# pigimonaco/Pinocchio

Measured on AMD Instinct MI355X. Metric: grid-cells/sec for full Fmax sweep (all smoothing radii) + 3LPT, 1024^3 box, higher is better.
Workload: dtype f64

## Files before the change

### include/pinfmax.h

```cpp
#ifndef PINFMAX_H
#define PINFMAX_H

#include <stddef.h>
#include <stdint.h>

#ifdef __cplusplus
extern "C" {
#endif

#define PF_NBINS 210
#define PF_MAX_SMOOTH 64

typedef struct pf_ctx pf_ctx;

typedef struct {
  int64_t n;
  int     rank;
  int     nranks;
  int     device;
  int     field_bytes;
  int     flags;
} pf_config;

#define PF_FLAG_TIMING 1
// ... 140 lines not shown
int pf_gather_velocities(pf_ctx *ctx, const pf_peak_region *box, size_t count, const unsigned int *frag_pos, const int *order,
                         size_t capacity, unsigned int *index, void *vel24, size_t *found);
int pf_refresh_velocities(pf_ctx *ctx, const pf_peak_region *box, size_t count, const unsigned int *frag_pos, const int *order,
                          void *frag, const pf_product_layout *layout, const pf_prev_layout *prev, size_t *found);
int pf_debug_gather_velocities(int n, int x0, int nxl, int pb, const void *cols24, const pf_peak_region *box, size_t count,
                               const unsigned int *frag_pos, const int *order, unsigned int *index, void *vel24, size_t *found);
typedef struct { size_t stride; long off_Mass, off_Vel, off_Vel_2LPT, off_Vel_3LPT_1, off_Vel_3LPT_2,
                 off_Vel_prev, off_Vel_2LPT_prev, off_Vel_3LPT_1_prev, off_Vel_3LPT_2_prev; } pf_group_layout;
int pf_group_velocity_sums(pf_ctx *ctx, const pf_peak_region *box, size_t count, const unsigned int *frag_pos,
                           const int *group_id, size_t group_stride, int first_group,
                           size_t capacity, int *group, unsigned int *npart, double *sum24,
                           size_t *groups_found, size_t *particles_found);
int pf_refresh_segment(pf_ctx *ctx, const pf_peak_region *box, size_t count, const unsigned int *frag_pos, const int *order,
                       const int *group_id, size_t group_stride, int first_group,
                       void *frag, const pf_product_layout *layout, const pf_prev_layout *prev,
                       void *groups, size_t ngroups, const pf_group_layout *gl,
                       size_t *loose, size_t *grouped, size_t *mass_mismatch);
int pf_debug_group_velocity_sums(int n, int x0, int nxl, int pb, const void *cols24, const pf_peak_region *box, size_t count,
                                 const unsigned int *frag_pos, const int *group_id, int first_group,
                                 int *group, unsigned int *npart, double *sum24, size_t *groups_found, size_t *particles_found);
int pf_debug_groupvel_times(double *ms3);
#define PF_PLC_LAST_CHECK 0
#define PF_PLC_EVENTS 1
typedef struct { int n; const double *x, *comvdist, *hubble; int nk; const double *grow[4], *fomega[4];
                 double logkmin, deltalogk, k_for_GM, rad_gm0; int nsmooth; const double *k_gm_displ; } pf_plc_cosmology;
typedef struct { int i, j, k; double F1, F2; } pf_plc_replication;
typedef struct { double center[3], xvers[3], yvers[3], zvers[3], aperture, Fstop, InterPartDist; long long GSglobal[3];
                 size_t nrep; const pf_plc_replication *repls; double LastzForPLC, delta_z; int nzbins; } pf_plc_geometry;
typedef struct { int myseg, use_v31; double z_seg, z_prev; } pf_plc_segment;
typedef struct { size_t stride; long off_Mass, off_Pos, off_name, off_Flast, off_good, off_point, off_Vel, off_Vel_2LPT, off_Vel_3LPT_1, off_Vel_3LPT_2,
                 off_Vel_prev, off_Vel_2LPT_prev, off_Vel_3LPT_1_prev, off_Vel_3LPT_2_prev; } pf_plc_group_layout;
typedef struct { size_t stride; long off_Mass, off_name, off_z, off_x, off_v; } pf_plc_out_layout;
int pf_plc_set_cosmology(pf_ctx *ctx, const pf_plc_cosmology *cosmo);
int pf_plc_set_geometry(pf_ctx *ctx, const pf_plc_geometry *geom);
int pf_plc_cross(pf_ctx *ctx, int mode, const pf_plc_segment *seg, const pf_peak_region *box,
                 size_t ncand, const void *groups, const pf_plc_group_layout *gl,
                 const void *f_lo, size_t f_lo_stride, int min_mass,
                 size_t capacity, void *plcgroups, const pf_plc_out_layout *ol,
                 unsigned int *cand_of, int *rep_of, double *nz,
                 size_t *count, size_t *unconverged);
int pf_debug_plc_times(double *ms2);
typedef struct { double F, InterPartDist, ParticleMass, hfactor; long long GSglobal[3]; int pbc[3]; int min_mass; } pf_catalog_params;
typedef struct { size_t stride; long off_name, off_M, off_x, off_v, off_q, off_n; } pf_catalog_out_layout;
typedef struct { int nbin; double mmin, deltam; } pf_mf_bins;
int pf_catalog(pf_ctx *ctx, const pf_plc_segment *seg, const pf_peak_region *box, const pf_catalog_params *par,
               size_t ngroups, const void *groups, const pf_plc_group_layout *gl,
               size_t capacity, void *catalog, const pf_catalog_out_layout *ol, unsigned int *group_of,
               const pf_mf_bins *bins, int *ninbin, double *massinbin, size_t *count);
int pf_debug_catalog_times(double *ms2);
int pf_debug_catalog_parts(double *ms4);
typedef struct { double sigma0, k_sigma, k_point; int order; } pf_point_params;
int pf_point_states(pf_ctx *ctx, const pf_plc_segment *seg, const pf_peak_region *box, const pf_point_params *par,
                    size_t count, const unsigned int *frag_pos, const int *order,
                    size_t capacity, unsigned int *index, void *states, size_t *found);
int pf_debug_point_states(int n, int x0, int nxl, int pb, const void *fmax_col, const void *cols24,
                          pf_ctx *tables_ctx, const pf_plc_segment *seg, const pf_peak_region *box, const pf_point_params *par,
                          size_t count, const unsigned int *frag_pos, const int *order,
                          unsigned int *index, void *states, size_t *found);
int pf_debug_point_times(double *ms2);
int pf_get_block(pf_ctx *ctx, const char *name, int id_bytes, void *host);
int pf_get_second_derivative(pf_ctx *ctx, int i, double *host);
int pf_get_kvector(pf_ctx *ctx, int which, double *host);
int pf_get_density(pf_ctx *ctx, double *host);
int pf_debug_replicated_rows(pf_ctx *ctx, int kx0, int nkx, double *host);
int pf_forward_transform(pf_ctx *ctx, const double *real_host, double *spec_host);
int pf_reverse_transform(pf_ctx *ctx, const double *spec_host, double *real_host);
int pf_derivative(pf_ctx *ctx, const double *spec_host, int first_derivative, int second_derivative, double rs_cells,
                  int order, double *real_host);
int pf_debug_math(pf_ctx *ctx, int which, const double *a, const double *b, size_t count, double *out);
int pf_debug_stream_rate(pf_ctx *ctx, int kind, int reps, double *gbps);
int pf_debug_lines(int field_bytes, int n, int pass, int mul, int band, int nouter, int ncols, int pre, double rs,
                   double growth, int outer_offset, const double *in, double *out);
int pf_debug_pk(int which, const float *a, const float *b, float *out, int count);
int pf_debug_gfft(int n, int dir, const double *in, double *out);
int pf_debug_gfft_lines(int n, int mode, int dir, int nlines, const double *in, double *out);
int pf_debug_strided_jobs(int field_bytes, int n, int njobs, int nin, const int *in_of, const int *mul, int nouter, int ncols,
                          const double *in, double *out);
int pf_debug_strided_band(int field_bytes, int n, int njobs, int nin, const int *in_of, const int *mul, int nouter, int ncols,
                          int in_pitch, int out_pitch, int band_e, int band_outer, int outer_offset, int pre, double rs, double growth,
                          const double *in, double *out, int *guard_ok);
int pf_debug_zpass_jobs(int field_bytes, int n, int form, int njobs, const int *mul, const int *out_f32, int in_place, int nrows, int band,
                        double norm, const double *dc, int ncu, const double *spec, const double *hess, const double *acc, double *out,
                        int *sentinel_ok);
int pf_debug_strided_xfuse(int field_bytes, int n, int njobs, const int *mul, int nouter, int ncols, int pre, double rs, double growth,
                           int outer_offset, const double *in, double *out_fused, double *out_plain);
int pf_debug_invariant_reruns(pf_ctx *ctx);
int pf_solve_ran_beside_zpass(pf_ctx *ctx);
int pf_transform_path(pf_ctx *ctx);
int pf_invgrow_table_status(pf_ctx *ctx, int ismooth, double *max_rel_err);
int pf_collapse_cells(pf_ctx *ctx, int ismooth, const double *d, size_t count, double *F);
enum { PF_ARITH_FAST = 0, PF_ARITH_EXACT = 1 };
int pf_set_arithmetic(pf_ctx *ctx, int flavour);
int pf_get_arithmetic(pf_ctx *ctx);
#define PF_CENSUS_BINS 64
typedef struct {
  unsigned long long cells;
  unsigned long long differing_bits;
  unsigned long long hist[PF_CENSUS_BINS];
  unsigned long long beyond_2ulp;
  unsigned long long rmax_differing;
  unsigned long long nonfinite;
  unsigned long long outliers;
  double max_abs, max_ulps;
  unsigned long long max_abs_cell;
} pf_census;
typedef struct { unsigned long long cell; double fast, exact; int rmax_fast, rmax_exact; } pf_census_cell;
int pf_flavour_census(pf_ctx *ctx, int ns, const double *radius_cells, double *true_variance,
                      pf_census *out, size_t capacity, pf_census_cell *cells);
int pf_debug_census(int product_bytes, unsigned long long first_cell, size_t count,
                    const void *fmax_fast, const int *rmax_fast, const void *fmax_exact, const int *rmax_exact,
                    pf_census *out, size_t capacity, pf_census_cell *cells);

int pf_power_bins(int n);
typedef struct {
  unsigned long long modes;
  unsigned long long nonfinite;
} pf_power_info;
int pf_power_spectrum(pf_ctx *ctx, int which, int ns, const double *radius_cells,
                      unsigned long long *nmodes, unsigned long long *k2sum, double *power,
                      double *variance, pf_power_info *info);
int pf_debug_power_spectrum(int field_bytes, int n, int y0, int nyl, const double *spec_host,
                            int ns, const double *radius_cells,
                            unsigned long long *nmodes, unsigned long long *k2sum, double *power,
                            double *variance, pf_power_info *info);
int pf_debug_power_times(double *ms);

#define PF_MATTER_NGP 1
#define PF_MATTER_DECONVOLVE 2
typedef struct {
  unsigned long long deposited, nonfinite, outside, empty_cells, max_cell, sum_hi32, sum_lo32, modes, nonfinite_modes;
} pf_matter_info;
int pf_matter_power(pf_ctx *ctx, int flags, const double *weight,
                    unsigned long long *nmodes, unsigned long long *k2sum, double *power, double *cross,
                    double *density_host, pf_matter_info *info);
int pf_debug_matter_deposit(int pb, int n, const void *vel12_host, int flags, const double *weight,
                            unsigned long long *grid_host, pf_matter_info *info);
int pf_debug_matter_shells(int field_bytes, int n, int y0, int nyl, const double *spec_m, const double *spec_lin,
                           int flags, unsigned long long *nmodes, unsigned long long *k2sum, double *power, double *cross,
                           pf_matter_info *info);
int pf_debug_matter_times(double *ms);
int pf_debug_matter_form(int *form);

int pf_matter_power_slabs(pf_ctx *ctx, int flags, const double *weight,
                          unsigned long long *nmodes, unsigned long long *k2sum, double *power, double *cross,
                          double *density_host, pf_matter_info *info);
int pf_debug_matter_slabs(pf_ctx *ctx, const void *vel12_slab_host, int flags, const double *weight,
                          unsigned long long *grid_slab_host, pf_matter_info *info);
int pf_debug_matter_exchange(unsigned long long out[6]);

#define PF_HALO_NGP 1
#define PF_HALO_DECONVOLVE 2
#define PF_HALO_MASS_WEIGHT 4
#define PF_HALO_MAX_BINS 8
typedef struct {
  unsigned long long selected, weight_sum, weight2_hi, weight2_lo, nonfinite, outside,
                     empty_cells, max_cell, modes, nonfinite_modes;
} pf_halo_info;
int pf_halo_power(pf_ctx *ctx, int flags, size_t count, const double *pos, double scale, const int *mass,
                  int nbins, const int *mass_range,
                  unsigned long long *nmodes, unsigned long long *k2sum,
                  double *power, double *cross, pf_halo_info *info);
int pf_debug_halo_deposit(int n, int x0, int nxl, int flags, size_t count, const double *pos, double scale,
                          const int *mass, int lo, int hi, unsigned long long *grid_host, pf_halo_info *info);
int pf_debug_halo_times(double *ms);

#define PF_MULTIPOLE_ORDERS 3
// ... 45 lines not shown
```

### pinocchio_amd/_lib.py

```python
from __future__ import annotations

import ctypes as C
import os

PKG = os.path.dirname(os.path.abspath(__file__))
SO = os.environ.get("PINFMAX_LIB") or os.path.join(PKG, "libpinfmax_hip.so")
NBINS = 210
MAX_SMOOTH = 64

FLAG_TIMING = 1
FLAG_DOUBLE_PRODUCTS = 2
MAP_CURRENT = 0
MAP_UPDATE = 1
NEIGH_SKIP, NEIGH_GOOD, NEIGH_PEAK = 1, 2, 4


class Config(C.Structure):
    _fields_ = [("n", C.c_int64), ("rank", C.c_int), ("nranks", C.c_int), ("device", C.c_int),
                ("field_bytes", C.c_int), ("flags", C.c_int)]


class ProductLayout(C.Structure):
    _fields_ = [("stride", C.c_size_t), ("off_Rmax", C.c_int), ("off_Fmax", C.c_int), ("off_Vel", C.c_int),
                ("off_Vel_2LPT", C.c_int), ("off_Vel_3LPT_1", C.c_int), ("off_Vel_3LPT_2", C.c_int)]
# ... 181 lines not shown
                                C.POINTER(C.c_uint), C.POINTER(C.c_size_t)]),
    "pf_debug_distribute": (C.c_int, [C.c_int, C.c_int, C.c_int, C.POINTER(C.c_float), C.c_double, C.POINTER(SubBox), C.POINTER(C.c_uint),
                                      C.c_size_t, C.POINTER(C.c_uint), C.POINTER(C.c_uint), C.POINTER(C.c_size_t)]),
    "pf_distribute_sorted": (C.c_int, [_vp, C.c_double, C.POINTER(SubBox), C.POINTER(C.c_uint), C.POINTER(ProductLayout), C.c_size_t, _vp,
                                       C.POINTER(C.c_uint), C.POINTER(C.c_uint), C.POINTER(C.c_int), C.POINTER(C.c_size_t)]),
    "pf_organize": (C.c_int, [_vp, C.POINTER(ProductLayout), C.c_size_t, _vp, C.POINTER(C.c_uint), C.POINTER(C.c_uint), C.POINTER(C.c_int)]),
    "pf_debug_organize": (C.c_int, [C.c_size_t, C.POINTER(C.c_float), C.POINTER(C.c_uint), C.POINTER(C.c_uint), C.POINTER(C.c_uint), C.POINTER(C.c_int)]),
    "pf_map_create": (C.c_int, [_vp, C.POINTER(PeakRegion), C.POINTER(_vp)]),
    "pf_map_destroy": (None, [_vp]),
    "pf_map_length": (C.c_size_t, [_vp]),
    "pf_map_fill_box": (C.c_int, [_vp]),
    "pf_map_update": (C.c_int, [_vp, C.c_size_t, _dp, C.POINTER(C.c_int), C.c_double, C.POINTER(C.c_ulonglong)]),
    "pf_map_commit": (C.c_int, [_vp, C.c_int]),
    "pf_map_get": (C.c_int, [_vp, C.c_int, C.POINTER(C.c_uint)]),
    "pf_map_set": (C.c_int, [_vp, C.c_int, C.POINTER(C.c_uint)]),
    "pf_map_count": (C.c_int, [_vp, C.c_int, C.POINTER(C.c_ulonglong)]),
    "pf_debug_map_atomics": (C.c_int, [_vp, C.POINTER(C.c_ulonglong)]),
    "pf_distribute_map": (C.c_int, [_vp, C.c_double, _vp, C.c_int, C.POINTER(ProductLayout), C.c_size_t, _vp, C.POINTER(C.c_uint),
                                    C.POINTER(C.c_size_t)]),
    "pf_distribute_sorted_map": (C.c_int, [_vp, C.c_double, _vp, C.c_int, C.POINTER(ProductLayout), C.c_size_t, _vp, C.POINTER(C.c_uint),
                                           C.POINTER(C.c_uint), C.POINTER(C.c_int), C.POINTER(C.c_size_t)]),
    "pf_count_peaks_map": (C.c_int, [_vp, C.c_double, _vp, C.c_int, C.POINTER(C.c_ulonglong)]),
    "pf_neighbours": (C.c_int, [_vp, C.POINTER(PeakRegion), C.c_size_t, C.POINTER(C.c_uint), _vp, C.c_size_t, C.POINTER(C.c_int),
                                C.POINTER(C.c_ubyte), C.POINTER(C.c_ulonglong)]),
    "pf_debug_neigh_ms": (C.c_int, [_dp, _dp]),
    "pf_distribute_sorted_neighbours_map": (C.c_int, [_vp, C.c_double, _vp, C.c_int, C.POINTER(ProductLayout), C.c_size_t, _vp, C.POINTER(C.c_uint),
                                                      C.POINTER(C.c_uint), C.POINTER(C.c_int), C.POINTER(C.c_int), C.POINTER(C.c_ubyte),
                                                      C.POINTER(C.c_ulonglong), C.POINTER(C.c_size_t)]),
    "pf_back_reset": (C.c_int, [_vp]),
    "pf_distribute_back": (C.c_int, [_vp, C.POINTER(PeakRegion), C.c_size_t, C.POINTER(C.c_uint), _vp, C.c_size_t, _vp, C.c_size_t, C.POINTER(C.c_size_t)]),
    "pf_back_apply": (C.c_int, [_vp, C.c_size_t, _vp, C.c_size_t, _vp, C.c_size_t, _vp, C.c_size_t]),
    "pf_update_back": (C.c_int, [_vp, _vp, C.c_size_t, C.c_long, C.c_long]),
    "pf_debug_distribute_back": (C.c_int, [C.c_int, C.c_int, C.c_int, C.POINTER(PeakRegion), C.c_size_t, C.POINTER(C.c_uint), C.POINTER(C.c_float),
                                           C.POINTER(C.c_int), C.POINTER(C.c_float), C.POINTER(C.c_int), C.POINTER(C.c_size_t)]),
    "pf_shift_displacements": (C.c_int, [_vp]),
    "pf_drop_prev": (C.c_int, [_vp]),
    "pf_prev_shifts": (C.c_int, [_vp]),
    "pf_gather_velocities": (C.c_int, [_vp, C.POINTER(PeakRegion), C.c_size_t, C.POINTER(C.c_uint), C.POINTER(C.c_int), C.c_size_t, C.POINTER(C.c_uint), _vp,
                                       C.POINTER(C.c_size_t)]),
    "pf_refresh_velocities": (C.c_int, [_vp, C.POINTER(PeakRegion), C.c_size_t, C.POINTER(C.c_uint), C.POINTER(C.c_int), _vp, C.POINTER(ProductLayout),
                                        C.POINTER(PrevLayout), C.POINTER(C.c_size_t)]),
    "pf_debug_gather_velocities": (C.c_int, [C.c_int, C.c_int, C.c_int, C.c_int, _vp, C.POINTER(PeakRegion), C.c_size_t, C.POINTER(C.c_uint), C.POINTER(C.c_int),
                                             C.POINTER(C.c_uint), _vp, C.POINTER(C.c_size_t)]),
    "pf_group_velocity_sums": (C.c_int, [_vp, C.POINTER(PeakRegion), C.c_size_t, C.POINTER(C.c_uint), C.POINTER(C.c_int), C.c_size_t, C.c_int, C.c_size_t,
                                         C.POINTER(C.c_int), C.POINTER(C.c_uint), C.POINTER(C.c_double), C.POINTER(C.c_size_t), C.POINTER(C.c_size_t)]),
    "pf_refresh_segment": (C.c_int, [_vp, C.POINTER(PeakRegion), C.c_size_t, C.POINTER(C.c_uint), C.POINTER(C.c_int), C.POINTER(C.c_int), C.c_size_t, C.c_int,
                                     _vp, C.POINTER(ProductLayout), C.POINTER(PrevLayout), _vp, C.c_size_t, C.POINTER(GroupLayout), C.POINTER(C.c_size_t),
                                     C.POINTER(C.c_size_t), C.POINTER(C.c_size_t)]),
    "pf_debug_group_velocity_sums": (C.c_int, [C.c_int, C.c_int, C.c_int, C.c_int, _vp, C.POINTER(PeakRegion), C.c_size_t, C.POINTER(C.c_uint),
                                               C.POINTER(C.c_int), C.c_int, C.POINTER(C.c_int), C.POINTER(C.c_uint), C.POINTER(C.c_double),
                                               C.POINTER(C.c_size_t), C.POINTER(C.c_size_t)]),
    "pf_debug_groupvel_times": (C.c_int, [C.POINTER(C.c_double)]),
    "pf_plc_set_cosmology": (C.c_int, [_vp, C.POINTER(PlcCosmology)]),
    "pf_plc_set_geometry": (C.c_int, [_vp, C.POINTER(PlcGeometry)]),
    "pf_plc_cross": (C.c_int, [_vp, C.c_int, C.POINTER(PlcSegment), C.POINTER(PeakRegion), C.c_size_t, _vp, C.POINTER(PlcGroupLayout), _vp, C.c_size_t, C.c_int,
                               C.c_size_t, _vp, C.POINTER(PlcOutLayout), C.POINTER(C.c_uint), C.POINTER(C.c_int), C.POINTER(C.c_double), C.POINTER(C.c_size_t),
                               C.POINTER(C.c_size_t)]),
    "pf_debug_plc_times": (C.c_int, [C.POINTER(C.c_double)]),
    "pf_catalog": (C.c_int, [_vp, C.POINTER(PlcSegment), C.POINTER(PeakRegion), C.POINTER(CatalogParams), C.c_size_t, _vp, C.POINTER(PlcGroupLayout), C.c_size_t, _vp,
                             C.POINTER(CatalogOutLayout), C.POINTER(C.c_uint), C.POINTER(MfBins), C.POINTER(C.c_int), C.POINTER(C.c_double), C.POINTER(C.c_size_t)]),
    "pf_debug_catalog_times": (C.c_int, [C.POINTER(C.c_double)]),
    "pf_debug_catalog_parts": (C.c_int, [C.POINTER(C.c_double)]),
    "pf_point_states": (C.c_int, [_vp, C.POINTER(PlcSegment), C.POINTER(PeakRegion), C.POINTER(PointParams), C.c_size_t, C.POINTER(C.c_uint), C.POINTER(C.c_int),
                                  C.c_size_t, C.POINTER(C.c_uint), _vp, C.POINTER(C.c_size_t)]),
    "pf_debug_point_states": (C.c_int, [C.c_int, C.c_int, C.c_int, C.c_int, _vp, _vp, _vp, C.POINTER(PlcSegment), C.POINTER(PeakRegion), C.POINTER(PointParams),
                                        C.c_size_t, C.POINTER(C.c_uint), C.POINTER(C.c_int), C.POINTER(C.c_uint), _vp, C.POINTER(C.c_size_t)]),
    "pf_debug_point_times": (C.c_int, [C.POINTER(C.c_double)]),
    "pf_set_collapse_model": (C.c_int, [_vp, C.c_int, C.POINTER(C.c_double), C.c_int, C.POINTER(C.c_double)]),
    "pf_set_modified_gravity": (C.c_int, [_vp, C.c_double, C.c_double, C.c_int, C.POINTER(C.c_double)]),
    "pf_set_tabulated_ct": (C.c_int, [_vp, C.c_int, C.POINTER(C.c_double)]),
    "pf_ct_build": (C.c_int, [_vp, C.c_int, C.c_double, C.POINTER(C.c_double)]),
    "pf_ct_load": (C.c_int, [_vp, C.c_int, C.c_double, C.POINTER(C.c_double)]),
    "pf_debug_math": (C.c_int, [_vp, C.c_int, C.POINTER(C.c_double), C.POINTER(C.c_double), C.c_size_t, C.POINTER(C.c_double)]),
    "pf_debug_stream_rate": (C.c_int, [_vp, C.c_int, C.c_int, _dp]),
    "pf_debug_lines": (C.c_int, [C.c_int, C.c_int, C.c_int, C.c_int, C.c_int, C.c_int, C.c_int, C.c_int, C.c_double, C.c_double, C.c_int, _dp, _dp]),
    "pf_debug_pk": (C.c_int, [C.c_int, C.POINTER(C.c_float), C.POINTER(C.c_float), C.POINTER(C.c_float), C.c_int]),
    "pf_debug_gfft": (C.c_int, [C.c_int, C.c_int, _dp, _dp]),
    "pf_debug_gfft_lines": (C.c_int, [C.c_int, C.c_int, C.c_int, C.c_int, _dp, _dp]),
    "pf_debug_strided_jobs": (C.c_int, [C.c_int, C.c_int, C.c_int, C.c_int, C.POINTER(C.c_int), C.POINTER(C.c_int), C.c_int, C.c_int, _dp, _dp]),
    "pf_debug_strided_band": (C.c_int, [C.c_int, C.c_int, C.c_int, C.c_int, C.POINTER(C.c_int), C.POINTER(C.c_int), C.c_int, C.c_int, C.c_int, C.c_int,
                                        C.c_int, C.c_int, C.c_int, C.c_int, C.c_double, C.c_double, _dp, _dp, C.POINTER(C.c_int)]),
    "pf_debug_zpass_jobs": (C.c_int, [C.c_int, C.c_int, C.c_int, C.c_int, C.POINTER(C.c_int), C.POINTER(C.c_int), C.c_int, C.c_int, C.c_int, C.c_double,
                                      _dp, C.c_int, _dp, _dp, _dp, _dp, C.POINTER(C.c_int)]),
    "pf_debug_strided_xfuse": (C.c_int, [C.c_int, C.c_int, C.c_int, C.POINTER(C.c_int), C.c_int, C.c_int, C.c_int, C.c_double, C.c_double, C.c_int,
                                         _dp, _dp, _dp]),
    "pf_debug_invariant_reruns": (C.c_int, [_vp]),
    "pf_solve_ran_beside_zpass": (C.c_int, [_vp]),
    "pf_transform_path": (C.c_int, [_vp]),
    "pf_invgrow_table_status": (C.c_int, [_vp, C.c_int, _dp]),
    "pf_set_loopback_exchange": (C.c_int, [_vp, C.c_int]),
    "pf_loopback_active": (C.c_int, [_vp]),
    "pf_set_sources_in_sweep": (C.c_int, [_vp, C.c_int]),
    "pf_set_lpt_order": (C.c_int, [_vp, C.c_int]),
    "pf_set_ct_interpolation": (C.c_int, [_vp, C.c_int]),
    "pf_set_transposed_spectra": (C.c_int, [_vp, C.c_int]),
    "pf_replicated_spectrum": (C.c_int, [_vp]),
    "pf_update_products": (C.c_int, [_vp, _vp, C.POINTER(ProductLayout)]),
    "pf_set_growth_table": (C.c_int, [_vp, C.c_int, C.POINTER(C.c_double), C.c_int, C.c_double, C.c_double, C.c_double]),
    "pf_get_second_derivative": (C.c_int, [_vp, C.c_int, _dp]),
    "pf_get_kvector": (C.c_int, [_vp, C.c_int, _dp]),
    "pf_get_density": (C.c_int, [_vp, _dp]),
    "pf_debug_replicated_rows": (C.c_int, [_vp, C.c_int, C.c_int, _dp]),
    "pf_plan_bytes": (C.c_int, [C.POINTER(Config), C.POINTER(C.c_size_t), C.POINTER(C.c_size_t)]),
    "pf_forward_transform": (C.c_int, [_vp, _dp, _dp]),
    "pf_reverse_transform": (C.c_int, [_vp, _dp, _dp]),
    "pf_collapse_cells": (C.c_int, [_vp, C.c_int, _dp, C.c_size_t, _dp]),
    "pf_set_arithmetic": (C.c_int, [_vp, C.c_int]),
    "pf_get_arithmetic": (C.c_int, [_vp]),
    "pf_flavour_census": (C.c_int, [_vp, C.c_int, _dp, _dp, C.POINTER(Census), C.c_size_t, C.POINTER(CensusCell)]),
    "pf_debug_census": (C.c_int, [C.c_int, C.c_ulonglong, C.c_size_t, _vp, C.POINTER(C.c_int), _vp, C.POINTER(C.c_int), C.POINTER(Census), C.c_size_t,
                                  C.POINTER(CensusCell)]),
    "pf_power_bins": (C.c_int, [C.c_int]),
    "pf_power_spectrum": (C.c_int, [_vp, C.c_int, C.c_int, _dp, C.POINTER(C.c_ulonglong), C.POINTER(C.c_ulonglong), _dp, _dp, C.POINTER(PowerInfo)]),
    "pf_debug_power_spectrum": (C.c_int, [C.c_int, C.c_int, C.c_int, C.c_int, _dp, C.c_int, _dp, C.POINTER(C.c_ulonglong), C.POINTER(C.c_ulonglong), _dp, _dp,
                                          C.POINTER(PowerInfo)]),
    "pf_debug_power_times": (C.c_int, [_dp]),
    "pf_matter_power": (C.c_int, [_vp, C.c_int, _dp, C.POINTER(C.c_ulonglong), C.POINTER(C.c_ulonglong), _dp, _dp, _dp, C.POINTER(MatterInfo)]),
    "pf_debug_matter_deposit": (C.c_int, [C.c_int, C.c_int, _vp, C.c_int, _dp, C.POINTER(C.c_ulonglong), C.POINTER(MatterInfo)]),
    "pf_debug_matter_shells": (C.c_int, [C.c_int, C.c_int, C.c_int, C.c_int, _dp, _dp, C.c_int, C.POINTER(C.c_ulonglong), C.POINTER(C.c_ulonglong), _dp, _dp,
                                         C.POINTER(MatterInfo)]),
    "pf_debug_matter_times": (C.c_int, [_dp]),
    "pf_debug_matter_form": (C.c_int, [C.POINTER(C.c_int)]),
    "pf_matter_power_slabs": (C.c_int, [_vp, C.c_int, _dp, C.POINTER(C.c_ulonglong), C.POINTER(C.c_ulonglong), _dp, _dp, _dp, C.POINTER(MatterInfo)]),
    "pf_debug_matter_slabs": (C.c_int, [_vp, _vp, C.c_int, _dp, C.POINTER(C.c_ulonglong), C.POINTER(MatterInfo)]),
    "pf_debug_matter_exchange": (C.c_int, [C.POINTER(C.c_ulonglong)]),
    "pf_halo_power": (C.c_int, [_vp, C.c_int, C.c_size_t, _dp, C.c_double, C.POINTER(C.c_int), C.c_int, C.POINTER(C.c_int), C.POINTER(C.c_ulonglong),
                                C.POINTER(C.c_ulonglong), _dp, _dp, C.POINTER(HaloInfo)]),
    "pf_debug_halo_deposit": (C.c_int, [C.c_int, C.c_int, C.c_int, C.c_int, C.c_size_t, _dp, C.c_double, C.POINTER(C.c_int), C.c_int, C.c_int,
                                        C.POINTER(C.c_ulonglong), C.POINTER(HaloInfo)]),
    "pf_debug_halo_times": (C.c_int, [_dp]),
    "pf_halo_multipoles": (C.c_int, [_vp, C.c_int, C.c_size_t, _dp, _dp, C.c_double, C.c_double, C.c_int, C.POINTER(C.c_int), C.c_int, C.POINTER(C.c_int),
                                     C.POINTER(C.c_ulonglong), C.POINTER(C.c_ulonglong), _dp, _dp, C.POINTER(HaloInfo)]),
    "pf_debug_halo_deposit_rsd": (C.c_int, [C.c_int, C.c_int, C.c_int, C.c_int, C.c_size_t, _dp, _dp, C.c_double, C.c_double, C.c_int, C.POINTER(C.c_int), C.c_int, C.c_int,
                                            C.POINTER(C.c_ulonglong), C.POINTER(HaloInfo)]),
    "pf_debug_multipole_shells": (C.c_int, [C.c_int, C.c_int, C.c_int, C.c_int, _dp, _dp, C.c_int, C.c_int, C.POINTER(C.c_ulonglong), C.POINTER(C.c_ulonglong), _dp, _dp, _dp,
                                            C.POINTER(MatterInfo)]),
    "pf_debug_multipole_form": (C.c_int, [C.POINTER(C.c_int)]),
    "pf_halo_correlation": (C.c_int, [_vp, C.c_int, C.c_size_t, _dp, _dp, C.c_double, C.c_double, C.c_int, C.POINTER(C.c_int), C.c_int, C.POINTER(C.c_int),
                                      C.POINTER(C.c_ulonglong), C.POINTER(C.c_ulonglong), _dp, _dp, C.POINTER(CorrInfo)]),
    "pf_debug_corr_form": (C.c_int, [C.c_int, C.c_int, C.c_int, C.c_int, _dp, _dp, C.c_int, C.c_int, _dp, C.POINTER(MatterInfo)]),
    "pf_debug_corr_shells": (C.c_int, [C.c_int, C.c_int, C.c_int, C.c_int, _dp, C.c_int, C.POINTER(C.c_ulonglong), C.POINTER(C.c_ulonglong), _dp, _dp,
                                       C.POINTER(C.c_ulonglong)]),
    "pf_debug_corr_times": (C.c_int, [_dp]),
    "pf_get_cputime": (C.c_int, [_vp, C.POINTER(CpuTime)]),
    "pf_reset_cputime": (C.c_int, [_vp]),
    "pf_kernel_stats": (C.c_int, [_vp, C.POINTER(KernelStat), C.c_int, C.POINTER(C.c_int)]),
    "pf_reset_kernel_stats": (C.c_int, [_vp]),
    "pf_synchronize": (C.c_int, [_vp]),
    "pf_device_bytes": (C.c_size_t, [_vp]),
}

_lib = None


def source_sha() -> str:
    import glob
    import hashlib
    h = hashlib.sha256()
    for path in sorted(glob.glob(os.path.join(PKG, "csrc", "*.hip")) + glob.glob(os.path.join(PKG, "csrc", "*.h")) +
                       glob.glob(os.path.join(PKG, "csrc", "*.cpp"))):
        h.update(os.path.basename(path).encode())
        with open(path, "rb") as fh:
            h.update(fh.read())
    return h.hexdigest()[:16]


# ... 15 lines not shown
```

### pinocchio_amd/csrc/pf_api.hip

```cpp
#include <hip/hip_runtime.h>

#include <math.h>
#include <stdarg.h>
#include <stdio.h>
#include <stdlib.h>
#include <string.h>

#include <atomic>
#include <string>
#include <functional>
#include <vector>

#include "../../include/pinfmax.h"
#include "pf_collapse_core.h"
#include "pf_hostpool.h"
#include "pf_internal.h"

extern "C" void pf_rccl_release(void *link);
extern "C" int pf_rccl_link_count(void *link);

static thread_local char g_err[512] = "";
int pf_fail(int task, const char *fmt, ...) {
  va_list ap;
  va_start(ap, fmt);
// ... 181 lines not shown
  }
  c->evs.clear();
  for (auto &e : c->phase_evs) {
    float ms = 0; hipEventElapsedTime(&ms, e.a, e.b);
    double s = 1e-3 * ms;
    if (e.kind == 0) c->cpu.deriv += s; else if (e.kind == 1) c->cpu.coll += s; else if (e.kind == 2) c->cpu.lpt += s;
    else if (e.kind == 3) c->cpu.mem_transf += s; else if (e.kind == 4) c->cpu.fmax += s;
    c->evpool.push_back(e.a); c->evpool.push_back(e.b);
  }
  c->phase_evs.clear();
}

static size_t ncell_of(const pf_ctx *c) { return (size_t)c->nxl * c->n * c->n; }
static int dev_alloc(pf_ctx *c, void **p, size_t bytes) {
  HIPCHK(c, hipMalloc(p, bytes));
  c->dev_bytes += bytes;
  return 0;
}

static int ensure_b2(pf_ctx *c, bool quiet = false) {
  if (c->blockB2) return 0;
  if (hipMalloc((void **)&c->blockB2, 6 * c->field_bytes) != hipSuccess) {
    (void)hipGetLastError(); c->blockB2 = nullptr;
    return quiet ? 1 : pf_fail(c->rank, "hipMalloc of the second field set failed (%.1f GB; %.1f GB held by this context)", 6e-9 * c->field_bytes, 1e-9 * c->dev_bytes);
  }
  c->dev_bytes += 6 * c->field_bytes;
  for (int i = 0; i < 6; i++) c->B2[i] = c->blockB2 + i * c->field_bytes;
  return 0;
}
static int inv_rows(pf_ctx *c, int set, bool quiet = false) {
  if (c->INV[set][0]) return 0;
  const size_t row_set = ncell_of(c) * sizeof(double);
  if (2 * c->field_bytes < row_set) return pf_fail(c->rank, "internal: an invariant row set does not fit two fields");
  if (set == 1) {
    if (ensure_b2(c, quiet)) return 1;
    for (int k = 0; k < 3; k++) c->INV[1][k] = (double *)(c->blockB2 + 2 * k * c->field_bytes);
    return 0;
  }
  for (int k = 0; k < 2; k++)
    if (!c->inv_own[k]) PFCHK(c, dev_alloc(c, (void **)&c->inv_own[k], row_set));
  c->INV[0][0] = (double *)c->blockS; c->INV[0][1] = c->inv_own[0]; c->INV[0][2] = c->inv_own[1];
  return 0;
}

static void host_twiddles(int n, int fb, std::vector<char> &h) {
  h.resize((size_t)n * 2 * fb);
  for (int j = 0; j < n; j++) {
    long double a = 2.0L * 3.14159265358979323846264338327950288L * (long double)j / (long double)n;
    double re = (double)cosl(a), im = (double)sinl(a);
    if (j == 0) { re = 1; im = 0; } else if (4 * j == n) { re = 0; im = 1; } else if (2 * j == n) { re = -1; im = 0; } else if (4 * j == 3 * n) { re = 0; im = -1; }
    if (fb == 8) { ((double *)h.data())[2 * j] = re; ((double *)h.data())[2 * j + 1] = im; }
    else { ((float *)h.data())[2 * j] = (float)re; ((float *)h.data())[2 * j + 1] = (float)im; }
  }
}

extern "C" void pf_layout_3lpt(pf_product_layout *l) {
  l->stride = 56; l->off_Rmax = 0; l->off_Fmax = 4; l->off_Vel = 8; l->off_Vel_2LPT = 20; l->off_Vel_3LPT_1 = 32; l->off_Vel_3LPT_2 = 44;
}

static size_t ncell(const pf_ctx *c) { return (size_t)c->nxl * c->n * c->n; }
static long long rpitch(const pf_ctx *c) { return c->general ? c->n : 2 * c->nzp; }
static double spec_bytes_alg(const pf_ctx *c) { return (double)c->n * c->nyl * c->nzh * 2.0 * c->fb; }
static double real_bytes_alg(const pf_ctx *c) { return (double)ncell(c) * c->fb; }

static int env_int(const char *name, int dflt) { const char *e = getenv(name); return e ? atoi(e) : dflt; }
static void read_tuning(PfTuning *t) {
  t->zpass_persist = env_int("PF_ZPASS_PERSIST", 24);
  t->zpass_inv_wg_per_cu = env_int("PF_ZPASS_INV_WG_PER_CU", 32);
  if (t->zpass_inv_wg_per_cu <= 0) t->zpass_inv_wg_per_cu = 32;
  t->spline_lut = env_int("PF_SPLINE_LUT", 1) != 0;
  t->exchange_rows = env_int("PF_EXCHANGE_ROWS", 1) != 0;
  t->invariants = env_int("PF_INVARIANTS", 1);
  t->lpt_fuse = env_int("PF_LPT_FUSE", 1);
  t->collapse_wg_per_cu = env_int("PF_COLLAPSE_WG_PER_CU", 8);
  if (t->collapse_wg_per_cu <= 0) t->collapse_wg_per_cu = 8;
  t->general = env_int("PF_GENERAL", 0) != 0;

  t->pipeline = env_int("PF_PIPELINE", 1) != 0;
  t->replicate = env_int("PF_REPLICATE_DK", -1);
  t->exact_libm = env_int("PF_EXACT_LIBM", 0) != 0;
  t->solve_beside_z = env_int("PF_SOLVE_BESIDE_Z", -1);
  t->gtab = env_int("PF_GTAB", 1) != 0;
  t->lpt_xfuse = env_int("PF_LPT_XFUSE", 1) != 0;
  t->lpt3b_start = env_int("PF_LPT3B_START", 0) != 0;
  t->preflight = env_int("PF_PREFLIGHT", 1) != 0;
  t->handoff_chunk_mb = env_int("PF_HANDOFF_CHUNK_MB", 256);
  if (t->handoff_chunk_mb <= 0) t->handoff_chunk_mb = 256;
  t->handoff_threads = env_int("PF_HANDOFF_THREADS", 0);
  t->host_register = env_int("PF_HOST_REGISTER", 0) != 0;
  t->distribute_lds = env_int("PF_DISTRIBUTE_LDS", 1) != 0;
  const char *fault = getenv("PF_DEBUG_PIPELINE_FAULT");
  t->debug_fault = !fault ? 0 : !strcmp(fault, "recv") ? 1 : !strcmp(fault, "send") ? 2 : 0;
  t->prune_eps = 8.673617379884035e-19;
  if (const char *e = getenv("PF_PRUNE_EPS")) t->prune_eps = atof(e);
}

static void plan_bytes(const pf_ctx *c, size_t *at_create, size_t *peak) {
  const size_t field = c->field_bytes, nc = ncell_of(c);
  size_t fields = 1 + 3 + 6 + 3;
  if (c->P > 1) fields += 3;
  if (c->replicate) fields += (size_t)c->P;
  if (c->pipeline) fields += 6;
  if (c->general) fields += 1;
  size_t b = fields * field + nc * ((size_t)c->pb + sizeof(int) + 12 * (size_t)c->pb);
  b += (2 * PF_NBLK + PF_NBLK + SC_COUNT) * sizeof(double) + PF_NBINS * sizeof(unsigned long long) +
       (size_t)(PF_MAX_SMOOTH + 1) * (5 * PF_KNOT_CAP * sizeof(double) + PF_GT_DOUBLES * sizeof(double) + PF_GT_MAX_BINS * sizeof(unsigned short)) +
       4 * PF_KBIN_CAP * sizeof(double) + (size_t)c->n * sizeof(double) + (size_t)c->n * 2 * c->fb;
  *at_create = b;
  b += 6 * field;
  if (c->fb == 4 && !c->general && pf_c2r_invariants_supported(c->fb, c->n)) b += 2 * nc * sizeof(double);
  *peak = b;
}
extern "C" int pf_plan_bytes(const pf_config *cfg, size_t *at_create, size_t *peak) {
  if (!cfg || cfg->nranks < 1 || cfg->n < 4 || cfg->n % cfg->nranks || (cfg->field_bytes != 4 && cfg->field_bytes != 8)) return 1;
  PfTuning tune;
  read_tuning(&tune);
  pf_ctx v;
  const int n = (int)cfg->n;
  const bool pow2 = !(n & (n - 1));
  v.n = n; v.P = cfg->nranks; v.fb = cfg->field_bytes; v.pb = (cfg->flags & PF_FLAG_DOUBLE_PRODUCTS) ? 8 : 4;
  v.general = tune.general || (!pow2 && !pf_mixed_supported(n));
  v.nzh = n / 2 + 1; v.nzp = v.general ? v.nzh : n / 2 + 64 / v.fb; v.nxl = v.nyl = n / v.P;
  v.field_bytes = (size_t)v.n * v.nyl * v.nzp * 2 * v.fb;
  v.pipeline = v.P > 1 && tune.pipeline;
  v.replicate = v.P > 1 && !v.general && (tune.replicate < 0 ? v.P <= 4 : tune.replicate != 0);
  size_t a = 0, b = 0;
  plan_bytes(&v, &a, &b);
  if (at_create) *at_create = a;
  if (peak) *peak = b;
  return 0;
}

static int create_body(pf_ctx *c, const pf_config *cfg) {
  const int rank = cfg->rank;
  HIPCHK(c, hipSetDevice(cfg->device));
  c->field_bytes = (size_t)c->n * c->nyl * c->nzp * 2 * c->fb;
  c->replicate = c->P > 1 && !c->general && (c->tune.replicate < 0 ? c->P <= 4 : c->tune.replicate != 0);
  if (c->tune.preflight) {
    size_t at_create = 0, peak = 0, free_b = 0, total_b = 0;
    plan_bytes(c, &at_create, &peak);
    HIPCHK(c, hipMemGetInfo(&free_b, &total_b));
    if (peak > free_b)
      return pf_fail(rank, "pf_create: %d^3 on %d ranks with %d-byte fields needs %.1f GB of device memory per rank (%.1f GB at creation, the rest with the "
                           "LPT part), device %d has %.1f GB free of %.1f GB", c->n, c->P, c->fb, 1e-9 * peak, 1e-9 * at_create, cfg->device, 1e-9 * free_b, 1e-9 * total_b);
  }
  HIPCHK(c, hipStreamCreate(&c->stream));
  HIPCHK(c, hipStreamCreate(&c->cstream));
  {
    int lo = 0, hi = 0;
    HIPCHK(c, hipDeviceGetStreamPriorityRange(&lo, &hi));
    HIPCHK(c, hipStreamCreateWithPriority(&c->sstream, hipStreamNonBlocking, lo));
  }
  for (int i = 0; i < 2; i++) {
    HIPCHK(c, hipEventCreateWithFlags(&c->ev_y[i], hipEventDisableTiming));
    HIPCHK(c, hipEventCreateWithFlags(&c->ev_s[i], hipEventDisableTiming));
    HIPCHK(c, hipEventCreateWithFlags(&c->ev_x[i], hipEventDisableTiming));
    HIPCHK(c, hipEventCreateWithFlags(&c->ev_r[i], hipEventDisableTiming));
  }
  {
    hipDeviceProp_t prop;
    HIPCHK(c, hipGetDeviceProperties(&prop, cfg->device));
    c->fast_libm = !c->tune.exact_libm;
    c->ncu = prop.multiProcessorCount;
    c->prune_eps = c->tune.prune_eps;
    c->collapse_blocks = prop.multiProcessorCount * c->tune.collapse_wg_per_cu;
    if (c->collapse_blocks > PF_NBLK) c->collapse_blocks = PF_NBLK;
// ... 267 lines not shown
  if (!piece) return pf_fail(c->rank, "hand-off: a record of %zu bytes does not fit the staging pieces", granule);
  const size_t np = (bytes + piece - 1) / piece;
  auto issue = [&](size_t k) -> int {
    const int b = (int)(k & 1);
    const size_t off = k * piece, len = bytes - off < piece ? bytes - off : piece;
    const char *src = src_dev ? src_dev + off : handoff_dev(c, b);
    if (fill(off, len, handoff_dev(c, b), h->st[b])) return 1;
    HIPCHK(c, hipMemcpyAsync(h->pin[b], src, len, hipMemcpyDeviceToHost, h->st[b]));
    return 0;
  };
  if (np && issue(0)) return 1;
  for (size_t k = 0; k < np; k++) {
    if (k + 1 < np && issue(k + 1)) return 1;
    const int b = (int)(k & 1);
    HIPCHK(c, hipStreamSynchronize(h->st[b]));
    const size_t off = k * piece, len = bytes - off < piece ? bytes - off : piece;
    char *dst = host + off; const char *src = h->pin[b];
    h->pool->run(len, [=](size_t a, size_t e) { memcpy(dst + a, src + a, e - a); });
  }
  return 0;
}
static int no_fill(size_t, size_t, char *, hipStream_t) { return 0; }
static int handoff_h2d(pf_ctx *c, char *dst_dev, const char *host, size_t bytes) {
  PfHandoff *h;
  if (handoff_get(c, &h)) return 1;
  PFCHK(c, handoff_begin(c, h));
  const size_t piece = h->chunk, np = (bytes + piece - 1) / piece;
  for (size_t k = 0; k < np; k++) {
    const int b = (int)(k & 1);
    const size_t off = k * piece, len = bytes - off < piece ? bytes - off : piece;
    HIPCHK(c, hipStreamSynchronize(h->st[b]));
    char *dst = h->pin[b]; const char *src = host + off;
    h->pool->run(len, [=](size_t a, size_t e) { memcpy(dst + a, src + a, e - a); });
    HIPCHK(c, hipMemcpyAsync(dst_dev + off, h->pin[b], len, hipMemcpyHostToDevice, h->st[b]));
  }
  for (int i = 0; i < 2; i++) HIPCHK(c, hipStreamSynchronize(h->st[i]));
  return 0;
}
static bool handoff_registered(pf_ctx *c, PfHandoff *h, void *host, size_t bytes) {
  if (!h->want_register || ((uintptr_t)host & 4095)) return false;
  if (h->reg_ptr == host && h->reg_bytes >= bytes) return true;
  if (h->reg_ptr) { (void)hipHostUnregister(h->reg_ptr); h->reg_ptr = nullptr; h->reg_bytes = 0; }
  if (hipHostRegister(host, bytes, hipHostRegisterDefault) != hipSuccess) { (void)hipGetLastError(); return false; }
  h->reg_ptr = host; h->reg_bytes = bytes;
  return true;
}

static int ilog2i(int v) { int l = 0; while ((1 << l) < v) l++; return l; }
static PfAddr addr_ky_x(const pf_ctx *c) {
  PfAddr a; a.os = c->nzp; a.el_shift = ilog2i(c->n); a.el_len = c->n; a.ehs = 0; a.els = (long long)c->nyl * c->nzp; return a;
}
static PfAddr addr_blocks_y(const pf_ctx *c) {
  PfAddr a; a.os = (long long)c->nyl * c->nzp; a.el_shift = ilog2i(c->nyl); a.el_len = c->nyl; a.ehs = (long long)c->nxl * c->nyl * c->nzp; a.els = c->nzp; return a;
}
static PfAddr addr_yblocks_x(const pf_ctx *c, int zp) {
  PfAddr a; a.os = (long long)c->nxl * zp; a.el_shift = ilog2i(c->nxl); a.el_len = c->nxl; a.ehs = (long long)c->nyl * c->nxl * c->nzp; a.els = zp; return a;
}
static PfAddr addr_yblocks_y(const pf_ctx *c, int zp) {
  PfAddr a; a.os = zp; a.el_shift = ilog2i(c->nyl); a.el_len = c->nyl; a.ehs = (long long)c->nyl * c->nxl * c->nzp; a.els = (long long)c->nxl * zp; return a;
}
static PfAddr addr_full_x(const pf_ctx *c) {
  PfAddr a; a.os = c->nzp; a.el_shift = ilog2i(c->n); a.el_len = c->n; a.ehs = 0; a.els = (long long)c->n * c->nzp; return a;
}
static PfAddr addr_local_x(const pf_ctx *c, int zp) {
  PfAddr a; a.os = (long long)c->nxl * zp; a.el_shift = ilog2i(c->nxl); a.el_len = c->nxl; a.ehs = 0; a.els = zp; return a;
}
static PfAddr addr_local_y(const pf_ctx *c, int zp) {
  PfAddr a; a.os = zp; a.el_shift = ilog2i(c->n); a.el_len = c->n; a.ehs = 0; a.els = (long long)c->nxl * zp; return a;
}
static PfAddr addr_xs_y(const pf_ctx *c) {
  PfAddr a; a.os = (long long)c->n * c->nzp; a.el_shift = ilog2i(c->n); a.el_len = c->n; a.ehs = 0; a.els = c->nzp; return a;
}

struct Job { const void *in; void *out; int mul; };

static int xpass(pf_ctx *c, int kind, int dir, int njobs, const Job *jobs, int pre, double rs, double growth, int nin, int band = 1 << 30,
                 bool out_yblocks = false, bool replicated = false, bool fwd_first = false) {
  PfStridedParams p; memset(&p, 0, sizeof(p));
  p.njobs = njobs;
  for (int j = 0; j < njobs; j++) { p.job[j].in = jobs[j].in; p.job[j].out = jobs[j].out; p.job[j].mul = jobs[j].mul; }
  p.ain = p.aout = addr_ky_x(c);
  if (out_yblocks) p.aout = addr_yblocks_x(c, band_zpitch(c, band));
  p.ncols = c->nzh; p.nouter = c->nyl; p.pre = pre; p.outer_offset = c->rank * c->nyl; p.rs = rs; p.growth = growth; p.tw = c->tw;
  p.etab = c->etab; p.dev = c->dev;
  if (replicated) {
    p.ain = addr_full_x(c); p.aout = addr_local_x(c, band_zpitch(c, band));
    p.nouter = c->n; p.outer_offset = 0; p.out_e0 = c->rank * c->nxl; p.out_ne = c->nxl;
  }
  if (pre && rs != 0.0) PFCHK(c, pf_launch_exp_table(c->etab, c->n, rs, c->stream));
  p.band_e = p.band_outer = c->n;
  double frac_cols = 1.0, frac_in = 1.0, frac_outer = 1.0;
  if (band < c->n / 2) {
    p.band_e = p.band_outer = band;
    p.ncols = band + 1;
    frac_cols = (double)(band + 1) / c->nzh; frac_in = frac_outer = (double)(2 * band + 1) / c->n;
  }
  KTimer t(c, kind, (nin * frac_in * (replicated ? c->P : 1) + njobs) * frac_cols * frac_outer * spec_bytes_alg(c));
  if (fwd_first) {
    if (dir < 0 || replicated) return pf_fail(c->rank, "xpass: a pending forward x-transform goes with an inverse pass over this rank's own spectrum");
    PFCHK(c, pf_launch_strided_xfuse(c->fb, c->n, p, c->stream));
    return 0;
  }
  PFCHK(c, pf_launch_strided(c->fb, c->n, dir, p, c->stream));
  return 0;
}
static int ypass(pf_ctx *c, int kind, int dir, int njobs, const Job *jobs, bool in_blocks, bool out_blocks, int nin, int band = 1 << 30,
                 bool in_yblocks = false, bool in_local = false) {
  PfStridedParams p; memset(&p, 0, sizeof(p));
  p.njobs = njobs;
  for (int j = 0; j < njobs; j++) { p.job[j].in = jobs[j].in; p.job[j].out = jobs[j].out; p.job[j].mul = jobs[j].mul; }
  p.ain = in_blocks ? (in_yblocks ? addr_yblocks_y(c, band_zpitch(c, band)) : addr_blocks_y(c)) : addr_xs_y(c);
  if (in_local) p.ain = addr_local_y(c, band_zpitch(c, band));
  p.aout = out_blocks ? addr_blocks_y(c) : addr_xs_y(c);
  p.ncols = c->nzh; p.nouter = c->nxl; p.pre = 0; p.outer_offset = 0; p.rs = 0; p.growth = 1; p.tw = c->tw; p.dev = c->dev;
  p.band_e = p.band_outer = c->n;
  double frac_cols = 1.0, frac_in = 1.0;
  if (band < c->n / 2) {
    p.band_e = band;
    p.ncols = band + 1;
    frac_cols = (double)(band + 1) / c->nzh; frac_in = (double)(2 * band + 1) / c->n;
  }
  KTimer t(c, kind, (nin * frac_in + njobs) * frac_cols * spec_bytes_alg(c));
  PFCHK(c, pf_launch_strided(c->fb, c->n, dir, p, c->stream));
  return 0;
}
struct ZJob { const void *in; void *out; int mul; int f32; };
static int zpass_c2r(pf_ctx *c, int kind, int njobs, const ZJob *jobs, const double *dc, int band = 1 << 30, bool invariants = false,
                     void *acc = nullptr) {
  PfC2RParams p; memset(&p, 0, sizeof(p));
  p.njobs = njobs;
  double outb = 0;
  for (int j = 0; j < njobs; j++) {
    p.job[j].in = jobs[j].in; p.job[j].out = jobs[j].out; p.job[j].mul = jobs[j].mul; p.job[j].out_f32 = jobs[j].f32;
    outb += jobs[j].f32 ? (double)ncell(c) * 4.0 : real_bytes_alg(c);
  }
  p.nlines = (long long)c->nxl * c->n; p.in_pitch = c->nzp; p.out_pitch = 2 * c->nzp;
  p.norm = 1.0 / ((double)c->n * c->n * c->n); p.dc = dc; p.tw = c->tw;
  p.band_k = c->n;
  double frac_in = 1.0;
  if (band < c->n / 2) { p.band_k = band; frac_in = (double)(band + 1) / c->nzh; }
  p.ncu = c->ncu; p.dev = c->dev; p.persist_per_cu = c->tune.zpass_persist; p.inv_per_cu = c->tune.zpass_inv_wg_per_cu;
  p.flag = c->scal + SC_INV_FLAG;
  if (acc) {
    p.acc = acc;
    const bool start_here = c->s3b_start_absent;
    KTimer t(c, KS_ZPASS_LPT3B, njobs * frac_in * spec_bytes_alg(c) + (start_here ? 7.0 : 8.0) * real_bytes_alg(c));
    PFCHK(c, pf_launch_c2r_invariants(c->fb, c->n, p, c->stream, start_here ? 2 : 1));
    c->s3b_start_absent = false;
    return 0;
  }
  if (invariants) {
    if (c->fb == 4) {
      if (inv_rows(c, c->inv_w)) return 1;
      for (int k = 0; k < 3; k++) p.inv_out[k] = c->INV[c->inv_w][k];
      p.inv_pitch = c->n;
      if (c->inv_w == 0) c->have_sources = false;
    }
    KTimer t(c, KS_ZPASS_INV, njobs * frac_in * spec_bytes_alg(c) + 3.0 * (double)ncell(c) * 8.0);
    PFCHK(c, pf_launch_c2r_invariants(c->fb, c->n, p, c->stream));
    return 0;
  }
  KTimer t(c, kind, njobs * frac_in * spec_bytes_alg(c) + outb);
  PFCHK(c, pf_launch_c2r(c->fb, c->n, p, c->stream));
  return 0;
}

__global__ void k_debug_idle(long long ticks) {
  const long long t0 = wall_clock64();
  while (wall_clock64() - t0 < ticks) __builtin_amdgcn_s_sleep(32);
}
template <class Pre, class Dst, class Post, class Band>
static int pipelined_band(pf_ctx *c, int count, int nf, Pre pre, Dst dst, Post post, Band band, bool local = false) {
  void *A[2][3];
  const void *R[3];
  if (local) {
    for (int i = 0; i < count; i++) {
      void *D[3];
      for (int f = 0; f < nf; f++) { D[f] = dst(i, 0, f); R[f] = D[f]; }
      if (pre(i, D)) return 1;
      if (post(i, R)) return 1;
    }
    return 0;
  }
  for (int f = 0; f < 3; f++) { A[0][f] = c->A[f]; A[1][f] = c->pipeline ? (void *)(c->blockA2 + f * c->field_bytes) : c->A[f]; }
  if (c->P == 1 || !c->pipeline) {
    for (int i = 0; i < count; i++) {
      if (pre(i, A[0])) return 1;
      for (int f = 0; f < nf; f++) {
        R[f] = A[0][f];
        if (c->P > 1) { void *d = dst(i, 0, f); PFCHK(c, exchange_band(c, A[0][f], d, band(i))); R[f] = d; }
      }
      if (post(i, R)) return 1;
    }
    return 0;
  }
  auto issue = [&](int i) -> int {
    const int s = i & 1;
    if (c->tune.debug_fault == 2) hipLaunchKernelGGL(k_debug_idle, dim3(1), dim3(1), 0, c->stream, 200000LL);
    if (pre(i, A[s])) return 1;
    HIPCHK(c, hipEventRecord(c->ev_x[s], c->stream));
    if (c->tune.debug_fault != 2) HIPCHK(c, hipStreamWaitEvent(c->cstream, c->ev_x[s], 0));
    for (int f = 0; f < nf; f++) PFCHK(c, exchange_band(c, A[s][f], dst(i, s, f), band(i), c->cstream));
    HIPCHK(c, hipEventRecord(c->ev_r[s], c->cstream));
    return 0;
  };
  if (issue(0)) return 1;
  for (int i = 0; i < count; i++) {
    if (i + 1 < count && issue(i + 1)) return 1;
    if (c->tune.debug_fault != 1) HIPCHK(c, hipStreamWaitEvent(c->stream, c->ev_r[i & 1], 0));
    for (int f = 0; f < nf; f++) R[f] = dst(i, i & 1, f);
    if (post(i, R)) return 1;
  }
  return 0;
}
template <class Pre, class Dst, class Post>
static int pipelined(pf_ctx *c, int count, int nf, Pre pre, Dst dst, Post post) {
  return pipelined_band(c, count, nf, pre, dst, post, [](int) { return 1 << 30; });
}
static void *recv_field(pf_ctx *c, int set, int f) { return (char *)(set ? c->recvA2 : c->recvA) + (size_t)f * c->field_bytes; }

static int g_filter(pf_ctx *c, const void *in, void *out, int a, int b, double rs, int order, bool normalise) {
  double growth = order ? c->growth[order - 1] : 1.0;
  const int o = order - 1;
  const bool tab = order && c->gt_n[o];
// ... 1634 lines not shown
      return pf_fail(c->rank, "pf_debug_exchange: row-range all-to-all failed");
    HIPCHK(c, hipMemcpyAsync(h.data(), recv, h.size() * 8, hipMemcpyDeviceToHost, c->stream));
    HIPCHK(c, hipStreamSynchronize(c->stream));
    for (int p = 0; p < c->P; p++)
      for (size_t i = 0; i < nw; i++) {
        const bool in = 8 * i >= off[p] && 8 * i < off[p] + len[p];
        const unsigned long long want = in ? (((unsigned long long)p << 48) | ((unsigned long long)c->rank << 40) | i) : 0ull;
        if (h[p * nw + i] != want) return pf_fail(c->rank, "pf_debug_exchange: row-range exchange, wrong word from rank %d at %zu", p, i);
      }
  }
  if (c->ared) {
    double v[2] = {1.0 + c->rank, 2.0};
    HIPCHK(c, hipMemcpyAsync(c->scal, v, sizeof(v), hipMemcpyHostToDevice, c->stream));
    if (c->ared(c->ared_user, c->scal, 2, 0, (void *)c->stream)) return pf_fail(c->rank, "pf_debug_exchange: all-reduce failed");
    HIPCHK(c, hipMemcpyAsync(v, c->scal, sizeof(v), hipMemcpyDeviceToHost, c->stream));
    HIPCHK(c, hipStreamSynchronize(c->stream));
    if (v[0] != 0.5 * c->P * (c->P + 1) || v[1] != 2.0 * c->P) return pf_fail(c->rank, "pf_debug_exchange: wrong all-reduce result");
    HIPCHK(c, hipMemsetAsync(c->scal, 0, 2 * sizeof(double), c->stream));
  }
  return 0;
}

extern "C" int pf_debug_lines(int field_bytes, int n, int pass, int mul, int band, int nouter, int ncols, int pre, double rs,
                              double growth, int outer_offset, const double *in, double *out) {
  double *flag_out = (pass == 4 && out) ? out + (size_t)3 * nouter * n : nullptr;
  if (!in || !out || nouter < 1 || (field_bytes != 8 && field_bytes != 4) || n < 8 || n > 2048 || pass < 0 || pass > 4)
    return pf_fail(0, "pf_debug_lines: bad argument");
  if (n & (n - 1)) {
    PfMixedPlan pl;
    if (!(pass <= 1 ? pf_mixed_plan(n, false, &pl) : (n % 2 == 0 && pf_mixed_plan(n / 2, true, &pl))))
      return pf_fail(0, "pf_debug_lines: no stage plan for %d points in pass %d", n, pass);
  } else if (n < 16) return pf_fail(0, "pf_debug_lines: bad argument");
  if (pass == 4 && !pf_c2r_invariants_supported(field_bytes, n))
    return pf_fail(0, "pf_debug_lines: the invariant z-pass takes rows whose six lines fit a workgroup (fp64 rows of at most 1024 points, fp32 rows of at most 2048; n = 8 m as the grids)");
  const int fb = field_bytes, nzh = n / 2 + 1;
  pf_ctx *nc = nullptr;
  size_t n_in, n_out;
  const int pc = (ncols + 15) & ~15;
  if (pass <= 1) { if (ncols < 1) return pf_fail(0, "pf_debug_lines: ncols"); n_in = n_out = (size_t)nouter * n * ncols * 2; }
  else if (pass == 2) { n_in = (size_t)nouter * nzh * 2; n_out = (size_t)nouter * n; }
  else if (pass == 3) { n_in = (size_t)nouter * n; n_out = (size_t)nouter * nzh * 2; }
  else { n_in = (size_t)6 * nouter * nzh * 2; n_out = (size_t)3 * nouter * n; }
  const size_t n_in_alloc = pass == 3 ? (n_in > n_out ? n_in : n_out) : n_in;
  void *d_in = nullptr, *d_out = nullptr, *d_tw = nullptr; double *d_etab = nullptr, *d_flag = nullptr;
  PfTuning tune;
  read_tuning(&tune);
  int dev = 0, ncu = 0;
  {
    hipDeviceProp_t prop;
    if (hipGetDevice(&dev) != hipSuccess || hipGetDeviceProperties(&prop, dev) != hipSuccess) return pf_fail(0, "pf_debug_lines: no HIP device");
    ncu = prop.multiProcessorCount;
  }
  std::vector<char> tw;
  host_twiddles(n, fb, tw);
  int rc = 0;
  auto body = [&]() -> int {
    const size_t nrows01 = (size_t)nouter * n;
    const size_t dev01 = nrows01 * (size_t)pc * 2;
    HIPCHK(nc, hipMalloc(&d_in, (pass <= 1 ? dev01 : n_in_alloc) * fb));
    const size_t out_b = (pass == 4) ? 8 : (size_t)fb;
    HIPCHK(nc, hipMalloc(&d_out, (pass <= 1 ? dev01 : n_out) * out_b));
    HIPCHK(nc, hipMalloc(&d_tw, tw.size()));
    HIPCHK(nc, hipMalloc((void **)&d_etab, (size_t)n * sizeof(double)));
    HIPCHK(nc, hipMalloc((void **)&d_flag, sizeof(double)));
    HIPCHK(nc, hipMemset(d_flag, 0, sizeof(double)));
    HIPCHK(nc, hipMemcpy(d_tw, tw.data(), tw.size(), hipMemcpyHostToDevice));
    const size_t hrow = (size_t)ncols * 2 * fb, drow = (size_t)pc * 2 * fb;
    if (pass <= 1) HIPCHK(nc, hipMemset(d_in, 0, dev01 * fb));
    if (fb == 8) {
      if (pass <= 1) HIPCHK(nc, hipMemcpy2D(d_in, drow, in, hrow, hrow, nrows01, hipMemcpyHostToDevice));
      else HIPCHK(nc, hipMemcpy(d_in, in, n_in * 8, hipMemcpyHostToDevice));
    } else {
      std::vector<float> h(n_in);
      for (size_t i = 0; i < n_in; i++) h[i] = (float)in[i];
      if (pass <= 1) HIPCHK(nc, hipMemcpy2D(d_in, drow, h.data(), hrow, hrow, nrows01, hipMemcpyHostToDevice));
      else HIPCHK(nc, hipMemcpy(d_in, h.data(), n_in * 4, hipMemcpyHostToDevice));
    }
    HIPCHK(nc, hipMemset(d_out, 0, (pass <= 1 ? dev01 : n_out) * out_b));
    if (pass <= 1) {
      PfStridedParams p; memset(&p, 0, sizeof(p));
      p.njobs = 1; p.job[0].in = d_in; p.job[0].out = d_out; p.job[0].mul = mul;
      p.ain.os = (long long)n * pc; p.ain.el_shift = ilog2i(n); p.ain.el_len = n; p.ain.ehs = 0; p.ain.els = pc; p.aout = p.ain;
      p.ncols = ncols; p.nouter = nouter; p.pre = pre; p.outer_offset = outer_offset; p.rs = rs; p.growth = growth; p.tw = d_tw; p.etab = d_etab;
      p.band_e = p.band_outer = n; p.dev = dev;
      if (band < n / 2) p.band_e = band;
      if (pre && rs != 0.0) PFCHK0(pf_launch_exp_table(d_etab, n, rs, nullptr));
      PFCHK0(pf_launch_strided(fb, n, pass == 0 ? +1 : -1, p, nullptr));
    } else if (pass == 2 || pass == 4) {
      PfC2RParams p; memset(&p, 0, sizeof(p));
      p.njobs = pass == 2 ? 1 : 6;
      static const int mul6[6] = {PF_MUL_ONE, PF_MUL_ONE, PF_MUL_K2, PF_MUL_ONE, PF_MUL_K, PF_MUL_K};
      for (int j = 0; j < p.njobs; j++) {
        p.job[j].in = (char *)d_in + (size_t)j * nouter * nzh * 2 * fb;
        p.job[j].out = pass == 2 ? d_out : (char *)d_out + (size_t)(j % 3) * nouter * n * 8;
        if (pass == 4 && j < 3) p.inv_out[j] = (double *)((char *)d_out + (size_t)j * nouter * n * 8);
        p.job[j].mul = pass == 2 ? mul : mul6[j]; p.job[j].out_f32 = 0;
      }
      p.nlines = nouter; p.in_pitch = nzh; p.out_pitch = n; p.norm = 1.0; p.dc = nullptr; p.tw = d_tw; p.band_k = band < n / 2 ? band : n;
      p.ncu = ncu; p.dev = dev; p.persist_per_cu = tune.zpass_persist; p.inv_per_cu = tune.zpass_inv_wg_per_cu; p.flag = d_flag;
      p.inv_pitch = n;
      if (pass == 2) PFCHK0(pf_launch_c2r(fb, n, p, nullptr));
      else PFCHK0(pf_launch_c2r_invariants(fb, n, p, nullptr, 0));
    } else {
      PfR2CParams p; p.in = d_in; p.out = d_out; p.nlines = nouter; p.in_pitch = n; p.out_pitch = nzh; p.tw = d_tw;
      PFCHK0(pf_launch_r2c(fb, n, p, nullptr));
    }
    HIPCHK(nc, hipDeviceSynchronize());
    if (pass == 4 && flag_out) HIPCHK(nc, hipMemcpy(flag_out, d_flag, sizeof(double), hipMemcpyDeviceToHost));
    if (fb == 8 || pass == 4) {
      if (pass <= 1) HIPCHK(nc, hipMemcpy2D(out, hrow, d_out, drow, hrow, nrows01, hipMemcpyDeviceToHost));
      else HIPCHK(nc, hipMemcpy(out, d_out, n_out * 8, hipMemcpyDeviceToHost));
    } else {
      std::vector<float> h(n_out);
      if (pass <= 1) HIPCHK(nc, hipMemcpy2D(h.data(), hrow, d_out, drow, hrow, nrows01, hipMemcpyDeviceToHost));
      else HIPCHK(nc, hipMemcpy(h.data(), d_out, n_out * 4, hipMemcpyDeviceToHost));
      for (size_t i = 0; i < n_out; i++) out[i] = (double)h[i];
    }
    return 0;
  };
  rc = body();
  hipFree(d_in); hipFree(d_out); hipFree(d_tw); hipFree(d_etab); hipFree(d_flag);
  return rc;
}

extern "C" int pf_debug_strided_jobs(int field_bytes, int n, int njobs, int nin, const int *in_of, const int *mul, int nouter, int ncols,
                                     const double *in, double *out) {
  if (!in || !out || !in_of || !mul || njobs < 1 || njobs > PF_MAX_JOBS || nin < 1 || nin > njobs || nouter < 1 || ncols < 1 || (field_bytes != 8 && field_bytes != 4) ||
      n < 16 || n > 2048 || ((n & (n - 1)) && !pf_mixed_supported(n)))
    return pf_fail(0, "pf_debug_strided_jobs: bad argument");
  const int fb = field_bytes, pc = (ncols + 15) & ~15;
  pf_ctx *nc = nullptr;
  const size_t nrows = (size_t)nouter * n, field = nrows * (size_t)pc * 2;
  void *d_in = nullptr, *d_out = nullptr, *d_tw = nullptr;
  int dev = 0;
  if (hipGetDevice(&dev) != hipSuccess) return pf_fail(0, "pf_debug_strided_jobs: no HIP device");
  std::vector<char> tw;
  host_twiddles(n, fb, tw);
  auto body = [&]() -> int {
    HIPCHK(nc, hipMalloc(&d_in, (size_t)nin * field * fb));
    HIPCHK(nc, hipMalloc(&d_out, (size_t)njobs * field * fb));
    HIPCHK(nc, hipMalloc(&d_tw, tw.size()));
    HIPCHK(nc, hipMemcpy(d_tw, tw.data(), tw.size(), hipMemcpyHostToDevice));
    HIPCHK(nc, hipMemset(d_in, 0, (size_t)nin * field * fb));
    HIPCHK(nc, hipMemset(d_out, 0, (size_t)njobs * field * fb));
    const size_t hrow = (size_t)ncols * 2 * fb, drow = (size_t)pc * 2 * fb, hfield = nrows * (size_t)ncols * 2;
    std::vector<float> hf;
    for (int i = 0; i < nin; i++) {
      const void *src = in + (size_t)i * hfield;
      if (fb == 4) { hf.resize(hfield); for (size_t k = 0; k < hfield; k++) hf[k] = (float)in[(size_t)i * hfield + k]; src = hf.data(); }
      HIPCHK(nc, hipMemcpy2D((char *)d_in + (size_t)i * field * fb, drow, src, hrow, hrow, nrows, hipMemcpyHostToDevice));
    }
    PfStridedParams p; memset(&p, 0, sizeof(p));
    p.njobs = njobs;
    for (int j = 0; j < njobs; j++) {
      if (in_of[j] < 0 || in_of[j] >= nin) return pf_fail(0, "pf_debug_strided_jobs: in_of");
      p.job[j].in = (char *)d_in + (size_t)in_of[j] * field * fb; p.job[j].out = (char *)d_out + (size_t)j * field * fb; p.job[j].mul = mul[j];
    }
    p.ain.os = (long long)n * pc; p.ain.el_shift = (n & (n - 1)) ? 0 : ilog2i(n); p.ain.el_len = n; p.ain.ehs = 0; p.ain.els = pc; p.aout = p.ain;
    p.ncols = ncols; p.nouter = nouter; p.tw = d_tw; p.band_e = p.band_outer = n; p.dev = dev; p.growth = 1.0;
    PFCHK0(pf_launch_strided(fb, n, +1, p, nullptr));
    HIPCHK(nc, hipDeviceSynchronize());
    for (int j = 0; j < njobs; j++) {
      if (fb == 8) HIPCHK(nc, hipMemcpy2D(out + (size_t)j * hfield, hrow, (char *)d_out + (size_t)j * field * fb, drow, hrow, nrows, hipMemcpyDeviceToHost));
      else {
        hf.resize(hfield);
        HIPCHK(nc, hipMemcpy2D(hf.data(), hrow, (char *)d_out + (size_t)j * field * fb, drow, hrow, nrows, hipMemcpyDeviceToHost));
        for (size_t k = 0; k < hfield; k++) out[(size_t)j * hfield + k] = (double)hf[k];
      }
    }
    return 0;
  };
  const int rc = body();
  hipFree(d_in); hipFree(d_out); hipFree(d_tw);
  return rc;
}

extern "C" int pf_debug_strided_band(int field_bytes, int n, int njobs, int nin, const int *in_of, const int *mul, int nouter, int ncols,
                                     int in_pitch, int out_pitch, int band_e, int band_outer, int outer_offset, int pre, double rs, double growth,
                                     const double *in, double *out, int *guard_ok) {
  if (!in || !out || !in_of || !mul || !guard_ok || njobs < 1 || njobs > PF_MAX_JOBS || nin < 1 || nin > njobs || nouter < 1 || ncols < 1 ||
      (field_bytes != 8 && field_bytes != 4) || n < 16 || n > 2048 || ((n & (n - 1)) && !pf_mixed_supported(n)) || band_e < 0 || band_outer < 0 ||
      outer_offset < 0 || outer_offset >= n)
    return pf_fail(0, "pf_debug_strided_band: bad argument");
  const int fb = field_bytes, line = 64 / fb;
  if (in_pitch < ncols || out_pitch < ncols || in_pitch % line || out_pitch % line || in_pitch > 4096 || out_pitch > 4096)
    return pf_fail(0, "pf_debug_strided_band: rows of %d columns need pitches of whole 128-byte lines (%d complex) that hold them, not %d / %d", ncols, line, in_pitch, out_pitch);
  for (int j = 0; j < njobs; j++) if (in_of[j] < 0 || in_of[j] >= nin) return pf_fail(0, "pf_debug_strided_band: in_of");
  *guard_ok = 0;
  pf_ctx *nc = nullptr;
  const size_t nrows = (size_t)nouter * n, cb = (size_t)2 * fb;
  const size_t in_field = nrows * (size_t)in_pitch * cb, out_field = nrows * (size_t)out_pitch * cb;
  const size_t slot = (in_field > out_field ? in_field : out_field) + 4096, guard = slot - out_field;
  void *d_in = nullptr, *d_out = nullptr, *d_tw = nullptr; double *d_etab = nullptr;
  int dev = 0;
  if (hipGetDevice(&dev) != hipSuccess) return pf_fail(0, "pf_debug_strided_band: no HIP device");
  std::vector<char> tw;
  host_twiddles(n, fb, tw);
  auto body = [&]() -> int {
    HIPCHK(nc, hipMalloc(&d_in, (size_t)nin * in_field));
    HIPCHK(nc, hipMalloc(&d_out, (size_t)njobs * slot));
    HIPCHK(nc, hipMalloc(&d_tw, tw.size()));
    HIPCHK(nc, hipMalloc((void **)&d_etab, (size_t)n * sizeof(double)));
    HIPCHK(nc, hipMemcpy(d_tw, tw.data(), tw.size(), hipMemcpyHostToDevice));
    HIPCHK(nc, hipMemset(d_in, 0x7f, (size_t)nin * in_field));
    for (int j = 0; j < njobs; j++) {
      HIPCHK(nc, hipMemset((char *)d_out + (size_t)j * slot, 0, out_field));
      HIPCHK(nc, hipMemset((char *)d_out + (size_t)j * slot + out_field, 0xa5, guard));
    }
    const size_t hrow = (size_t)ncols * cb, hfield = nrows * (size_t)ncols * 2;
    std::vector<float> hf;
    for (int i = 0; i < nin; i++) {
      const void *src = in + (size_t)i * hfield;
      if (fb == 4) { hf.resize(hfield); for (size_t k = 0; k < hfield; k++) hf[k] = (float)in[(size_t)i * hfield + k]; src = hf.data(); }
      HIPCHK(nc, hipMemcpy2D((char *)d_in + (size_t)i * in_field, (size_t)in_pitch * cb, src, hrow, hrow, nrows, hipMemcpyHostToDevice));
    }
    PfStridedParams p; memset(&p, 0, sizeof(p));
    p.njobs = njobs;
    for (int j = 0; j < njobs; j++) { p.job[j].in = (char *)d_in + (size_t)in_of[j] * in_field; p.job[j].out = (char *)d_out + (size_t)j * slot; p.job[j].mul = mul[j]; }
    p.ain.os = (long long)n * in_pitch; p.ain.el_shift = (n & (n - 1)) ? 0 : ilog2i(n); p.ain.el_len = n; p.ain.ehs = 0; p.ain.els = in_pitch;
    p.aout = p.ain; p.aout.os = (long long)n * out_pitch; p.aout.els = out_pitch;
    p.ncols = ncols; p.nouter = nouter; p.pre = pre ? 1 : 0; p.outer_offset = outer_offset; p.rs = rs; p.growth = growth; p.tw = d_tw; p.etab = d_etab; p.dev = dev;
    p.band_e = band_e < n / 2 ? band_e : n; p.band_outer = band_outer < n / 2 ? band_outer : n;
    if (pre && rs != 0.0) PFCHK0(pf_launch_exp_table(d_etab, n, rs, nullptr));
    PFCHK0(pf_launch_strided(fb, n, +1, p, nullptr));
    HIPCHK(nc, hipDeviceSynchronize());
    for (int j = 0; j < njobs; j++) {
      const char *f = (const char *)d_out + (size_t)j * slot;
      if (fb == 8) HIPCHK(nc, hipMemcpy2D(out + (size_t)j * hfield, hrow, f, (size_t)out_pitch * cb, hrow, nrows, hipMemcpyDeviceToHost));
      else {
        hf.resize(hfield);
        HIPCHK(nc, hipMemcpy2D(hf.data(), hrow, f, (size_t)out_pitch * cb, hrow, nrows, hipMemcpyDeviceToHost));
        for (size_t k = 0; k < hfield; k++) out[(size_t)j * hfield + k] = (double)hf[k];
      }
    }
    std::vector<unsigned char> g(guard);
    int ok = 1;
    for (int j = 0; j < njobs; j++) {
      HIPCHK(nc, hipMemcpy(g.data(), (const char *)d_out + (size_t)j * slot + out_field, guard, hipMemcpyDeviceToHost));
      for (size_t k = 0; k < guard; k++) if (g[k] != 0xa5) { ok = 0; break; }
    }
    *guard_ok = ok;
    return 0;
  };
  const int rc = body();
  hipFree(d_in); hipFree(d_out); hipFree(d_tw); hipFree(d_etab);
  return rc;
}

extern "C" int pf_debug_zpass_jobs(int field_bytes, int n, int form, int njobs, const int *mul, const int *out_f32, int in_place, int nrows, int band,
                                   double norm, const double *dc, int ncu, const double *spec, const double *hess, const double *acc, double *out,
                                   int *sentinel_ok) {
  static const int mul6[6] = {PF_MUL_ONE, PF_MUL_ONE, PF_MUL_K2, PF_MUL_ONE, PF_MUL_K, PF_MUL_K};
  if (!spec || !out || !sentinel_ok || (field_bytes != 8 && field_bytes != 4) || n < 16 || n > 2048 || n % 2 || form < 0 || form > 2 || nrows < 1 ||
      nrows > (1 << 20) || band < 0 || ncu < 0)
    return pf_fail(0, "pf_debug_zpass_jobs: bad argument");
  const int fb = field_bytes;
  if (n & (n - 1)) {
    PfMixedPlan pl;
    if (!pf_mixed_supported(n) || !pf_mixed_plan(n / 2, true, &pl)) return pf_fail(0, "pf_debug_zpass_jobs: no stage plan for rows of %d points", n);
  }
  int f32[PF_MAX_JOBS], mu[PF_MAX_JOBS];
  if (form == 0) {
    if (!mul || !out_f32 || njobs < 1 || njobs > PF_MAX_JOBS) return pf_fail(0, "pf_debug_zpass_jobs: njobs");
    for (int j = 0; j < njobs; j++) {
      if (mul[j] < PF_MUL_ONE || mul[j] > PF_MUL_IK || out_f32[j] < 0 || out_f32[j] > 2) return pf_fail(0, "pf_debug_zpass_jobs: mul / out_f32");
      if (out_f32[j] == 2 && fb != 8) return pf_fail(0, "pf_debug_zpass_jobs: double products go with fp64 fields");
      if (in_place && out_f32[j] != 0) return pf_fail(0, "pf_debug_zpass_jobs: only F rows of the fields' own pitch are written in place");
      mu[j] = mul[j]; f32[j] = out_f32[j];
    }
  } else {
    if (!hess || !acc) return pf_fail(0, "pf_debug_zpass_jobs: bad argument");
    if (!pf_c2r_invariants_supported(fb, n) || (form == 2 && (n & (n - 1))))
      return pf_fail(0, "pf_debug_zpass_jobs: no contracting z-pass (mode %d) for rows of %d points in fields of %d bytes", form, n, fb);
    njobs = 6; in_place = 0;
    for (int j = 0; j < 6; j++) { mu[j] = mul6[j]; f32[j] = 0; }
  }
  *sentinel_ok = 0;
  pf_ctx *nc = nullptr;
  const size_t nzh = (size_t)n / 2 + 1, nzp = (size_t)n / 2 + 64 / fb;
  const size_t R = (size_t)nrows, row_b = 2 * nzp * fb;
  const size_t field_b = R * row_b;
  auto out_rows_b = [&](int j) { return f32[j] == 0 ? field_b : R * n * (f32[j] == 1 ? 4 : fb); };
  auto out_buf_b = [&](int j) { return f32[j] == 0 ? field_b : out_rows_b(j) + (size_t)n * 8 + 4096; };
  void *d_in[PF_MAX_JOBS] = {}, *d_out[PF_MAX_JOBS] = {}, *d_acc = nullptr, *d_tw = nullptr; double *d_dc = nullptr;
  int dev = 0;
  {
    hipDeviceProp_t prop;
    if (hipGetDevice(&dev) != hipSuccess || hipGetDeviceProperties(&prop, dev) != hipSuccess) return pf_fail(0, "pf_debug_zpass_jobs: no HIP device");
    if (ncu == 0) ncu = prop.multiProcessorCount;
  }
  PfTuning tune;
  read_tuning(&tune);
  std::vector<char> tw;
  host_twiddles(n, fb, tw);
  auto image = [&](const double *src, size_t cnt, std::vector<unsigned char> &h) {
    h.assign(field_b, 0xa5);
    for (size_t r = 0; r < R; r++)
      for (size_t k = 0; k < cnt; k++) {
        if (fb == 8) ((double *)(h.data() + r * row_b))[k] = src[r * cnt + k];
        else ((float *)(h.data() + r * row_b))[k] = (float)src[r * cnt + k];
      }
  };
  auto body = [&]() -> int {
    std::vector<unsigned char> h, before[PF_MAX_JOBS], acc_before, after;
    for (int j = 0; j < njobs; j++) {
      HIPCHK(nc, hipMalloc(&d_in[j], field_b));
      image(spec + (size_t)j * R * nzh * 2, nzh * 2, h);
      HIPCHK(nc, hipMemcpy(d_in[j], h.data(), field_b, hipMemcpyHostToDevice));
      if (in_place) { d_out[j] = d_in[j]; before[j] = h; continue; }
      HIPCHK(nc, hipMalloc(&d_out[j], out_buf_b(j)));
      if (form == 0) before[j].assign(out_buf_b(j), 0xa5);
      else image(hess + (size_t)j * R * n, (size_t)n, before[j]);
      HIPCHK(nc, hipMemcpy(d_out[j], before[j].data(), before[j].size(), hipMemcpyHostToDevice));
    }
    if (form != 0) {
      HIPCHK(nc, hipMalloc(&d_acc, field_b));
      image(acc, (size_t)n, acc_before);
      HIPCHK(nc, hipMemcpy(d_acc, acc_before.data(), field_b, hipMemcpyHostToDevice));
    }
    HIPCHK(nc, hipMalloc(&d_tw, tw.size()));
    HIPCHK(nc, hipMemcpy(d_tw, tw.data(), tw.size(), hipMemcpyHostToDevice));
    if (dc) {
      HIPCHK(nc, hipMalloc((void **)&d_dc, sizeof(double)));
      HIPCHK(nc, hipMemcpy(d_dc, dc, sizeof(double), hipMemcpyHostToDevice));
    }
    PfC2RParams p; memset(&p, 0, sizeof(p));
    p.njobs = njobs;
    for (int j = 0; j < njobs; j++) { p.job[j].in = d_in[j]; p.job[j].out = d_out[j]; p.job[j].mul = mu[j]; p.job[j].out_f32 = f32[j]; }
    p.nlines = nrows; p.in_pitch = (long long)nzp; p.out_pitch = 2 * (long long)nzp;
    p.norm = norm; p.dc = d_dc; p.tw = d_tw;
    p.band_k = band < n / 2 ? band : n;
    p.ncu = ncu; p.dev = dev; p.persist_per_cu = tune.zpass_persist; p.inv_per_cu = tune.zpass_inv_wg_per_cu;
    if (form == 0) PFCHK0(pf_launch_c2r(fb, n, p, nullptr));
    else { p.acc = d_acc; PFCHK0(pf_launch_c2r_invariants(fb, n, p, nullptr, form)); }
    HIPCHK(nc, hipDeviceSynchronize());
    int ok = 1;
    auto collect = [&](const std::vector<unsigned char> &got, const std::vector<unsigned char> &was, size_t pitch_b, size_t sb, double *dst) {
      for (size_t r = 0; r < R; r++) {
        const unsigned char *g = got.data() + r * pitch_b;
        if (dst) for (size_t k = 0; k < (size_t)n; k++) dst[r * n + k] = sb == 8 ? ((const double *)g)[k] : (double)((const float *)g)[k];
        const size_t from = r * pitch_b + (dst ? (size_t)n * sb : 0), to = (r + 1) * pitch_b;
        if (memcmp(got.data() + from, was.data() + from, to - from)) ok = 0;
      }
      if (got.size() > R * pitch_b && memcmp(got.data() + R * pitch_b, was.data() + R * pitch_b, got.size() - R * pitch_b)) ok = 0;
    };
    for (int j = 0; j < njobs; j++) {
      after.resize(before[j].size());
      HIPCHK(nc, hipMemcpy(after.data(), d_out[j], after.size(), hipMemcpyDeviceToHost));
      if (form != 0) collect(after, before[j], row_b, fb, nullptr);
      else if (f32[j] == 0) collect(after, before[j], row_b, fb, out + (size_t)j * R * n);
      else { const size_t sb = f32[j] == 1 ? 4 : fb; collect(after, before[j], (size_t)n * sb, sb, out + (size_t)j * R * n); }
    }
    if (form != 0) {
      after.resize(field_b);
      HIPCHK(nc, hipMemcpy(after.data(), d_acc, field_b, hipMemcpyDeviceToHost));
      collect(after, acc_before, row_b, fb, out);
    }
    *sentinel_ok = ok;
    return 0;
  };
  const int rc = body();
  for (int j = 0; j < PF_MAX_JOBS; j++) { if (d_out[j] != d_in[j]) hipFree(d_out[j]); hipFree(d_in[j]); }
  hipFree(d_acc); hipFree(d_tw); hipFree(d_dc);
  return rc;
}

extern "C" int pf_debug_strided_xfuse(int field_bytes, int n, int njobs, const int *mul, int nouter, int ncols, int pre, double rs, double growth,
                                      int outer_offset, const double *in, double *out_fused, double *out_plain) {
  if (!in || !out_fused || !out_plain || !mul || njobs < 1 || njobs > PF_MAX_JOBS || nouter < 1 || ncols < 1 || (field_bytes != 8 && field_bytes != 4) ||
      outer_offset < 0 || outer_offset >= n)
    return pf_fail(0, "pf_debug_strided_xfuse: bad argument");
  if (!pf_strided_xfuse_supported(field_bytes, n)) return pf_fail(0, "pf_debug_strided_xfuse: no fused x-pass for lines of %d points in fields of %d bytes", n, field_bytes);
  const int fb = field_bytes, pc = (ncols + 15) & ~15;
  pf_ctx *nc = nullptr;
  const size_t nrows = (size_t)nouter * n, field = nrows * (size_t)pc * 2;
  void *d_in = nullptr, *d_mid = nullptr, *d_out = nullptr, *d_tw = nullptr; double *d_etab = nullptr;
  int dev = 0;
  if (hipGetDevice(&dev) != hipSuccess) return pf_fail(0, "pf_debug_strided_xfuse: no HIP device");
  std::vector<char> tw;
  host_twiddles(n, fb, tw);
  auto body = [&]() -> int {
    HIPCHK(nc, hipMalloc(&d_in, field * fb));
    HIPCHK(nc, hipMalloc(&d_mid, field * fb));
    HIPCHK(nc, hipMalloc(&d_out, (size_t)2 * njobs * field * fb));
    HIPCHK(nc, hipMalloc(&d_tw, tw.size()));
    HIPCHK(nc, hipMalloc((void **)&d_etab, (size_t)n * sizeof(double)));
    HIPCHK(nc, hipMemcpy(d_tw, tw.data(), tw.size(), hipMemcpyHostToDevice));
    HIPCHK(nc, hipMemset(d_in, 0, field * fb));
    HIPCHK(nc, hipMemset(d_mid, 0, field * fb));
    HIPCHK(nc, hipMemset(d_out, 0, (size_t)2 * njobs * field * fb));
    const size_t hrow = (size_t)ncols * 2 * fb, drow = (size_t)pc * 2 * fb, hfield = nrows * (size_t)ncols * 2;
    std::vector<float> hf;
    const void *src = in;
    if (fb == 4) { hf.resize(hfield); for (size_t k = 0; k < hfield; k++) hf[k] = (float)in[k]; src = hf.data(); }
    HIPCHK(nc, hipMemcpy2D(d_in, drow, src, hrow, hrow, nrows, hipMemcpyHostToDevice));
    PfStridedParams p; memset(&p, 0, sizeof(p));
    p.ain.os = (long long)n * pc; p.ain.el_shift = ilog2i(n); p.ain.el_len = n; p.ain.ehs = 0; p.ain.els = pc; p.aout = p.ain;
    p.ncols = ncols; p.nouter = nouter; p.tw = d_tw; p.etab = d_etab; p.band_e = p.band_outer = n; p.dev = dev; p.outer_offset = outer_offset;
    PfStridedParams q = p;
    q.njobs = njobs; q.pre = pre ? 1 : 0; q.rs = rs; q.growth = growth;
    if (pre && rs != 0.0) PFCHK0(pf_launch_exp_table(d_etab, n, rs, nullptr));
    for (int j = 0; j < njobs; j++) { q.job[j].in = d_in; q.job[j].out = (char *)d_out + (size_t)j * field * fb; q.job[j].mul = mul[j]; }
    PFCHK0(pf_launch_strided_xfuse(fb, n, q, nullptr));
    p.njobs = 1; p.job[0].in = d_in; p.job[0].out = d_mid; p.job[0].mul = PF_MUL_ONE; p.growth = 1.0;
    PFCHK0(pf_launch_strided(fb, n, -1, p, nullptr));
    for (int j = 0; j < njobs; j++) { q.job[j].in = d_mid; q.job[j].out = (char *)d_out + (size_t)(njobs + j) * field * fb; }
    PFCHK0(pf_launch_strided(fb, n, +1, q, nullptr));
    HIPCHK(nc, hipDeviceSynchronize());
    for (int j = 0; j < 2 * njobs; j++) {
      double *dst = (j < njobs ? out_fused : out_plain) + (size_t)(j % njobs) * hfield;
      const char *f = (const char *)d_out + (size_t)j * field * fb;
      if (fb == 8) HIPCHK(nc, hipMemcpy2D(dst, hrow, f, drow, hrow, nrows, hipMemcpyDeviceToHost));
      else {
        hf.resize(hfield);
        HIPCHK(nc, hipMemcpy2D(hf.data(), hrow, f, drow, hrow, nrows, hipMemcpyDeviceToHost));
        for (size_t k = 0; k < hfield; k++) dst[k] = (double)hf[k];
      }
    }
    return 0;
  };
  const int rc = body();
  hipFree(d_in); hipFree(d_mid); hipFree(d_out); hipFree(d_tw); hipFree(d_etab);
  return rc;
}

extern "C" int pf_ctx_set_rccl(pf_ctx *c, void *link) {
  if (!c) return 1;
  pf_rccl_release(c->rccl);
  c->rccl = link;
  return 0;
}
extern "C" int pf_release_rccl(pf_ctx *c) {
  if (!c) return 1;
  if (c->rccl) {
    hipStreamSynchronize(c->stream); hipStreamSynchronize(c->cstream);
    pf_rccl_release(c->rccl); c->rccl = nullptr;
    c->a2a = nullptr; c->a2av = nullptr; c->ared = nullptr; c->a2a_user = c->a2av_user = c->ared_user = nullptr;
  }
  return 0;
}
extern "C" int pf_rccl_comm_count(pf_ctx *c) {
  if (!c) return -1;
  return c->rccl ? pf_rccl_link_count(c->rccl) : 0;
}
extern "C" int pf_ctx_rank_size(pf_ctx *c, int *rank, int *nranks) {
  if (!c) return 1;
  *rank = c->rank; *nranks = c->P;
// ... 3 lines not shown
```

### pinocchio_amd/csrc/pf_fft_core.h

```cpp
#pragma once

#if defined(__HIPCC__)
#define PF_HD __host__ __device__ __forceinline__
#else
#define PF_HD inline
#endif
#include "pf_cxpk.h"
#ifndef PF_PK_F32
#define PF_PK_F32 1
#endif
#if defined(__HIP_DEVICE_COMPILE__) && PF_PK_F32
#define PF_PK_DEV 1
#else
#define PF_PK_DEV 0
#endif

template <typename F>
struct alignas(2 * sizeof(F)) pfc {
  F x, y;
};

template <typename F> PF_HD pfc<F> pf_mk(F x, F y) { pfc<F> r; r.x = x; r.y = y; return r; }
template <typename F> struct pf_is_f32 { static constexpr bool value = false; };
template <> struct pf_is_f32<float> { static constexpr bool value = true; };
// ... 20 lines not shown
  PF_IF_PK(F, PfCxPk::muli<DIR>(pf_pk(a)))
  return DIR > 0 ? pf_mk<F>(-a.y, a.x) : pf_mk<F>(a.y, -a.x);
}
template <int DIR, typename F> PF_HD pfc<F> pf_addi(pfc<F> a, pfc<F> b) { PF_IF_PK(F, PfCxPk::addi<DIR>(pf_pk(a), pf_pk(b))) return a + pf_mul_i<DIR>(b); }
template <int DIR, typename F> PF_HD pfc<F> pf_subi(pfc<F> a, pfc<F> b) { PF_IF_PK(F, PfCxPk::subi<DIR>(pf_pk(a), pf_pk(b))) return a - pf_mul_i<DIR>(b); }
template <typename F> PF_HD pfc<F> pf_addc(pfc<F> a, pfc<F> b) { PF_IF_PK(F, PfCxPk::addc(pf_pk(a), pf_pk(b))) return a + pf_conj(b); }
template <typename F> PF_HD pfc<F> pf_subc(pfc<F> a, pfc<F> b) { PF_IF_PK(F, PfCxPk::subc(pf_pk(a), pf_pk(b))) return a - pf_conj(b); }

#if defined(__HIPCC__)
typedef float pf_f32x2 __attribute__((ext_vector_type(2)));
#endif
template <typename F> struct pf_lane { typedef F type; static constexpr int n = 1; };
#if defined(__HIPCC__)
template <> struct pf_lane<pf_f32x2> { typedef float type; static constexpr int n = 2; };
#endif
template <typename F> PF_HD pfc<F> pf_bcast(pfc<typename pf_lane<F>::type> a) { return pf_mk<F>((F)a.x, (F)a.y); }
template <typename F> PF_HD pfc<F> pf_zero() { return pf_mk<F>((F)0, (F)0); }

#ifndef PF_NT
#define PF_NT 1
#endif
#if defined(__HIPCC__)
template <typename F> struct pf_vec2 { typedef F type __attribute__((ext_vector_type(2))); };
template <typename F> __device__ __forceinline__ pfc<F> pf_ld_stream(const pfc<F> *p) {
#if PF_NT
  const typename pf_vec2<F>::type v = __builtin_nontemporal_load(reinterpret_cast<const typename pf_vec2<F>::type *>(p));
  return pf_mk<F>(v.x, v.y);
#else
  return *p;
#endif
}
template <typename F> __device__ __forceinline__ void pf_st_stream(pfc<F> *p, pfc<F> v) {
#if PF_NT
  typename pf_vec2<F>::type t;
  t.x = v.x; t.y = v.y;
  __builtin_nontemporal_store(t, reinterpret_cast<typename pf_vec2<F>::type *>(p));
#else
  *p = v;
#endif
}
#endif

constexpr int pf_ilog2(int n) { return n <= 1 ? 0 : 1 + pf_ilog2(n >> 1); }
constexpr bool pf_pair16_length(int n) { return n >= 128 && pf_ilog2(n) % 3 == 1; }
constexpr int pf_nstages(int n, bool p16 = false) { return p16 ? (pf_ilog2(n) - 4) / 3 + 1 : (pf_ilog2(n) + 2) / 3; }
constexpr int pf_radix(int n, int s, bool p16 = false) {
  return p16 ? (s == 0 ? 16 : 8) : (s < pf_ilog2(n) / 3 ? 8 : (1 << (pf_ilog2(n) - 3 * (pf_ilog2(n) / 3))));
}
constexpr int pf_ns(int n, int s, bool p16 = false) { return s == 0 ? 1 : pf_ns(n, s - 1, p16) * pf_radix(n, s - 1, p16); }
template <int N, bool P16 = false> PF_HD int pf_line_index(int tl, int m) {
  return P16 ? (tl >> 1) + (N / 16) * (tl & 1) + m * (N / 8) : tl + m * (N / 8);
}

template <int DIR, typename F> PF_HD void pf_bfly2(pfc<F> &a, pfc<F> &b) {
  pfc<F> t = a - b;
  a = a + b;
  b = t;
}
template <int DIR, typename F> PF_HD void pf_bfly4(pfc<F> &v0, pfc<F> &v1, pfc<F> &v2, pfc<F> &v3) {
  pfc<F> a = v0 + v2, b = v0 - v2, c = v1 + v3, d = v1 - v3;
  v0 = a + c;
  v1 = pf_addi<DIR>(b, d);
  v2 = a - c;
  v3 = pf_subi<DIR>(b, d);
}
template <int DIR, typename F> PF_HD void pf_bfly8(pfc<F> (&u)[8]) {
  pf_bfly4<DIR>(u[0], u[2], u[4], u[6]);
  pf_bfly4<DIR>(u[1], u[3], u[5], u[7]);
  const F h = (F)0.70710678118654752440;
  pfc<F> o1, o3;
#if PF_PK_DEV
  if constexpr (pf_is_f32<F>::value) {
    o1 = pf_unpk<F>(PfCxPk::cmulc<DIR>(pf_pk(u[3]), 0.70710678118654752440, 0.70710678118654752440));
    o3 = pf_unpk<F>(PfCxPk::cmulc<DIR>(pf_pk(u[7]), -0.70710678118654752440, 0.70710678118654752440));
  } else
#endif
  {
    o1 = DIR > 0 ? pf_mk<F>(h * (u[3].x - u[3].y), h * (u[3].y + u[3].x))
                 : pf_mk<F>(h * (u[3].x + u[3].y), h * (u[3].y - u[3].x));
    o3 = DIR > 0 ? pf_mk<F>(h * (-u[7].x - u[7].y), h * (-u[7].y + u[7].x))
                 : pf_mk<F>(h * (-u[7].x + u[7].y), h * (-u[7].y - u[7].x));
  }
  pfc<F> e0 = u[0], e1 = u[2], e2 = u[4], e3 = u[6], o0 = u[1], o2 = u[5];
  u[0] = e0 + o0; u[4] = e0 - o0;
  u[1] = e1 + o1; u[5] = e1 - o1;
  u[2] = pf_addi<DIR>(e2, o2); u[6] = pf_subi<DIR>(e2, o2);
  u[3] = e3 + o3; u[7] = e3 - o3;
}

template <int N, int S, bool P16 = false> PF_HD int pf_stage_pos(int tl, int m) {
  if (P16 && S == 0) return 16 * (tl >> 1) + 8 * (tl & 1) + m;
  constexpr int R = (P16 && S == 0) ? 8 : pf_radix(N, S, P16), NS = pf_ns(N, S, P16), Q = 8 / R, NT = N / 8;
  const int q = m % Q, t = m / Q;
  const int jb = tl + q * NT;
  const int k = jb & (NS - 1);
  return (jb - k) * R + k + t * NS;
}

constexpr int pf_stage_ntw(int n, int s, bool p16 = false) { return pf_ns(n, s, p16) > 1 ? 8 / pf_radix(n, s, p16) : 0; }
constexpr int pf_ntw_before(int n, int s, bool p16 = false) { return s == 0 ? 0 : pf_ntw_before(n, s - 1, p16) + pf_stage_ntw(n, s - 1, p16); }
constexpr int pf_ntw_total(int n, bool p16 = false) { return pf_ntw_before(n, pf_nstages(n, p16), p16); }

template <typename F, int N, int S, int DIR, int TWS, int OFF = 0, bool P16 = false, int NW>
PF_HD void pf_stage_twiddles(int tl, const pfc<typename pf_lane<F>::type> *__restrict__ tw, pfc<F> (&w)[NW]) {
  constexpr int R = pf_radix(N, S, P16), NS = pf_ns(N, S, P16), Q = 8 / R, NT = N / 8;
  constexpr int TWM = (N / (NS * R)) * TWS;
  if (NS > 1) {
#pragma unroll
    for (int q = 0; q < Q; q++) {
      const int jb = tl + q * NT;
      const int k = jb & (NS - 1);
      w[OFF + q] = pf_bcast<F>(tw[k * TWM]);
      if (DIR < 0) w[OFF + q].y = -w[OFF + q].y;
    }
  }
}

template <typename F, int N, int S, int DIR, int OFF = 0, bool P16 = false, int NW>
PF_HD void pf_stage_apply(pfc<F> (&v)[8], const pfc<F> (&w)[NW]) {
  constexpr int R = pf_radix(N, S, P16), NS = pf_ns(N, S, P16), Q = 8 / R;
#pragma unroll
  for (int q = 0; q < Q; q++) {
    if (NS > 1) {
      const pfc<F> w1 = w[OFF + q];
      v[q + 1 * Q] = pf_cmul(v[q + 1 * Q], w1);
      if (R >= 4) {
        const pfc<F> w2 = pf_cmul(w1, w1), w3 = pf_cmul(w2, w1);
        v[q + 2 * Q] = pf_cmul(v[q + 2 * Q], w2);
        v[q + 3 * Q] = pf_cmul(v[q + 3 * Q], w3);
        if (R == 8) {
          const pfc<F> w4 = pf_cmul(w2, w2), w5 = pf_cmul(w4, w1), w6 = pf_cmul(w3, w3), w7 = pf_cmul(w4, w3);
          v[q + 4 * Q] = pf_cmul(v[q + 4 * Q], w4);
          v[q + 5 * Q] = pf_cmul(v[q + 5 * Q], w5);
          v[q + 6 * Q] = pf_cmul(v[q + 6 * Q], w6);
          v[q + 7 * Q] = pf_cmul(v[q + 7 * Q], w7);
        }
      }
    }
    if (R == 8) {
      pf_bfly8<DIR>(v);
    } else if (R == 4) {
      pf_bfly4<DIR>(v[q], v[q + Q], v[q + 2 * Q], v[q + 3 * Q]);
    } else if (R == 2) {
      pf_bfly2<DIR>(v[q], v[q + Q]);
    }
  }
}

template <typename F, int N, int S, int DIR, int TWS>
PF_HD void pf_stage(pfc<F> (&v)[8], int tl, const pfc<typename pf_lane<F>::type> *__restrict__ tw) {
  pfc<F> w[8 / pf_radix(N, S)];
  pf_stage_twiddles<F, N, S, DIR, TWS>(tl, tw, w);
  pf_stage_apply<F, N, S, DIR>(v, w);
}

template <int DIR, typename F> PF_HD void pf_pair16_local(pfc<F> (&v)[8], int tl) {
  pf_bfly8<DIR>(v);
  if (tl & 1) {
    const F c1 = (F)0.92387953251128675613, s1 = (F)0.38268343236508977173, h = (F)0.70710678118654752440;
    v[1] = DIR > 0 ? pf_mk<F>(c1 * v[1].x - s1 * v[1].y, c1 * v[1].y + s1 * v[1].x) : pf_mk<F>(c1 * v[1].x + s1 * v[1].y, c1 * v[1].y - s1 * v[1].x);
    v[2] = DIR > 0 ? pf_mk<F>(h * (v[2].x - v[2].y), h * (v[2].y + v[2].x)) : pf_mk<F>(h * (v[2].x + v[2].y), h * (v[2].y - v[2].x));
    v[3] = DIR > 0 ? pf_mk<F>(s1 * v[3].x - c1 * v[3].y, s1 * v[3].y + c1 * v[3].x) : pf_mk<F>(s1 * v[3].x + c1 * v[3].y, s1 * v[3].y - c1 * v[3].x);
    v[4] = pf_mul_i<DIR>(v[4]);
    v[5] = DIR > 0 ? pf_mk<F>(-s1 * v[5].x - c1 * v[5].y, -s1 * v[5].y + c1 * v[5].x) : pf_mk<F>(-s1 * v[5].x + c1 * v[5].y, -s1 * v[5].y - c1 * v[5].x);
    v[6] = DIR > 0 ? pf_mk<F>(h * (-v[6].x - v[6].y), h * (-v[6].y + v[6].x)) : pf_mk<F>(h * (-v[6].x + v[6].y), h * (-v[6].y - v[6].x));
    v[7] = DIR > 0 ? pf_mk<F>(-c1 * v[7].x - s1 * v[7].y, -c1 * v[7].y + s1 * v[7].x) : pf_mk<F>(-c1 * v[7].x + s1 * v[7].y, -c1 * v[7].y - s1 * v[7].x);
  }
}
template <typename F> PF_HD pfc<F> pf_pair16_combine1(pfc<F> v, pfc<F> o, F sgn) { return pf_mk<F>(o.x + sgn * v.x, o.y + sgn * v.y); }
template <typename F> PF_HD void pf_pair16_combine(pfc<F> (&v)[8], const pfc<F> (&o)[8], int tl) {
  const F sgn = (tl & 1) ? (F)-1 : (F)1;
#if defined(__HIP_DEVICE_COMPILE__)
#pragma unroll
#endif
  for (int m = 0; m < 8; m++) v[m] = pf_pair16_combine1(v[m], o[m], sgn);
}

PF_HD int pf_lpad(int p) { return p + (p >> 3); }

template <typename F> PF_HD pfc<F> pf_c2r_pre(pfc<F> xk, pfc<F> xmk, pfc<F> wk , bool k0) {
  if (k0) {
    return pf_mk<F>(xk.x + xmk.x, xk.x - xmk.x);
  }
  pfc<F> s = pf_addc(xk, xmk), d = pf_cmul(pf_subc(xk, xmk), wk);
  return pf_addi<+1>(s, d);
}
template <typename F> PF_HD pfc<F> pf_r2c_post(pfc<F> zk, pfc<F> zmk, pfc<F> wk ) {
  pfc<F> e = pf_scale(pf_addc(zk, zmk), (F)0.5);
  pfc<F> d = pf_scale(pf_subc(zk, zmk), (F)0.5);
#if PF_PK_DEV
  if constexpr (pf_is_f32<F>::value) return pf_subi<+1>(e, pf_cmulc(d, wk));
#endif
  pfc<F> o = pf_mk<F>(d.y, -d.x);
  return e + pf_cmul(o, pf_conj(wk));
}
```

### pinocchio_amd/csrc/pf_fft_kernels.hip

```cpp
#include <atomic>
#include <cstdio>

#include "pf_internal.h"
#include "pf_fft_core.h"

#include "pf_fft_stages.h"
#include "pf_fft16.h"
#include "pf_strided_addr.h"
#include "pf_collapse_core.h"

#ifndef PF_SLAB_STORE
#define PF_SLAB_STORE 1
#endif
template <typename F> struct PfCols {
  using S = F;
  static constexpr int n = 1;
  static __device__ __forceinline__ pfc<F> load(const pfc<S> *base, long long off) { return pf_ld_stream(base + off); }
  static __device__ __forceinline__ void store(pfc<S> *base, long long off, pfc<F> v, bool) { pf_st_stream(base + off, v); }
  static __device__ __forceinline__ pfc<F> load_ul(const pfc<S> *base, long long u, unsigned lane) {
    return pf_ld_stream(reinterpret_cast<const pfc<S> *>(reinterpret_cast<const char *>(base + u) + (size_t)(lane * (unsigned)sizeof(pfc<S>))));
  }
  static __device__ __forceinline__ void store_ul(pfc<S> *base, long long u, unsigned lane, pfc<F> v, bool) {
    pf_st_stream(reinterpret_cast<pfc<S> *>(reinterpret_cast<char *>(base + u) + (size_t)(lane * (unsigned)sizeof(pfc<S>))), v);
  }
};
template <> struct PfCols<pf_f32x2> {
  using S = float;
  static constexpr int n = 2;
  typedef float f4 __attribute__((ext_vector_type(4)));
  static __device__ __forceinline__ pfc<pf_f32x2> load(const pfc<float> *base, long long off) {
#if PF_NT
    const f4 t = __builtin_nontemporal_load(reinterpret_cast<const f4 *>(base + off));
#else
    const f4 t = *reinterpret_cast<const f4 *>(base + off);
#endif
    pfc<pf_f32x2> r;
    r.x = (pf_f32x2){t.x, t.z}; r.y = (pf_f32x2){t.y, t.w};
    return r;
  }
  static __device__ __forceinline__ void store(pfc<float> *base, long long off, pfc<pf_f32x2> v, bool v1) {
    if (v1) {
      const f4 t = (f4){v.x.x, v.y.x, v.x.y, v.y.y};
#if PF_NT
      __builtin_nontemporal_store(t, reinterpret_cast<f4 *>(base + off));
#else
      *reinterpret_cast<f4 *>(base + off) = t;
#endif
    } else {
      pf_st_stream(base + off, pf_mk<float>(v.x.x, v.y.x));
    }
  }
  static __device__ __forceinline__ pfc<pf_f32x2> load_ul(const pfc<float> *base, long long u, unsigned lane) {
    return load(reinterpret_cast<const pfc<float> *>(reinterpret_cast<const char *>(base + u) + (size_t)(lane * (unsigned)sizeof(pfc<float>))), 0);
  }
  static __device__ __forceinline__ void store_ul(pfc<float> *base, long long u, unsigned lane, pfc<pf_f32x2> v, bool v1) {
    store(reinterpret_cast<pfc<float> *>(reinterpret_cast<char *>(base + u) + (size_t)(lane * (unsigned)sizeof(pfc<float>))), 0, v, v1);
  }
};

constexpr int PF_DIR_XF = 2;
template <typename F, int N, int T, int DIRS, bool FA>
__global__ void __launch_bounds__(T *N / 8) __attribute__((amdgpu_waves_per_eu(4))) k_strided(const PfStridedParams p, const long long nwork, const int ntiles) {
  constexpr bool XF = DIRS == PF_DIR_XF;
  constexpr int DIR = XF ? +1 : DIRS;
  using C = pfc<F>;
  using COLS = PfCols<F>;
  using S = typename COLS::S;
  constexpr int NL = COLS::n;
  constexpr int NT = N / 8;
#ifndef PF_PAIR16
#define PF_PAIR16 1
#endif
  constexpr bool P16 = PF_PAIR16 && pf_pair16_length(N) && T == 8;
  extern __shared__ __attribute__((aligned(16))) char smem[];
  C *lds = reinterpret_cast<C *>(smem);
  const long long w = pf_xcd_swizzle(blockIdx.x, (nwork + 7) >> 3);
  if (w >= nwork) return;
  const int tid = threadIdx.x;
  const int c = tid % T, tl = tid / T;
  const int tile = (int)(w % ntiles);
  const int outer = (int)(w / ntiles);
  const int col = NL * (tile * T + c);
  const bool valid = col < p.ncols, valid1 = NL > 1 && col + 1 < p.ncols;
  const pfc<S> *__restrict__ tw = reinterpret_cast<const pfc<S> *>(p.tw);
  const double kf = 2.0 * 3.14159265358979323846 / (double)N;
  if (p.band_outer < N / 2) {
    int so = outer + p.outer_offset;
    if (so > N / 2) so -= N;
    if (so > p.band_outer || so < -p.band_outer) return;
  }

  C src[8], v[8];
  auto load_tile = [&](const void *inp, int tlj, int colj) {
    const pfc<S> *__restrict__ in = reinterpret_cast<const pfc<S> *>(inp);
#pragma unroll
    for (int m = 0; m < 8; m++) {
      const int e = pf_line_index<N, P16>(tlj, m);
      const int se = e > N / 2 ? e - N : e;
      const bool inband = se <= p.band_e && se >= -p.band_e;
      if constexpr (FA) src[m] = (valid && inband) ? COLS::load_ul(in, pf_addr_uniform<NT>(p.ain, outer, m, NL * tile * T), pf_addr_lane(p.ain, pf_line_index<N, P16>(tlj, 0), colj - NL * tile * T)) : pf_zero<F>();
      else src[m] = (valid && inband) ? COLS::load(in, pf_addr(p.ain, outer, e, colj)) : pf_zero<F>();
      if constexpr (NL > 1) { if (!valid1) { src[m].x.y = 0.f; src[m].y.y = 0.f; } }
    }
  };
  load_tile(p.job[0].in, tl, col);
  if constexpr (XF) {
    PfStages<F, N, -1, 1, 0, false, P16>::run(
        src, tl, tw, [&](int pos, C val) { lds[pos * T + c] = val; }, [&](int pos) { return lds[pos * T + c]; });
    if constexpr (P16) {
#pragma unroll
      for (int m = 0; m < 8; m++) lds[(tl + m * NT) * T + c] = src[m];
      __syncthreads();
#pragma unroll
      for (int m = 0; m < 8; m++) src[m] = lds[pf_line_index<N, P16>(tl, m) * T + c];
      __syncthreads();
    }
  }
  double ko = 0.0, woc[NL];
#pragma unroll
  for (int l = 0; l < NL; l++) woc[l] = 1.0;
  if (p.pre) {
    int so = outer + p.outer_offset;
    if (so > N / 2) so -= N;
    ko = kf * so;
#pragma unroll
    for (int l = 0; l < NL; l++) {
      const double kc = kf * (col + l);
      const double ko2kc2 = ko * ko + kc * kc;
      woc[l] = (p.rs != 0.0 ? exp(-0.5 * ko2kc2 * p.rs * p.rs) : 1.0) * p.growth;
    }
  }
#pragma unroll 1
  for (int j = 0; j < p.njobs; j++) {
    int tlj = tl, cj = c;
    asm volatile("" : "+v"(tlj), "+v"(cj));
    const int colj = NL * (tile * T + cj);
    if (p.pre && (j == 0 || p.job[j].in != p.job[j - 1].in)) {
      double we[8];
      if (p.rs != 0.0) {
#pragma unroll
        for (int m = 0; m < 8; m++) we[m] = p.etab[pf_line_index<N, P16>(tlj, m)];
      } else {
#pragma unroll
        for (int m = 0; m < 8; m++) we[m] = 1.0;
      }
#pragma unroll
      for (int l = 0; l < NL; l++) {
        const double kc = kf * (colj + l);
        const double ko2kc2 = ko * ko + kc * kc;
#pragma unroll
        for (int m = 0; m < 8; m++) {
          const int e = pf_line_index<N, P16>(tlj, m);
          const double ke = kf * (e > N / 2 ? e - N : e);
          const double k2 = ke * ke + ko2kc2;
          const S fac = (S)((k2 != 0.0) ? pf_div_fast(we[m] * woc[l], k2) : 0.0);
          if constexpr (NL > 1) { src[m].x[l] = src[m].x[l] * fac; src[m].y[l] = src[m].y[l] * fac; }
          else src[m] = pf_scale(src[m], (F)fac);
        }
      }
    }
    const int mul = p.job[j].mul;
#pragma unroll
    for (int m = 0; m < 8; m++) {
      const int e = pf_line_index<N, P16>(tlj, m);
      const F ke = (F)(S)(kf * (e > N / 2 ? e - N : e));
      C x = src[m];
      if (mul == PF_MUL_K) x = pf_scale(x, ke);
      else if (mul == PF_MUL_K2) x = pf_scale(x, ke * ke);
      else if (mul == PF_MUL_IK) x = pf_mul_i<+1>(pf_scale(x, ke));
      v[m] = x;
    }
    if (j + 1 < p.njobs && p.job[j + 1].in != p.job[j].in) load_tile(p.job[j + 1].in, tlj, colj);
    PfStages<F, N, DIR, 1, 0, false, P16>::run(
        v, tlj, tw, [&](int pos, C val) { lds[pos * T + cj] = val; }, [&](int pos) { return lds[pos * T + cj]; });
#if defined(PF_DUMMY_VALU) && PF_DUMMY_VALU > 0
    if constexpr (NL == 1) {
      double a = (double)v[0].x;
      for (int i = 0; i < PF_DUMMY_VALU; i++) a = __builtin_fma(a, 1.0000001, 1e-30);
      v[0].x = (F)a;
    }
#endif
    if (valid) {
      pfc<S> *__restrict__ out = reinterpret_cast<pfc<S> *>(p.job[j].out);
      if (PF_SLAB_STORE && p.out_ne > 0) {
#pragma unroll
        for (int m = 0; m < 8; m++) {
          const int e = tlj + m * NT;
          if ((unsigned)(e - p.out_e0) < (unsigned)p.out_ne) COLS::store(out, pf_addr(p.aout, outer, e, colj), v[m], valid1);
        }
      } else if constexpr (FA) {
        const unsigned lane = pf_addr_lane(p.aout, tlj, colj - NL * tile * T);
#pragma unroll
        for (int m = 0; m < 8; m++) COLS::store_ul(out, pf_addr_uniform<NT>(p.aout, outer, m, NL * tile * T), lane, v[m], valid1);
      } else {
#pragma unroll
        for (int m = 0; m < 8; m++) {
          const int e = tlj + m * NT;
          COLS::store(out, pf_addr(p.aout, outer, e, colj), v[m], valid1);
        }
      }
    }
  }
}

template <typename F, int N, int TL>
__global__ void __launch_bounds__(TL *(N / 16)) k_c2r(const PfC2RParams p) {
  using C = pfc<F>;
  constexpr int M = N / 2, NT = M / 8;
  constexpr int LPL = (M + 1 > M + M / 8) ? M + 1 : M + M / 8;
  constexpr int NTHR = TL * NT;
  extern __shared__ __attribute__((aligned(16))) char smem[];
  C *lds = reinterpret_cast<C *>(smem);
  const int tid = threadIdx.x;
  const int l = tid / NT, tl = tid % NT;
  const int job = blockIdx.x % p.njobs;
  const long long line0 = (long long)(blockIdx.x / p.njobs) * TL;
  const C *__restrict__ in = reinterpret_cast<const C *>(p.job[job].in);
  const int mul = p.job[job].mul;
  const C *__restrict__ tw = reinterpret_cast<const C *>(p.tw);

  for (int idx = tid; idx < TL * (M + 1); idx += NTHR) {
    const int ll = idx / (M + 1), k = idx % (M + 1);
    const long long row = line0 + ll;
    lds[ll * LPL + k] = (row < p.nlines && k <= p.band_k) ? in[row * p.in_pitch + k] : pf_mk<F>(0, 0);
  }
  __syncthreads();

  C *L = lds + l * LPL;
  const F kf = (F)(2.0 * 3.14159265358979323846 / (double)N);
  C v[8];
#pragma unroll
  for (int m = 0; m < 8; m++) {
    const int e = tl + m * NT;
    v[m] = pf_zfold<F>(L[e], L[M - e], e, M, mul, kf, tw[e], m == 0);
  }
  __syncthreads();

  PfStages<F, M, +1, 2>::run(
      v, tl, tw, [&](int pos, C val) { L[pf_lpad(pos)] = val; }, [&](int pos) { return L[pf_lpad(pos)]; });

  const long long row = line0 + l;
  if (row < p.nlines) {
    const F norm = (F)p.norm;
    const F dcv = p.dc ? (F)(*p.dc) : (F)0;
    if (p.job[job].out_f32 == 1) {
      float2 *o = reinterpret_cast<float2 *>(reinterpret_cast<float *>(p.job[job].out) + row * (long long)N);
#pragma unroll
      for (int m = 0; m < 8; m++) {
        const int n2 = tl + m * NT;
        o[n2] = make_float2((float)pf_norm_dc(v[m].x, norm, dcv), (float)pf_norm_dc(v[m].y, norm, dcv));
      }
    } else {
      C *o = reinterpret_cast<C *>(reinterpret_cast<F *>(p.job[job].out) + row * (p.job[job].out_f32 == 2 ? (long long)N : p.out_pitch));
#pragma unroll
      for (int m = 0; m < 8; m++) {
        const int n2 = tl + m * NT;
// ... 50 lines not shown
    C *L = lds + lj * LPL;
    C v[8];
#pragma unroll
    for (int m = 0; m < 8; m++) {
      const int e = tlj + m * NT;
      v[m] = pf_zfold<F>(L[e], L[M - e], e, M, mul, kf, tw[e], m == 0);
    }
    if (NT <= 64) pf_wave_sync(); else __syncthreads();
    if (t + gridDim.x < ntiles) fetch(t + gridDim.x);
    PfStages<F, M, +1, 2, 0, (NT <= 64)>::run(
        v, tlj, tw, [&](int pos, C val) { L[pf_lpad(pos)] = val; }, [&](int pos) { return L[pf_lpad(pos)]; });
    const long long row = (t / p.njobs) * TL + lj;
    if (row < p.nlines) {
      if (p.job[job].out_f32 == 1) {
        float2 *o = reinterpret_cast<float2 *>(reinterpret_cast<float *>(p.job[job].out) + row * (long long)N);
#pragma unroll
        for (int m = 0; m < 8; m++)
          pf_st_stream(reinterpret_cast<pfc<float> *>(&o[tlj + m * NT]), pf_mk<float>((float)pf_norm_dc(v[m].x, norm, dcv), (float)pf_norm_dc(v[m].y, norm, dcv)));
      } else {
        C *o = reinterpret_cast<C *>(reinterpret_cast<F *>(p.job[job].out) + row * (p.job[job].out_f32 == 2 ? (long long)N : p.out_pitch));
#pragma unroll
        for (int m = 0; m < 8; m++) pf_st_stream(&o[tlj + m * NT], pf_norm_dc2(v[m], norm, dcv));
      }
    }
    if (NT <= 64 || pf_nstages(M) == 1) __syncthreads();
  }
}

#ifndef PF_ZI_PREFETCH
#define PF_ZI_PREFETCH -1
#endif
#ifndef PF_ZI_WAVES
#define PF_ZI_WAVES 0
#endif
#define PF_ZI_PRAGMA_(x) _Pragma(#x)
#define PF_ZI_PRAGMA(x) PF_ZI_PRAGMA_(x)
#ifndef PF_ZI_SPEC_F32
#define PF_ZI_SPEC_F32 1
#endif
#ifndef PF_ZI_SPEC_512
#define PF_ZI_SPEC_512 1
#endif
#ifndef PF_ZI_SPEC_2048
#define PF_ZI_SPEC_2048 1
#endif
#ifndef PF_ZI_SPEC_LPT
#define PF_ZI_SPEC_LPT 0
#endif
#ifndef PF_ZI_RUNROLL
#define PF_ZI_RUNROLL 1
#endif
#ifndef PF_ZI_LATE
#define PF_ZI_LATE 0
#endif
#ifndef PF_ZI_SPEC
#define PF_ZI_SPEC 1
#endif
#ifndef PF_ZI_UNIFORM_MUL
#define PF_ZI_UNIFORM_MUL(F) (sizeof(F) == 4)
#endif
#ifndef PF_ZFOLD_K0_ALL
#define PF_ZFOLD_K0_ALL(F) (sizeof(F) == 8)
#endif
#ifndef PF_ZI_ROT
#define PF_ZI_ROT 2
#endif
#ifndef PF_ZI_OWN
#define PF_ZI_OWN 1
#endif
#ifndef PF_ZI_DMA
#define PF_ZI_DMA 0
#endif
template <typename F, int M> struct PfZiPlan {
  static constexpr bool lean = PF_ZI_PREFETCH < 0 ? (sizeof(F) == 8 && M >= 256) : PF_ZI_PREFETCH == 0;
  static constexpr int full = (M + 1 > M + M / 8) ? M + 1 : M + M / 8, narrow = (M + 1 > M + M / 16) ? M + 1 : M + M / 16;
  static constexpr int line = (lean && M >= 256) ? narrow : full;
  static __device__ __forceinline__ int pad(int p) { return (lean && M >= 256) ? p + (p >> 4) : pf_lpad(p); }
  static constexpr bool spec0 = PF_ZI_SPEC && !PF_ZI_DMA &&
                                (((M == 512 || (M == 256 && PF_ZI_SPEC_512)) && (lean || (PF_ZI_SPEC_F32 && sizeof(F) == 4))) ||
                                 (M == 1024 && sizeof(F) == 4 && PF_ZI_SPEC_2048));
  static constexpr bool spec(int mode) { return spec0 && (mode == 0 || PF_ZI_SPEC_LPT); }
  static constexpr int reducer_waves = M / 256;
};
template <typename F, int N, int MODE, bool SPEC>
__device__ __forceinline__ void pf_c2r_invariants_body(const PfC2RParams &p, long long nrows) {
  using C = pfc<F>;
  using F2 = typename pf_vec2<F>::type;
  constexpr bool IN_PLACE = sizeof(F) == 8;
  constexpr int M = N / 2, NT = M / 8, TL = 6;
  using PLAN = PfZiPlan<F, M>;
  constexpr int LPL = PLAN::line;
  constexpr bool DMA = PF_ZI_DMA && PLAN::lean && NT == 64 && sizeof(C) == 16;
  constexpr bool PREFETCH = !PLAN::lean && !SPEC;
  constexpr bool LATE = PF_ZI_LATE && PLAN::lean && !SPEC && !DMA && MODE == 0;
  constexpr int NTHR = TL * NT;
  static_assert((size_t)LPL * sizeof(C) >= (size_t)N * sizeof(F), "a line's LDS holds its real row");
  extern __shared__ __attribute__((aligned(16))) char smem[];
  C *lds = reinterpret_cast<C *>(smem);
  const int tid = threadIdx.x;
  const int lw = tid / NT, tl = tid % NT;
  const bool reducer = SPEC && lw >= TL;
  const int l = reducer ? 0 : (lw + PF_ZI_ROT) % TL;
  const C *__restrict__ tw = reinterpret_cast<const C *>(p.tw);
  const F kf = (F)(2.0 * 3.14159265358979323846 / (double)N);
  const F norm = (F)p.norm;
  const F dcv = p.dc ? (F)(*p.dc) : (F)0;
  const C *in = reinterpret_cast<const C *>(p.job[0].in);
  int mul = p.job[0].mul;
#pragma unroll
  for (int j = 1; j < TL; j++)
    if (l == j) { in = reinterpret_cast<const C *>(p.job[j].in); mul = p.job[j].mul; }
  if constexpr (NT >= 64 && PF_ZI_UNIFORM_MUL(F)) mul = __builtin_amdgcn_readfirstlane(mul);
  double *__restrict__ o1 = IN_PLACE ? reinterpret_cast<double *>(p.job[0].out) : p.inv_out[0],
         *__restrict__ o2 = IN_PLACE ? reinterpret_cast<double *>(p.job[1].out) : p.inv_out[1],
         *__restrict__ o3 = IN_PLACE ? reinterpret_cast<double *>(p.job[2].out) : p.inv_out[2];

  auto line_sync = [&]() { if (NT > 64) __syncthreads(); else pf_wave_sync(); };
  C nxt[9];
  auto fetch = [&](long long R) {
    const C *__restrict__ row = in + R * p.in_pitch;
#pragma unroll
    for (int m = 0; m < 8; m++) {
      const int k = tl + m * NT;
      nxt[m] = (k <= p.band_k) ? pf_ld_stream(&row[k]) : pf_mk<F>(0, 0);
    }
    nxt[8] = (tl == 0 && M <= p.band_k) ? pf_ld_stream(&row[M]) : pf_mk<F>(0, 0);
  };

  auto reduce_row = [&](long long R, int c0, int cstep) {
PF_ZI_PRAGMA(unroll PF_ZI_RUNROLL)
    for (int c = c0; c < N; c += cstep) {
      F2 h[6];
#pragma unroll
      for (int k = 0; k < 6; k++) h[k] = *reinterpret_cast<const F2 *>(reinterpret_cast<const F *>(lds + k * LPL) + c);
      const double da[6] = {(double)h[0].x, (double)h[1].x, (double)h[2].x, (double)h[3].x, (double)h[4].x, (double)h[5].x},
                   db[6] = {(double)h[0].y, (double)h[1].y, (double)h[2].y, (double)h[3].y, (double)h[4].y, (double)h[5].y};
      const long long a = R * p.out_pitch + c;
      if (MODE == 0) {
        double a1, a2, a3, b1, b2, b3;
        pf_invariants(da, a1, a2, a3);
        pf_invariants(db, b1, b2, b3);
        if (pf_invariants_lose_diagonal(da, a1, a2) || pf_invariants_lose_diagonal(db, b1, b2)) *p.flag = 1.0;
        const long long ao = IN_PLACE ? a : R * p.inv_pitch + c;
#if PF_NT
        typedef double pf_d2 __attribute__((ext_vector_type(2)));
        pf_d2 w1, w2, w3;
        w1.x = a1; w1.y = b1; w2.x = a2; w2.y = b2; w3.x = a3; w3.y = b3;
        __builtin_nontemporal_store(w1, reinterpret_cast<pf_d2 *>(o1 + ao));
        __builtin_nontemporal_store(w2, reinterpret_cast<pf_d2 *>(o2 + ao));
        __builtin_nontemporal_store(w3, reinterpret_cast<pf_d2 *>(o3 + ao));
#else
        *reinterpret_cast<double2 *>(o1 + ao) = make_double2(a1, b1);
        *reinterpret_cast<double2 *>(o2 + ao) = make_double2(a2, b2);
        *reinterpret_cast<double2 *>(o3 + ao) = make_double2(a3, b3);
#endif
      } else {
        double ha[6], hb[6];
#pragma unroll
        for (int k = 0; k < 6; k++) {
          const F2 g = *reinterpret_cast<const F2 *>(reinterpret_cast<const F *>(p.job[k].out) + a);
          ha[k] = (double)g.x; hb[k] = (double)g.y;
        }
        F2 *acc = reinterpret_cast<F2 *>(reinterpret_cast<F *>(p.acc) + a);
        F2 s;
        if constexpr (MODE == 2) {
          double s2, s31, sa, sb;
          pf_lpt_sources_cell(ha, s2, s31, sa);
          pf_lpt_sources_cell(hb, s2, s31, sb);
          s.x = (F)sa; s.y = (F)sb;
        } else s = *acc;
        F2 r;
        r.x = (F)pf_lpt3b_accumulate((double)s.x, da, ha);
        r.y = (F)pf_lpt3b_accumulate((double)s.y, db, hb);
        *acc = r;
      }
    }
  };
  if (SPEC && reducer) {
    constexpr int LINE_BARRIERS = NT > 64 ? 3 + 2 * (pf_nstages(M) - 1) : 0;
#pragma unroll 1
    for (long long Rr = blockIdx.x; Rr < nrows; Rr += gridDim.x) {
      int tr = tid - TL * NT;
      asm volatile("" : "+v"(tr));
#pragma unroll
      for (int i = 0; i < LINE_BARRIERS; i++) __syncthreads();
      __syncthreads();
      reduce_row(Rr, 2 * tr, 2 * 64 * PLAN::reducer_waves);
      __syncthreads();
    }
    return;
  }
  long long R = blockIdx.x;
  if ((PREFETCH || SPEC || LATE) && R < nrows) fetch(R);
#pragma unroll 1
  for (; R < nrows; R += gridDim.x) {
    int tlj = tl, lj = l, tidj = tid;
    asm volatile("" : "+v"(tlj), "+v"(lj), "+v"(tidj));
    C *L = lds + lj * LPL;
    if (DMA) {
      const C *__restrict__ row = in + R * p.in_pitch;
      const unsigned lbase = (unsigned)__builtin_amdgcn_readfirstlane((int)(unsigned)(size_t)(__attribute__((address_space(3))) char *)(lds + (tid / NT) * LPL));
#pragma unroll
      for (int m = 0; m < 8; m++) {
        const int k = tlj + m * NT;
        if (m * NT + NT - 1 <= p.band_k)
          __builtin_amdgcn_global_load_lds((const __attribute__((address_space(1))) void *)(&row[k]),
                                           (__attribute__((address_space(3))) void *)(size_t)(lbase + m * NT * (unsigned)sizeof(C)), 16, 0, PF_NT ? 2 : 0);
        else
          L[k] = (k <= p.band_k) ? pf_ld_stream(&row[k]) : pf_mk<F>(0, 0);
      }
      if (tlj == 0) L[M] = (M <= p.band_k) ? pf_ld_stream(&row[M]) : pf_mk<F>(0, 0);
      __builtin_amdgcn_s_waitcnt(0x0f70);
    } else {
      if (!PREFETCH && !SPEC && !LATE) fetch(R);
#pragma unroll
      for (int m = 0; m < 8; m++) L[tlj + m * NT] = nxt[m];
      if (tlj == 0) L[M] = nxt[8];
    }
    line_sync();
    C v[8];
#pragma unroll
    for (int m = 0; m < 8; m++) {
      const int e = tlj + m * NT;
      v[m] = pf_zfold<F>((PF_ZI_OWN && !PREFETCH && !DMA) ? nxt[m] : L[e], L[M - e], e, M, mul, kf, tw[e], m == 0 || PF_ZFOLD_K0_ALL(F));
    }
    line_sync();
    if (PREFETCH && R + gridDim.x < nrows) fetch(R + gridDim.x);
#ifndef PF_ZI_HOIST_TW
#define PF_ZI_HOIST_TW 0
#endif
    PfStages<F, M, +1, 2, 0, (NT <= 64)>::run(
        v, tlj, tw, [&](int pos, C val) { L[PLAN::pad(pos)] = val; }, [&](int pos) { return L[PLAN::pad(pos)]; }, PF_ZI_HOIST_TW ? tl : -1);
    line_sync();
    C *H = L;
#pragma unroll
    for (int m = 0; m < 8; m++) H[tlj + m * NT] = pf_norm_dc2(v[m], norm, dcv);
    __syncthreads();
    if (SPEC || LATE) {
      if (R + gridDim.x < nrows) fetch(R + gridDim.x);
      else {
#pragma unroll
        for (int m = 0; m < 9; m++) nxt[m] = pf_mk<F>(0, 0);
      }
    }
    if (!SPEC) reduce_row(R, 2 * tidj, 2 * NTHR);
    __syncthreads();
  }
}
template <typename F, int N, int MODE = 0>
__global__ void __launch_bounds__(6 * (N / 16))
#if PF_ZI_WAVES > 0
__attribute__((amdgpu_waves_per_eu(PF_ZI_WAVES, PF_ZI_WAVES)))
#endif
k_c2r_invariants(const PfC2RParams p, long long nrows) { pf_c2r_invariants_body<F, N, MODE, false>(p, nrows); }
template <typename F, int N, int MODE = 0>
__global__ void __launch_bounds__(6 * (N / 16) + 64 * (N / 512)) __attribute__((amdgpu_waves_per_eu(N >= 2048 ? 8 : 6)))
k_c2r_invariants_spec(const PfC2RParams p, long long nrows) { pf_c2r_invariants_body<F, N, MODE, true>(p, nrows); }

#ifndef PF_ZI_PK2
#define PF_ZI_PK2 1
#endif
#ifndef PF_ZI_PK2_MAXN
#define PF_ZI_PK2_MAXN 1024
#endif
struct alignas(16) PfRow2 { pf_f2 a, b; };

template <int M, int S, int NW>
__device__ __forceinline__ void pf_pk2_stage(pf_f2 (&a)[8], pf_f2 (&b)[8], const pf_f2 (&w)[NW]) {
  using A = PfCxPk;
  constexpr int R = pf_radix(M, S), NS = pf_ns(M, S), Q = 8 / R;
#pragma unroll
  for (int q = 0; q < Q; q++) {
    if constexpr (NS > 1) {
      const pf_f2 w1 = w[q];
      a[q + Q] = A::cmul<+1>(a[q + Q], w1); b[q + Q] = A::cmul<+1>(b[q + Q], w1);
      if constexpr (R >= 4) {
        const pf_f2 w2 = A::twmul(w1, w1), w3 = A::twmul(w2, w1);
        a[q + 2 * Q] = A::cmul<+1>(a[q + 2 * Q], w2); b[q + 2 * Q] = A::cmul<+1>(b[q + 2 * Q], w2);
        a[q + 3 * Q] = A::cmul<+1>(a[q + 3 * Q], w3); b[q + 3 * Q] = A::cmul<+1>(b[q + 3 * Q], w3);
        if constexpr (R == 8) {
          const pf_f2 w4 = A::twmul(w2, w2), w5 = A::twmul(w4, w1), w6 = A::twmul(w3, w3), w7 = A::twmul(w4, w3);
          a[4] = A::cmul<+1>(a[4], w4); b[4] = A::cmul<+1>(b[4], w4);
          a[5] = A::cmul<+1>(a[5], w5); b[5] = A::cmul<+1>(b[5], w5);
          a[6] = A::cmul<+1>(a[6], w6); b[6] = A::cmul<+1>(b[6], w6);
          a[7] = A::cmul<+1>(a[7], w7); b[7] = A::cmul<+1>(b[7], w7);
        }
      }
    }
    if constexpr (R == 8) { pfx_bfly8<A, +1>(a); pfx_bfly8<A, +1>(b); }
    else if constexpr (R == 4) {
      pfx_bfly4<A, +1>(a[q], a[q + Q], a[q + 2 * Q], a[q + 3 * Q]);
      pfx_bfly4<A, +1>(b[q], b[q + Q], b[q + 2 * Q], b[q + 3 * Q]);
    } else {
      const pf_f2 ta = A::sub(a[q], a[q + Q]), tb = A::sub(b[q], b[q + Q]);
      a[q] = A::add(a[q], a[q + Q]); b[q] = A::add(b[q], b[q + Q]);
      a[q + Q] = ta; b[q + Q] = tb;
    }
  }
}
template <int M, int S, bool WAVE_LOCAL>
struct PfPk2Stages {
  template <typename WR, typename RD>
  static __device__ __forceinline__ void run(pf_f2 (&a)[8], pf_f2 (&b)[8], int tl, const pf_f2 *__restrict__ tw, WR wr, RD rd) {
    constexpr int NT = M / 8;
    if constexpr (S == 0) {
      const pf_f2 none[1] = {PfCxPk::mk(1.f, 0.f)};
      pf_pk2_stage<M, 0>(a, b, none);
    }
    if constexpr (S + 1 < pf_nstages(M)) {
      constexpr int R1 = pf_radix(M, S + 1), NS1 = pf_ns(M, S + 1), Q1 = 8 / R1;
      constexpr int TWM1 = (M / (NS1 * R1)) * 2;
      pf_f2 w[Q1];
#pragma unroll
      for (int q = 0; q < Q1; q++) w[q] = tw[((tl + q * NT) & (NS1 - 1)) * TWM1];
#pragma unroll
      for (int m = 0; m < 8; m++) wr(pf_stage_pos<M, S>(tl, m), a[m], b[m]);
      if constexpr (WAVE_LOCAL) pf_wave_sync(); else __syncthreads();
#pragma unroll
      for (int m = 0; m < 8; m++) rd(tl + m * NT, a[m], b[m]);
      if constexpr (WAVE_LOCAL) pf_wave_sync(); else __syncthreads();
      pf_pk2_stage<M, S + 1>(a, b, w);
      PfPk2Stages<M, S + 1, WAVE_LOCAL>::run(a, b, tl, tw, wr, rd);
    }
  }
};

template <int N, int RW>
__global__ void __launch_bounds__(6 * (N / 16) + 64 * RW) k_c2r_invariants_pk2(const PfC2RParams p, long long nrows) {
  using A = PfCxPk;
  constexpr int M = N / 2, NT = M / 8, TL = 6;
  constexpr int LPL = M + M / 16 + 1;
  constexpr bool WAVE_LOCAL = NT <= 64;
  constexpr int NSTAGES = pf_nstages(M);
  extern __shared__ __attribute__((aligned(16))) char smem[];
  PfRow2 *lds = reinterpret_cast<PfRow2 *>(smem);
  const int tid = threadIdx.x;
  const long long npairs = (nrows + 1) >> 1;
  double *__restrict__ o1 = p.inv_out[0], *__restrict__ o2 = p.inv_out[1], *__restrict__ o3 = p.inv_out[2];
  if (tid >= TL * NT) {
    constexpr int LINE_BARRIERS = WAVE_LOCAL ? 0 : 3 + 2 * (NSTAGES - 1);
// ... 92 lines not shown
      const int e = tlj + m * NT;
      const PfRow2 mk = L[M - e];
      pf_f2 xa = na[m], xb = nb[m], ya = mk.a, yb = mk.b;
      if (mul != 0 ) {
        float fk = kf * (float)e, fm = kf * (float)(M - e);
        if (mul == 2 ) { fk *= fk; fm *= fm; }
        xa = A::scale(xa, fk); xb = A::scale(xb, fk); ya = A::scale(ya, fm); yb = A::scale(yb, fm);
      }
      if (m == 0 && e == 0) {
        a[m] = A::mk(xa.x + ya.x, xa.x - ya.x);
        b[m] = A::mk(xb.x + yb.x, xb.x - yb.x);
      } else {
        const pf_f2 wk = tw[e];
        a[m] = A::addi<+1>(A::addc(xa, ya), A::cmul<+1>(A::subc(xa, ya), wk));
        b[m] = A::addi<+1>(A::addc(xb, yb), A::cmul<+1>(A::subc(xb, yb), wk));
      }
    }
    line_sync();
    PfPk2Stages<M, 0, WAVE_LOCAL>::run(
        a, b, tlj, tw, [&](int pos, pf_f2 va, pf_f2 vb) { PfRow2 e; e.a = va; e.b = vb; L[pos + (pos >> 4)] = e; },
        [&](int pos, pf_f2 &va, pf_f2 &vb) { const PfRow2 e = L[pos + (pos >> 4)]; va = e.a; vb = e.b; });
    line_sync();
#pragma unroll
    for (int m = 0; m < 8; m++) { PfRow2 e; e.a = A::fma1(a[m], norm, dcv); e.b = A::fma1(b[m], norm, dcv); L[tlj + m * NT] = e; }
    __syncthreads();
    if (q + gridDim.x < npairs) fetch(q + gridDim.x);
    else {
#pragma unroll
      for (int m = 0; m < 9; m++) { na[m] = zero; nb[m] = zero; }
    }
    __syncthreads();
  }
}

template <typename F, int N, int TL>
__global__ void __launch_bounds__(TL *(N / 16)) k_r2c(const PfR2CParams p) {
  using C = pfc<F>;
  constexpr int M = N / 2, NT = M / 8;
  constexpr int LPL = M + M / 8;
  extern __shared__ __attribute__((aligned(16))) char smem[];
  C *lds = reinterpret_cast<C *>(smem);
  const int tid = threadIdx.x;
  const int l = tid / NT, tl = tid % NT;
  const long long row = (long long)blockIdx.x * TL + l;
  const bool valid = row < p.nlines;
  const C *__restrict__ tw = reinterpret_cast<const C *>(p.tw);
  C *L = lds + l * LPL;

  C v[8];
  {
    const C *in = reinterpret_cast<const C *>(reinterpret_cast<const F *>(p.in) + row * p.in_pitch);
#pragma unroll
    for (int m = 0; m < 8; m++) v[m] = valid ? pf_ld_stream(&in[tl + m * NT]) : pf_mk<F>(0, 0);
  }
  PfStages<F, M, -1, 2>::run(
      v, tl, tw, [&](int pos, C val) { L[pf_lpad(pos)] = val; }, [&](int pos) { return L[pf_lpad(pos)]; });
#pragma unroll
  for (int m = 0; m < 8; m++) L[pf_lpad(tl + m * NT)] = v[m];
  __syncthreads();
  if (valid) {
    C *out = reinterpret_cast<C *>(p.out) + row * p.out_pitch;
#pragma unroll
    for (int m = 0; m < 8; m++) {
      const int k = tl + m * NT;
      const C zk = v[m], zmk = L[pf_lpad((M - k) & (M - 1))];
      pf_st_stream(&out[k], pf_r2c_post<F>(zk, zmk, tw[k]));
      if (k == 0) out[M] = pf_mk<F>(zk.x - zk.y, (F)0);
    }
  }
}

__global__ void k_exp_table(double *etab, int n, double rs) {
  const int e = blockIdx.x * blockDim.x + threadIdx.x;
  if (e >= n) return;
  const double ke = 2.0 * 3.14159265358979323846 / (double)n * (e > n / 2 ? e - n : e);
  etab[e] = exp(-0.5 * ke * ke * rs * rs);
}
int pf_launch_exp_table(double *etab, int n, double rs, hipStream_t st) {
  hipLaunchKernelGGL(k_exp_table, dim3((n + 255) / 256), dim3(256), 0, st, etab, n, rs);
  return hipGetLastError() == hipSuccess ? 0 : 1;
}


template <typename F, int N> struct PfTileCols {
#ifndef PF_TILE_LDS_KB
#define PF_TILE_LDS_KB 128
#endif
  static constexpr int lds_budget = PF_TILE_LDS_KB * 1024;
  static constexpr int t0 = 128 / (2 * (int)sizeof(F));
  static constexpr int fit = lds_budget / (N * 2 * (int)sizeof(F));
  static constexpr int thr = 8192 / N;
  static constexpr int a = t0 < fit ? t0 : fit;
  static constexpr int b = a < thr ? a : thr;
  static constexpr int value = b < 1 ? 1 : b;
};

template <typename F, int N, int DIR, bool FA>
static int launch_strided_v(const PfStridedParams &p, hipStream_t st, int ntiles, long long nwork) {
  constexpr int T = PfTileCols<F, N>::value;
  dim3 grid((unsigned)(((nwork + 7) >> 3) << 3), 1, 1), block(T * N / 8, 1, 1);
  const size_t shm = (size_t)N * T * sizeof(pfc<F>);
  if (shm > 64 * 1024) {
    static std::atomic<bool> raised[PF_MAX_DEVICES];
    const int d = p.dev >= 0 && p.dev < PF_MAX_DEVICES ? p.dev : 0;
    if (!raised[d].load(std::memory_order_acquire)) {
      if (hipFuncSetAttribute(reinterpret_cast<const void *>(&k_strided<F, N, T, DIR, FA>), hipFuncAttributeMaxDynamicSharedMemorySize, (int)shm) != hipSuccess) {
        fprintf(stderr, "ERROR on task 0: hipFuncSetAttribute(MaxDynamicSharedMemorySize = %zu) refused for the %d-point strided pass on device %d\n", shm, N, d);
        return 3;
      }
      raised[d].store(true, std::memory_order_release);
    }
  }
  hipLaunchKernelGGL((k_strided<F, N, T, DIR, FA>), grid, block, shm, st, p, nwork, ntiles);
  return hipGetLastError() == hipSuccess ? 0 : 1;
}
template <typename F, int N, int DIR>
static int launch_strided_n(const PfStridedParams &p, hipStream_t st) {
  constexpr int T = PfTileCols<F, N>::value;
  constexpr int NL = pf_lane<F>::n;
  constexpr int NT = N / 8;
  using S = typename pf_lane<F>::type;
  const int ntiles = (p.ncols + NL * T - 1) / (NL * T);
  const long long nwork = (long long)ntiles * p.nouter;
  auto lane_fits = [&](const PfAddr &a) {
    return (1 << a.el_shift) >= NT && a.els > 0 && ((unsigned long long)(NT - 1) * (unsigned long long)a.els + (unsigned long long)(NL * T)) * sizeof(pfc<S>) < (1ull << 32);
  };
  if (lane_fits(p.ain) && lane_fits(p.aout)) return launch_strided_v<F, N, DIR, true>(p, st, ntiles, nwork);
  return launch_strided_v<F, N, DIR, false>(p, st, ntiles, nwork);
}
#ifndef PF_F32_PAIRS
#define PF_F32_PAIRS 1
#endif
template <int N, int DIR>
static int launch_strided_f32(const PfStridedParams &p, hipStream_t st) {
  if constexpr (N == 2048 || N == 1024) {
    const int rc = pf_launch_strided16(4, N, DIR, p, st);
    if (rc >= 0) return rc;
  }
  if constexpr (PF_F32_PAIRS && N >= 1024) return launch_strided_n<pf_f32x2, N, DIR>(p, st);
  else return launch_strided_n<float, N, DIR>(p, st);
}

template <int N>
static int launch_strided_xf_f32(const PfStridedParams &p, hipStream_t st) {
  if constexpr (N < 1024) return launch_strided_n<float, N, PF_DIR_XF>(p, st);
  else return 2;
}

template <typename F, int N>
static int launch_c2r_n(const PfC2RParams &p, hipStream_t st) {
  constexpr int M = N / 2, NT = M / 8;
  constexpr int TL = (NT >= 256) ? 1 : 256 / NT;
  constexpr int LPL = (M + 1 > M + M / 8) ? M + 1 : M + M / 8;
  const long long nblk = (p.nlines + TL - 1) / TL;
  dim3 grid((unsigned)(nblk * p.njobs), 1, 1), block(TL * NT, 1, 1);
  const size_t shm = (size_t)TL * LPL * sizeof(pfc<F>);
  const int persist = p.persist_per_cu;
  if (persist > 0 && N >= 64 && p.ncu > 0) {
    const long long ntiles = nblk * p.njobs;
    long long g = (long long)p.ncu * persist;
    if (g > ntiles) g = ntiles;
    hipLaunchKernelGGL((k_c2r_persistent<F, N, TL>), dim3((unsigned)g), block, shm, st, p, ntiles);
    return hipGetLastError() == hipSuccess ? 0 : 1;
  }
  hipLaunchKernelGGL((k_c2r<F, N, TL>), grid, block, shm, st, p);
  return hipGetLastError() == hipSuccess ? 0 : 1;
}

template <typename F, int N>
static int launch_c2r_invariants_n(const PfC2RParams &p, hipStream_t st, int mode) {
  constexpr int M = N / 2, NT = M / 8;
  constexpr int LPL = PfZiPlan<F, M>::line;
  long long g = (long long)(p.ncu > 0 ? p.ncu : 256) * (p.inv_per_cu > 0 ? p.inv_per_cu : 32);
  if (g > p.nlines) g = p.nlines;
  const size_t shm = (size_t)6 * LPL * sizeof(pfc<F>);
  if (mode == 1) {
    if constexpr (PfZiPlan<F, M>::spec(1)) hipLaunchKernelGGL((k_c2r_invariants_spec<F, N, 1>), dim3((unsigned)g), dim3(6 * NT + 64 * PfZiPlan<F, M>::reducer_waves), shm, st, p, p.nlines);
    else hipLaunchKernelGGL((k_c2r_invariants<F, N, 1>), dim3((unsigned)g), dim3(6 * NT), shm, st, p, p.nlines);
  } else if (mode == 2) {
    if constexpr (PfZiPlan<F, M>::spec(1)) hipLaunchKernelGGL((k_c2r_invariants_spec<F, N, 2>), dim3((unsigned)g), dim3(6 * NT + 64 * PfZiPlan<F, M>::reducer_waves), shm, st, p, p.nlines);
    else hipLaunchKernelGGL((k_c2r_invariants<F, N, 2>), dim3((unsigned)g), dim3(6 * NT), shm, st, p, p.nlines);
  } else if constexpr (PF_ZI_PK2 && sizeof(F) == 4 && N >= 512 && N <= PF_ZI_PK2_MAXN) {
    for (int j = 0; j < 6; j++) if (p.job[j].mul == PF_MUL_IK) return 2;
    constexpr int RW = N >= 2048 ? 4 : (N >= 1024 ? 2 : 1);
    constexpr int LPL2 = M + M / 16 + 1;
    const size_t shm2 = (size_t)6 * LPL2 * sizeof(PfRow2);
    const int threads = 6 * NT + 64 * RW;
    static std::atomic<bool> raised2[PF_MAX_DEVICES];
    if (shm2 > 64 * 1024 && p.dev >= 0 && p.dev < PF_MAX_DEVICES && !raised2[p.dev].load(std::memory_order_acquire)) {
      if (hipFuncSetAttribute(reinterpret_cast<const void *>(&k_c2r_invariants_pk2<N, RW>), hipFuncAttributeMaxDynamicSharedMemorySize, (int)shm2) != hipSuccess) return 3;
      raised2[p.dev].store(true, std::memory_order_release);
    }
    long long g2 = g;
    const long long npairs = (p.nlines + 1) / 2;
    if (g2 > npairs) g2 = npairs;
    hipLaunchKernelGGL((k_c2r_invariants_pk2<N, RW>), dim3((unsigned)g2), dim3(threads), shm2, st, p, p.nlines);
  } else if constexpr (PfZiPlan<F, M>::spec(0)) hipLaunchKernelGGL((k_c2r_invariants_spec<F, N, 0>), dim3((unsigned)g), dim3(6 * NT + 64 * PfZiPlan<F, M>::reducer_waves), shm, st, p, p.nlines);
  else hipLaunchKernelGGL((k_c2r_invariants<F, N, 0>), dim3((unsigned)g), dim3(6 * NT), shm, st, p, p.nlines);
  return hipGetLastError() == hipSuccess ? 0 : 1;
}

template <typename F, int N>
static int launch_r2c_n(const PfR2CParams &p, hipStream_t st) {
  constexpr int M = N / 2, NT = M / 8;
  constexpr int TL = (NT >= 256) ? 1 : 256 / NT;
  constexpr int LPL = M + M / 8;
  const long long nblk = (p.nlines + TL - 1) / TL;
  dim3 grid((unsigned)nblk, 1, 1), block(TL * NT, 1, 1);
  const size_t shm = (size_t)TL * LPL * sizeof(pfc<F>);
  hipLaunchKernelGGL((k_r2c<F, N, TL>), grid, block, shm, st, p);
  return hipGetLastError() == hipSuccess ? 0 : 1;
}

#define PF_SWITCH_N(n, CALL)                  \
  switch (n) {                                \
    case 16: return CALL(16);                 \
    case 32: return CALL(32);                 \
    case 64: return CALL(64);                 \
    case 128: return CALL(128);               \
    case 256: return CALL(256);               \
    case 512: return CALL(512);               \
    case 1024: return CALL(1024);             \
    case 2048: return CALL(2048);             \
    default: return 2;                        \
  }

int pf_launch_strided(int fb, int n, int dir, const PfStridedParams &p, hipStream_t st) {
  if (n & (n - 1)) return pf_launch_mixed_strided(fb, n, dir, p, st);
  if (fb == 8) {
    if (dir > 0) {
#define CALL(NN) launch_strided_n<double, NN, +1>(p, st)
      PF_SWITCH_N(n, CALL)
#undef CALL
    } else {
#define CALL(NN) launch_strided_n<double, NN, -1>(p, st)
      PF_SWITCH_N(n, CALL)
#undef CALL
    }
  } else {
    if (dir > 0) {
#define CALL(NN) launch_strided_f32<NN, +1>(p, st)
      PF_SWITCH_N(n, CALL)
#undef CALL
    } else {
#define CALL(NN) launch_strided_f32<NN, -1>(p, st)
      PF_SWITCH_N(n, CALL)
#undef CALL
    }
  }
}

bool pf_strided_xfuse_supported(int fb, int n) { return !(n & (n - 1)) && n >= 16 && n <= 2048 && (fb == 8 || n < 1024); }
int pf_launch_strided_xfuse(int fb, int n, const PfStridedParams &p, hipStream_t st) {
  if (!pf_strided_xfuse_supported(fb, n) || p.njobs < 1 || p.band_e < n / 2 || p.band_outer < n / 2 || p.out_ne > 0) return 2;
  for (int j = 1; j < p.njobs; j++) if (p.job[j].in != p.job[0].in) return 2;
  for (int j = 0; j < p.njobs; j++) if (p.job[j].out == p.job[0].in) return 2;
  if (fb == 8) {
#define CALL(NN) launch_strided_n<double, NN, PF_DIR_XF>(p, st)
    PF_SWITCH_N(n, CALL)
#undef CALL
  } else {
#define CALL(NN) launch_strided_xf_f32<NN>(p, st)
    PF_SWITCH_N(n, CALL)
#undef CALL
  }
}

int pf_launch_c2r(int fb, int n, const PfC2RParams &p, hipStream_t st) {
  if (n & (n - 1)) return pf_launch_mixed_c2r(fb, n, p, st);
  if (fb == 8) {
#define CALL(NN) launch_c2r_n<double, NN>(p, st)
    PF_SWITCH_N(n, CALL)
#undef CALL
  } else {
#define CALL(NN) launch_c2r_n<float, NN>(p, st)
    PF_SWITCH_N(n, CALL)
#undef CALL
  }
}

bool pf_c2r_invariants_supported(int fb, int n) {
// ... 35 lines not shown
```

### pinocchio_amd/csrc/pf_fft_stages.h

```cpp
#pragma once
#include "pf_fft_core.h"

__device__ __forceinline__ void pf_wave_sync() {
  __builtin_amdgcn_fence(__ATOMIC_RELEASE, "wavefront");
  __builtin_amdgcn_wave_barrier();
  __builtin_amdgcn_fence(__ATOMIC_ACQUIRE, "wavefront");
}

__device__ __forceinline__ int pf_lane_xor8(int x) { return __builtin_amdgcn_update_dpp(0, x, 0x128 , 0xf, 0xf, false); }
__device__ __forceinline__ double pf_lane_xor8(double x) {
  return __hiloint2double(pf_lane_xor8(__double2hiint(x)), pf_lane_xor8(__double2loint(x)));
}
__device__ __forceinline__ float pf_lane_xor8(float x) { return __int_as_float(pf_lane_xor8(__float_as_int(x))); }
__device__ __forceinline__ pf_f32x2 pf_lane_xor8(pf_f32x2 x) { pf_f32x2 r; r.x = pf_lane_xor8(x.x); r.y = pf_lane_xor8(x.y); return r; }
template <typename F> __device__ __forceinline__ pfc<F> pf_lane_xor8(pfc<F> a) { return pf_mk<F>(pf_lane_xor8(a.x), pf_lane_xor8(a.y)); }

template <typename F, int N, int DIR, int TWS, int S = 0, bool WAVE_LOCAL = false, bool P16 = false>
struct PfStages {
  template <typename WR, typename RD>
  static __device__ __forceinline__ void exchange(pfc<F> (&v)[8], int tl, WR wr, RD rd) {
    constexpr int NT = N / 8;
#pragma unroll
    for (int m = 0; m < 8; m++) wr(pf_stage_pos<N, S, P16>(tl, m), v[m]);
    if constexpr (WAVE_LOCAL) pf_wave_sync(); else __syncthreads();
#pragma unroll
    for (int m = 0; m < 8; m++) v[m] = rd(tl + m * NT);
    if constexpr (WAVE_LOCAL) pf_wave_sync(); else __syncthreads();
  }
  template <typename WR, typename RD>
  static __device__ __forceinline__ void run(pfc<F> (&v)[8], int tl, const pfc<typename pf_lane<F>::type> *__restrict__ tw, WR wr, RD rd, int tl_tw = -1) {
    static_assert(!WAVE_LOCAL || N / 8 <= 64, "a wave-local transform has at most 64 threads");
    const int tt = tl_tw < 0 ? tl : tl_tw;
    if constexpr (S == 0 && P16) {
      pf_pair16_local<DIR>(v, tl);
      typedef typename pf_lane<F>::type SC;
      const F sgn = (F)((tl & 1) ? (SC)-1 : (SC)1);
#pragma unroll
      for (int m = 0; m < 8; m++) v[m] = pf_pair16_combine1(v[m], pf_lane_xor8(v[m]), sgn);
    } else if constexpr (S == 0) pf_stage<F, N, 0, DIR, TWS>(v, tt, tw);
    if constexpr (S + 1 < pf_nstages(N, P16)) {
      pfc<F> w[8 / pf_radix(N, S + 1, P16)];
      pf_stage_twiddles<F, N, S + 1, DIR, TWS, 0, P16>(tt, tw, w);
      exchange(v, tl, wr, rd);
      pf_stage_apply<F, N, S + 1, DIR, 0, P16>(v, w);
      PfStages<F, N, DIR, TWS, S + 1, WAVE_LOCAL, P16>::run(v, tl, tw, wr, rd, tl_tw);
    }
  }
};

template <typename F> __device__ __forceinline__ F pf_norm_dc(F v, F norm, F dc) { return v * norm + dc; }
template <typename F> __device__ __forceinline__ pfc<F> pf_norm_dc2(pfc<F> v, F norm, F dc) {
#if PF_PK_DEV
  if constexpr (pf_is_f32<F>::value) return pf_unpk<F>(PfCxPk::fma1(pf_pk(v), (float)norm, (float)dc));
#endif
  return pf_mk<F>(pf_norm_dc(v.x, norm, dc), pf_norm_dc(v.y, norm, dc));
}

template <typename F>
__device__ __forceinline__ pfc<F> pf_zfold(pfc<F> xk, pfc<F> xmk, int e, int M, int mul, F kf, pfc<F> wk, bool maybe0 = true) {
  if (mul != 0 ) {
    F fk = kf * (F)e, fm = kf * (F)(M - e);
    if (mul == 2 ) { fk *= fk; fm *= fm; }
    xk = pf_scale(xk, fk);
    xmk = pf_scale(xmk, fm);
    if (mul == 3 ) { xk = pf_mul_i<+1>(xk); xmk = pf_mul_i<+1>(xmk); }
  }
  return pf_c2r_pre<F>(xk, xmk, wk, (maybe0 || sizeof(F) == 8) && e == 0);
}
```

### pinocchio_amd/csrc/pf_internal.h

```cpp
#pragma once
#include <hip/hip_runtime.h>
#include <stddef.h>
#include <stdint.h>

#include "../../include/pinfmax.h"

#define PF_MAX_JOBS 6
#define PF_MAX_DEVICES 64

struct PfTuning {
  int zpass_persist;
  int zpass_inv_wg_per_cu;
  int collapse_wg_per_cu;
  bool spline_lut, exchange_rows, general, pipeline, exact_libm;
  int invariants, lpt_fuse;
  int replicate;
  double prune_eps;
  int debug_fault;
  int solve_beside_z;
  int handoff_chunk_mb, handoff_threads;
  bool host_register;
  bool preflight;
  bool distribute_lds;
  bool gtab;
  bool lpt3b_start;
  bool lpt_xfuse;
};

enum { PF_MUL_ONE = 0, PF_MUL_K = 1, PF_MUL_K2 = 2, PF_MUL_IK = 3 };

struct PfAddr {
  long long os;
  int el_shift;
  long long ehs, els;
  int el_len;
};

struct PfStridedJob {
  const void *in;
  void *out;
  int mul;
};

struct PfStridedParams {
  int njobs;
  PfStridedJob job[PF_MAX_JOBS];
  PfAddr ain, aout;
  int ncols;
  int nouter;
  int pre;
  int outer_offset;
  double rs, growth;
  const double *etab;
  const void *tw;
  int band_e, band_outer;
  int dev;
  int out_e0, out_ne;
};

int pf_launch_strided(int field_bytes, int n, int dir, const PfStridedParams &p, hipStream_t st);
bool pf_strided_xfuse_supported(int field_bytes, int n);
int pf_launch_strided_xfuse(int field_bytes, int n, const PfStridedParams &p, hipStream_t st);
int pf_launch_exp_table(double *etab, int n, double rs, hipStream_t st);
int pf_launch_strided16(int field_bytes, int n, int dir, const PfStridedParams &p, hipStream_t st);

struct PfC2RJob {
  const void *in;
  void *out;
  int mul;
  int out_f32;
};

struct PfC2RParams {
  int njobs;
  PfC2RJob job[PF_MAX_JOBS];
  long long nlines;
  long long in_pitch;
  long long out_pitch;
  double norm;
  const double *dc;
  const void *tw;
  int band_k;
  void *acc;
  double *flag;
  int ncu, dev;
  int persist_per_cu;
  int inv_per_cu;
  double *inv_out[3];
  long long inv_pitch;
};
int pf_launch_c2r(int field_bytes, int n, const PfC2RParams &p, hipStream_t st);
int pf_launch_c2r_invariants(int field_bytes, int n, const PfC2RParams &p, hipStream_t st, int mode = 0);

struct PfR2CParams {
  const void *in;
  void *out;
  long long nlines, in_pitch, out_pitch;
  const void *tw;
};
int pf_launch_r2c(int field_bytes, int n, const PfR2CParams &p, hipStream_t st);

#define PF_MIXED_MAX_STAGES 12
struct PfMixedPlan { int n, nstages; int radix[PF_MIXED_MAX_STAGES]; unsigned magic[PF_MIXED_MAX_STAGES]; unsigned magic_in, magic_out;  };
bool pf_mixed_plan(int n, bool allow4, PfMixedPlan *pl);
bool pf_mixed_supported(int n);
int pf_launch_mixed_strided(int field_bytes, int n, int dir, const PfStridedParams &p, hipStream_t st);
int pf_launch_mixed_c2r(int field_bytes, int n, const PfC2RParams &p, hipStream_t st);
int pf_launch_mixed_r2c(int field_bytes, int n, const PfR2CParams &p, hipStream_t st);
bool pf_mixed_invariants_supported(int field_bytes, int n);
int pf_launch_mixed_c2r_invariants(int field_bytes, int n, const PfC2RParams &p, hipStream_t st, int mode);
bool pf_c2r_invariants_preferred(int field_bytes, int n);
bool pf_mixed_plan_compiled_in(int n);
bool pf_c2r_invariants_supported(int field_bytes, int n);

#define PF_KNOT_CAP 512
struct PfSplineDev {
  const double *x, *y, *c, *b, *d;
  int n;
  const double *gt;
  const unsigned short *gt_lut;
};
struct PfCtDev {
  double *delta, *y, *b, *c, *d;
  const double *alpha, *gamma;
  double ampl;
  int model;
  int flavour;
  double sng_cosmo[7], sng_Din;
};
struct PfCollapseParams {
  const void *h[6];
  long long pitch;
  long long nrows;
  int n;
  void *fmax;
  int prod_f64;
  int *rmax;
  int ismooth;
  PfSplineDev spline;
  double *partials;
  int nblocks;
  int fast;
  int no_lut;
  int invariants;
  int tabulated;
  int sng;
  int sources;
  void *src[3];
  double *src_partials;
  PfCtDev ct;
};
int pf_launch_ct_build(const PfSplineDev &sp, const PfCtDev &ct, int fast, int compute_table, hipStream_t st);
int pf_launch_collapse(int field_bytes, const PfCollapseParams &p, hipStream_t st);
int pf_launch_final_sum(const double *partials, int nblocks, double *out2, hipStream_t st);
int pf_launch_collapse_cells(const double *d, size_t count, PfSplineDev s, double *F, int fast, hipStream_t st);

struct PfLptSrcParams {
  const void *h[6];
  void *s2, *s3a, *s3b;
  long long pitch, nrows;
  int n;
  double *partials;
  int nblocks;
};
int pf_launch_lpt_sources(int field_bytes, const PfLptSrcParams &p, hipStream_t st);

struct PfLptAccParams {
  const void *h[6], *phi2[6];
  void *s3b;
  long long pitch, nrows;
  int n;
};
int pf_launch_lpt_accum(int field_bytes, const PfLptAccParams &p, hipStream_t st);

// ... 172 lines not shown
```

Measured before the change: 1.534 billion.

## Specialize FFT passes for band-limited zero registers to skip dead butterflies

```diff
diff --git a/include/pinfmax.h b/include/pinfmax.h
--- a/include/pinfmax.h
+++ b/include/pinfmax.h
@@ -246,6 +246,7 @@
 int pf_debug_zpass_jobs(int field_bytes, int n, int form, int njobs, const int *mul, const int *out_f32, int in_place, int nrows, int band,
                         double norm, const double *dc, int ncu, const double *spec, const double *hess, const double *acc, double *out,
                         int *sentinel_ok);
+int pf_debug_band_zero_class(int kind, int field_bytes, int n, int band, long long *launched);
 int pf_debug_strided_xfuse(int field_bytes, int n, int njobs, const int *mul, int nouter, int ncols, int pre, double rs, double growth,
                            int outer_offset, const double *in, double *out_fused, double *out_plain);
 int pf_debug_invariant_reruns(pf_ctx *ctx);
diff --git a/pinocchio_amd/_lib.py b/pinocchio_amd/_lib.py
--- a/pinocchio_amd/_lib.py
+++ b/pinocchio_amd/_lib.py
@@ -287,6 +287,7 @@
                                         C.c_int, C.c_int, C.c_int, C.c_int, C.c_double, C.c_double, _dp, _dp, C.POINTER(C.c_int)]),
     "pf_debug_zpass_jobs": (C.c_int, [C.c_int, C.c_int, C.c_int, C.c_int, C.POINTER(C.c_int), C.POINTER(C.c_int), C.c_int, C.c_int, C.c_int, C.c_double,
                                       _dp, C.c_int, _dp, _dp, _dp, _dp, C.POINTER(C.c_int)]),
+    "pf_debug_band_zero_class": (C.c_int, [C.c_int, C.c_int, C.c_int, C.c_int, C.POINTER(C.c_longlong)]),
     "pf_debug_strided_xfuse": (C.c_int, [C.c_int, C.c_int, C.c_int, C.POINTER(C.c_int), C.c_int, C.c_int, C.c_int, C.c_double, C.c_double, C.c_int,
                                          _dp, _dp, _dp]),
     "pf_debug_invariant_reruns": (C.c_int, [_vp]),
diff --git a/pinocchio_amd/csrc/pf_api.hip b/pinocchio_amd/csrc/pf_api.hip
--- a/pinocchio_amd/csrc/pf_api.hip
+++ b/pinocchio_amd/csrc/pf_api.hip
@@ -287,6 +287,7 @@
   t->solve_beside_z = env_int("PF_SOLVE_BESIDE_Z", -1);
   t->gtab = env_int("PF_GTAB", 1) != 0;
   t->lpt_xfuse = env_int("PF_LPT_XFUSE", 1) != 0;
+  t->band_zero = env_int("PF_BAND_ZERO", 1) != 0;
   t->lpt3b_start = env_int("PF_LPT3B_START", 0) != 0;
   t->preflight = env_int("PF_PREFLIGHT", 1) != 0;
   t->handoff_chunk_mb = env_int("PF_HANDOFF_CHUNK_MB", 256);
@@ -720,7 +721,7 @@
   p.ain = p.aout = addr_ky_x(c);
   if (out_yblocks) p.aout = addr_yblocks_x(c, band_zpitch(c, band));
   p.ncols = c->nzh; p.nouter = c->nyl; p.pre = pre; p.outer_offset = c->rank * c->nyl; p.rs = rs; p.growth = growth; p.tw = c->tw;
-  p.etab = c->etab; p.dev = c->dev;
+  p.etab = c->etab; p.dev = c->dev; p.band_zero = c->tune.band_zero && c->P == 1;
   if (replicated) {
     p.ain = addr_full_x(c); p.aout = addr_local_x(c, band_zpitch(c, band));
     p.nouter = c->n; p.outer_offset = 0; p.out_e0 = c->rank * c->nxl; p.out_ne = c->nxl;
@@ -750,7 +751,7 @@
   p.ain = in_blocks ? (in_yblocks ? addr_yblocks_y(c, band_zpitch(c, band)) : addr_blocks_y(c)) : addr_xs_y(c);
   if (in_local) p.ain = addr_local_y(c, band_zpitch(c, band));
   p.aout = out_blocks ? addr_blocks_y(c) : addr_xs_y(c);
-  p.ncols = c->nzh; p.nouter = c->nxl; p.pre = 0; p.outer_offset = 0; p.rs = 0; p.growth = 1; p.tw = c->tw; p.dev = c->dev;
+  p.ncols = c->nzh; p.nouter = c->nxl; p.pre = 0; p.outer_offset = 0; p.rs = 0; p.growth = 1; p.tw = c->tw; p.dev = c->dev; p.band_zero = c->tune.band_zero && c->P == 1;
   p.band_e = p.band_outer = c->n;
   double frac_cols = 1.0, frac_in = 1.0;
   if (band < c->n / 2) {
@@ -778,6 +779,7 @@
   double frac_in = 1.0;
   if (band < c->n / 2) { p.band_k = band; frac_in = (double)(band + 1) / c->nzh; }
   p.ncu = c->ncu; p.dev = c->dev; p.persist_per_cu = c->tune.zpass_persist; p.inv_per_cu = c->tune.zpass_inv_wg_per_cu;
+  p.band_zero = c->tune.band_zero && c->P == 1;
   p.flag = c->scal + SC_INV_FLAG;
   if (acc) {
     p.acc = acc;
@@ -2578,7 +2580,7 @@
       p.njobs = 1; p.job[0].in = d_in; p.job[0].out = d_out; p.job[0].mul = mul;
       p.ain.os = (long long)n * pc; p.ain.el_shift = ilog2i(n); p.ain.el_len = n; p.ain.ehs = 0; p.ain.els = pc; p.aout = p.ain;
       p.ncols = ncols; p.nouter = nouter; p.pre = pre; p.outer_offset = outer_offset; p.rs = rs; p.growth = growth; p.tw = d_tw; p.etab = d_etab;
-      p.band_e = p.band_outer = n; p.dev = dev;
+      p.band_e = p.band_outer = n; p.dev = dev; p.band_zero = tune.band_zero;
       if (band < n / 2) p.band_e = band;
       if (pre && rs != 0.0) PFCHK0(pf_launch_exp_table(d_etab, n, rs, nullptr));
       PFCHK0(pf_launch_strided(fb, n, pass == 0 ? +1 : -1, p, nullptr));
@@ -2594,7 +2596,7 @@
       }
       p.nlines = nouter; p.in_pitch = nzh; p.out_pitch = n; p.norm = 1.0; p.dc = nullptr; p.tw = d_tw; p.band_k = band < n / 2 ? band : n;
       p.ncu = ncu; p.dev = dev; p.persist_per_cu = tune.zpass_persist; p.inv_per_cu = tune.zpass_inv_wg_per_cu; p.flag = d_flag;
-      p.inv_pitch = n;
+      p.inv_pitch = n; p.band_zero = tune.band_zero;
       if (pass == 2) PFCHK0(pf_launch_c2r(fb, n, p, nullptr));
       else PFCHK0(pf_launch_c2r_invariants(fb, n, p, nullptr, 0));
     } else {
@@ -2717,6 +2719,7 @@
     p.aout = p.ain; p.aout.os = (long long)n * out_pitch; p.aout.els = out_pitch;
     p.ncols = ncols; p.nouter = nouter; p.pre = pre ? 1 : 0; p.outer_offset = outer_offset; p.rs = rs; p.growth = growth; p.tw = d_tw; p.etab = d_etab; p.dev = dev;
     p.band_e = band_e < n / 2 ? band_e : n; p.band_outer = band_outer < n / 2 ? band_outer : n;
+    { PfTuning tune; read_tuning(&tune); p.band_zero = tune.band_zero; }
     if (pre && rs != 0.0) PFCHK0(pf_launch_exp_table(d_etab, n, rs, nullptr));
     PFCHK0(pf_launch_strided(fb, n, +1, p, nullptr));
     HIPCHK(nc, hipDeviceSynchronize());
@@ -2747,7 +2750,7 @@
                                    double norm, const double *dc, int ncu, const double *spec, const double *hess, const double *acc, double *out,
                                    int *sentinel_ok) {
   static const int mul6[6] = {PF_MUL_ONE, PF_MUL_ONE, PF_MUL_K2, PF_MUL_ONE, PF_MUL_K, PF_MUL_K};
-  if (!spec || !out || !sentinel_ok || (field_bytes != 8 && field_bytes != 4) || n < 16 || n > 2048 || n % 2 || form < 0 || form > 2 || nrows < 1 ||
+  if (!spec || !out || !sentinel_ok || (field_bytes != 8 && field_bytes != 4) || n < 16 || n > 2048 || n % 2 || form < 0 || form > 3 || nrows < 1 ||
       nrows > (1 << 20) || band < 0 || ncu < 0)
     return pf_fail(0, "pf_debug_zpass_jobs: bad argument");
   const int fb = field_bytes;
@@ -2764,6 +2767,10 @@
       if (in_place && out_f32[j] != 0) return pf_fail(0, "pf_debug_zpass_jobs: only F rows of the fields' own pitch are written in place");
       mu[j] = mul[j]; f32[j] = out_f32[j];
     }
+  } else if (form == 3) {
+    if (fb != 8 || !pf_c2r_invariants_supported(fb, n)) return pf_fail(0, "pf_debug_zpass_jobs: the invariant z-pass in place takes fp64 rows of at most 1024 points, not %d points in fields of %d bytes", n, fb);
+    njobs = 6; in_place = 1;
+    for (int j = 0; j < 6; j++) { mu[j] = mul6[j]; f32[j] = 0; }
   } else {
     if (!hess || !acc) return pf_fail(0, "pf_debug_zpass_jobs: bad argument");
     if (!pf_c2r_invariants_supported(fb, n) || (form == 2 && (n & (n - 1))))
@@ -2778,7 +2785,7 @@
   const size_t field_b = R * row_b;
   auto out_rows_b = [&](int j) { return f32[j] == 0 ? field_b : R * n * (f32[j] == 1 ? 4 : fb); };
   auto out_buf_b = [&](int j) { return f32[j] == 0 ? field_b : out_rows_b(j) + (size_t)n * 8 + 4096; };
-  void *d_in[PF_MAX_JOBS] = {}, *d_out[PF_MAX_JOBS] = {}, *d_acc = nullptr, *d_tw = nullptr; double *d_dc = nullptr;
+  void *d_in[PF_MAX_JOBS] = {}, *d_out[PF_MAX_JOBS] = {}, *d_acc = nullptr, *d_tw = nullptr; double *d_dc = nullptr, *d_flag = nullptr;
   int dev = 0;
   {
     hipDeviceProp_t prop;
@@ -2809,7 +2816,10 @@
       else image(hess + (size_t)j * R * n, (size_t)n, before[j]);
       HIPCHK(nc, hipMemcpy(d_out[j], before[j].data(), before[j].size(), hipMemcpyHostToDevice));
     }
-    if (form != 0) {
+    if (form == 3) {
+      HIPCHK(nc, hipMalloc((void **)&d_flag, sizeof(double)));
+      HIPCHK(nc, hipMemset(d_flag, 0, sizeof(double)));
+    } else if (form != 0) {
       HIPCHK(nc, hipMalloc(&d_acc, field_b));
       image(acc, (size_t)n, acc_before);
       HIPCHK(nc, hipMemcpy(d_acc, acc_before.data(), field_b, hipMemcpyHostToDevice));
@@ -2826,8 +2836,9 @@
     p.nlines = nrows; p.in_pitch = (long long)nzp; p.out_pitch = 2 * (long long)nzp;
     p.norm = norm; p.dc = d_dc; p.tw = d_tw;
     p.band_k = band < n / 2 ? band : n;
-    p.ncu = ncu; p.dev = dev; p.persist_per_cu = tune.zpass_persist; p.inv_per_cu = tune.zpass_inv_wg_per_cu;
+    p.ncu = ncu; p.dev = dev; p.persist_per_cu = tune.zpass_persist; p.inv_per_cu = tune.zpass_inv_wg_per_cu; p.band_zero = tune.band_zero;
     if (form == 0) PFCHK0(pf_launch_c2r(fb, n, p, nullptr));
+    else if (form == 3) { p.flag = d_flag; PFCHK0(pf_launch_c2r_invariants(fb, n, p, nullptr, 0)); }
     else { p.acc = d_acc; PFCHK0(pf_launch_c2r_invariants(fb, n, p, nullptr, form)); }
     HIPCHK(nc, hipDeviceSynchronize());
     int ok = 1;
@@ -2843,11 +2854,12 @@
     for (int j = 0; j < njobs; j++) {
       after.resize(before[j].size());
       HIPCHK(nc, hipMemcpy(after.data(), d_out[j], after.size(), hipMemcpyDeviceToHost));
-      if (form != 0) collect(after, before[j], row_b, fb, nullptr);
+      if (form == 3) collect(after, before[j], row_b, fb, j < 3 ? out + (size_t)j * R * n : nullptr);
+      else if (form != 0) collect(after, before[j], row_b, fb, nullptr);
       else if (f32[j] == 0) collect(after, before[j], row_b, fb, out + (size_t)j * R * n);
       else { const size_t sb = f32[j] == 1 ? 4 : fb; collect(after, before[j], (size_t)n * sb, sb, out + (size_t)j * R * n); }
     }
-    if (form != 0) {
+    if (form == 1 || form == 2) {
       after.resize(field_b);
       HIPCHK(nc, hipMemcpy(after.data(), d_acc, field_b, hipMemcpyDeviceToHost));
       collect(after, acc_before, row_b, fb, out);
@@ -2857,8 +2869,13 @@
   };
   const int rc = body();
   for (int j = 0; j < PF_MAX_JOBS; j++) { if (d_out[j] != d_in[j]) hipFree(d_out[j]); hipFree(d_in[j]); }
-  hipFree(d_acc); hipFree(d_tw); hipFree(d_dc);
+  hipFree(d_acc); hipFree(d_tw); hipFree(d_dc); hipFree(d_flag);
   return rc;
+}
+
+extern "C" int pf_debug_band_zero_class(int kind, int field_bytes, int n, int band, long long *launched) {
+  if (launched) *launched = pf_band_zero_launches(kind);
+  return pf_band_zero_class(kind, field_bytes, n, band);
 }
 
 extern "C" int pf_debug_strided_xfuse(int field_bytes, int n, int njobs, const int *mul, int nouter, int ncols, int pre, double rs, double growth,
diff --git a/pinocchio_amd/csrc/pf_fft_core.h b/pinocchio_amd/csrc/pf_fft_core.h
--- a/pinocchio_amd/csrc/pf_fft_core.h
+++ b/pinocchio_amd/csrc/pf_fft_core.h
@@ -126,6 +126,49 @@
                  : pf_mk<F>(h * (-u[7].x + u[7].y), h * (-u[7].y - u[7].x));
   }
   pfc<F> e0 = u[0], e1 = u[2], e2 = u[4], e3 = u[6], o0 = u[1], o2 = u[5];
+  u[0] = e0 + o0; u[4] = e0 - o0;
+  u[1] = e1 + o1; u[5] = e1 - o1;
+  u[2] = pf_addi<DIR>(e2, o2); u[6] = pf_subi<DIR>(e2, o2);
+  u[3] = e3 + o3; u[7] = e3 - o3;
+}
+
+template <typename F, bool Z> struct pfz { pfc<F> v; };
+template <bool Z, typename F> PF_HD pfz<F, Z> pfz_mk(pfc<F> v) { pfz<F, Z> r; r.v = v; return r; }
+template <typename F, bool ZA, bool ZB> PF_HD pfz<F, ZA && ZB> pfz_add(pfz<F, ZA> a, pfz<F, ZB> b) {
+  if constexpr (ZB) return pfz_mk<ZA && ZB>(a.v);
+  else if constexpr (ZA) return pfz_mk<false>(b.v);
+  else return pfz_mk<false>(a.v + b.v);
+}
+template <typename F, bool ZA, bool ZB> PF_HD pfz<F, ZA && ZB> pfz_sub(pfz<F, ZA> a, pfz<F, ZB> b) {
+  if constexpr (ZB) return pfz_mk<ZA && ZB>(a.v);
+  else if constexpr (ZA) return pfz_mk<false>(pf_mk<F>(-b.v.x, -b.v.y));
+  else return pfz_mk<false>(a.v - b.v);
+}
+template <int DIR, typename F, bool ZA, bool ZB> PF_HD pfz<F, ZA && ZB> pfz_addi(pfz<F, ZA> a, pfz<F, ZB> b) {
+  if constexpr (ZB) return pfz_mk<ZA && ZB>(a.v);
+  else if constexpr (ZA) return pfz_mk<false>(pf_mul_i<DIR>(b.v));
+  else return pfz_mk<false>(pf_addi<DIR>(a.v, b.v));
+}
+template <int DIR, typename F, bool ZA, bool ZB> PF_HD pfz<F, ZA && ZB> pfz_subi(pfz<F, ZA> a, pfz<F, ZB> b) { return pfz_addi<-DIR>(a, b); }
+template <int DIR, typename F, bool Z0, bool Z1, bool Z2, bool Z3>
+PF_HD void pfz_bfly4(pfz<F, Z0> v0, pfz<F, Z1> v1, pfz<F, Z2> v2, pfz<F, Z3> v3, pfz<F, Z0 && Z1 && Z2 && Z3> (&o)[4]) {
+  const auto a = pfz_add(v0, v2), b = pfz_sub(v0, v2);
+  const auto c = pfz_add(v1, v3), d = pfz_sub(v1, v3);
+  constexpr bool Z = Z0 && Z1 && Z2 && Z3;
+  static_assert(!Z, "each half of a masked butterfly keeps a register: every output has a non-zero term");
+  o[0] = pfz_add(a, c); o[1] = pfz_addi<DIR>(b, d); o[2] = pfz_sub(a, c); o[3] = pfz_subi<DIR>(b, d);
+}
+template <int DIR, int ZMASK, typename F> PF_HD void pf_bfly8_masked(pfc<F> (&u)[8]) {
+#define PFZ_U(m) pfz_mk<((ZMASK >> (m)) & 1) != 0>(u[m])
+  pfz<F, false> e[4], o[4];
+  pfz_bfly4<DIR>(PFZ_U(0), PFZ_U(2), PFZ_U(4), PFZ_U(6), e);
+  pfz_bfly4<DIR>(PFZ_U(1), PFZ_U(3), PFZ_U(5), PFZ_U(7), o);
+#undef PFZ_U
+  const F h = (F)0.70710678118654752440;
+  const pfc<F> u3 = o[1].v, u7 = o[3].v;
+  const pfc<F> o1 = DIR > 0 ? pf_mk<F>(h * (u3.x - u3.y), h * (u3.y + u3.x)) : pf_mk<F>(h * (u3.x + u3.y), h * (u3.y - u3.x));
+  const pfc<F> o3 = DIR > 0 ? pf_mk<F>(h * (-u7.x - u7.y), h * (-u7.y + u7.x)) : pf_mk<F>(h * (-u7.x + u7.y), h * (-u7.y - u7.x));
+  const pfc<F> e0 = e[0].v, e1 = e[1].v, e2 = e[2].v, e3 = e[3].v, o0 = o[0].v, o2 = o[2].v;
   u[0] = e0 + o0; u[4] = e0 - o0;
   u[1] = e1 + o1; u[5] = e1 - o1;
   u[2] = pf_addi<DIR>(e2, o2); u[6] = pf_subi<DIR>(e2, o2);
@@ -198,8 +241,9 @@
   pf_stage_apply<F, N, S, DIR>(v, w);
 }
 
-template <int DIR, typename F> PF_HD void pf_pair16_local(pfc<F> (&v)[8], int tl) {
-  pf_bfly8<DIR>(v);
+template <int DIR, int ZMASK = 0, typename F> PF_HD void pf_pair16_local(pfc<F> (&v)[8], int tl) {
+  if constexpr (ZMASK != 0) pf_bfly8_masked<DIR, ZMASK>(v);
+  else pf_bfly8<DIR>(v);
   if (tl & 1) {
     const F c1 = (F)0.92387953251128675613, s1 = (F)0.38268343236508977173, h = (F)0.70710678118654752440;
     v[1] = DIR > 0 ? pf_mk<F>(c1 * v[1].x - s1 * v[1].y, c1 * v[1].y + s1 * v[1].x) : pf_mk<F>(c1 * v[1].x + s1 * v[1].y, c1 * v[1].y - s1 * v[1].x);
diff --git a/pinocchio_amd/csrc/pf_fft_kernels.hip b/pinocchio_amd/csrc/pf_fft_kernels.hip
--- a/pinocchio_amd/csrc/pf_fft_kernels.hip
+++ b/pinocchio_amd/csrc/pf_fft_kernels.hip
@@ -59,10 +59,14 @@
 };
 
 constexpr int PF_DIR_XF = 2;
+constexpr bool pf_zreg(int zc, int m) { return m >= 4 - zc / 2 && m < 4 + zc / 2; }
 template <typename F, int N, int T, int DIRS, bool FA>
 __global__ void __launch_bounds__(T *N / 8) __attribute__((amdgpu_waves_per_eu(4))) k_strided(const PfStridedParams p, const long long nwork, const int ntiles) {
   constexpr bool XF = DIRS == PF_DIR_XF;
-  constexpr int DIR = XF ? +1 : DIRS;
+  constexpr int ZC = DIRS > 16 ? DIRS - 16 : (DIRS < -16 ? -DIRS - 16 : 0);
+  constexpr int DIR = XF ? +1 : (ZC ? (DIRS > 0 ? +1 : -1) : DIRS);
+  constexpr int ZLO = 4 - ZC / 2, ZHI = 4 + ZC / 2, ZMASK = ((1 << ZHI) - 1) & ~((1 << ZLO) - 1);
+  static_assert(ZC == 0 || ((ZC == 4 || ZC == 6) && pf_lane<F>::n == 1), "zero classes of the strided passes: 4 or 6 registers, one column per thread");
   using C = pfc<F>;
   using COLS = PfCols<F>;
   using S = typename COLS::S;
@@ -95,6 +99,7 @@
     const pfc<S> *__restrict__ in = reinterpret_cast<const pfc<S> *>(inp);
 #pragma unroll
     for (int m = 0; m < 8; m++) {
+      if constexpr (ZC > 0) { if (pf_zreg(ZC, m)) { src[m] = pf_zero<F>(); continue; } }
       const int e = pf_line_index<N, P16>(tlj, m);
       const int se = e > N / 2 ? e - N : e;
       const bool inband = se <= p.band_e && se >= -p.band_e;
@@ -139,7 +144,10 @@
       double we[8];
       if (p.rs != 0.0) {
 #pragma unroll
-        for (int m = 0; m < 8; m++) we[m] = p.etab[pf_line_index<N, P16>(tlj, m)];
+        for (int m = 0; m < 8; m++) {
+          if constexpr (ZC > 0) { if (pf_zreg(ZC, m)) { we[m] = 1.0; continue; } }
+          we[m] = p.etab[pf_line_index<N, P16>(tlj, m)];
+        }
       } else {
 #pragma unroll
         for (int m = 0; m < 8; m++) we[m] = 1.0;
@@ -150,6 +158,7 @@
         const double ko2kc2 = ko * ko + kc * kc;
 #pragma unroll
         for (int m = 0; m < 8; m++) {
+          if constexpr (ZC > 0) { if (pf_zreg(ZC, m)) continue; }
           const int e = pf_line_index<N, P16>(tlj, m);
           const double ke = kf * (e > N / 2 ? e - N : e);
           const double k2 = ke * ke + ko2kc2;
@@ -162,6 +171,7 @@
     const int mul = p.job[j].mul;
 #pragma unroll
     for (int m = 0; m < 8; m++) {
+      if constexpr (ZC > 0) { if (pf_zreg(ZC, m)) { v[m] = pf_zero<F>(); continue; } }
       const int e = pf_line_index<N, P16>(tlj, m);
       const F ke = (F)(S)(kf * (e > N / 2 ? e - N : e));
       C x = src[m];
@@ -171,7 +181,7 @@
       v[m] = x;
     }
     if (j + 1 < p.njobs && p.job[j + 1].in != p.job[j].in) load_tile(p.job[j + 1].in, tlj, colj);
-    PfStages<F, N, DIR, 1, 0, false, P16>::run(
+    PfStages<F, N, DIR, 1, 0, false, P16, ZMASK>::run(
         v, tlj, tw, [&](int pos, C val) { lds[pos * T + cj] = val; }, [&](int pos) { return lds[pos * T + cj]; });
 #if defined(PF_DUMMY_VALU) && PF_DUMMY_VALU > 0
     if constexpr (NL == 1) {
@@ -388,9 +398,11 @@
   static constexpr bool spec(int mode) { return spec0 && (mode == 0 || PF_ZI_SPEC_LPT); }
   static constexpr int reducer_waves = M / 256;
 };
-template <typename F, int N, int MODE, bool SPEC>
+template <typename F, int N, int MODE, bool SPEC, int ZC = 0>
 __device__ __forceinline__ void pf_c2r_invariants_body(const PfC2RParams &p, long long nrows) {
   using C = pfc<F>;
+  constexpr int ZLO = 4 - ZC / 2, ZHI = 4 + ZC / 2, ZMASK = ((1 << ZHI) - 1) & ~((1 << ZLO) - 1);
+  static_assert(ZC == 0 || (SPEC && MODE == 0 && sizeof(F) == 8 && !PF_ZI_DMA && PF_ZI_OWN && (ZC == 2 || ZC == 4)), "zero classes: the fp64 sweep form only");
   using F2 = typename pf_vec2<F>::type;
   constexpr bool IN_PLACE = sizeof(F) == 8;
   constexpr int M = N / 2, NT = M / 8, TL = 6;
@@ -427,6 +439,7 @@
     const C *__restrict__ row = in + R * p.in_pitch;
 #pragma unroll
     for (int m = 0; m < 8; m++) {
+      if constexpr (ZC > 0) { if (pf_zreg(ZC, m)) continue; }
       const int k = tl + m * NT;
       nxt[m] = (k <= p.band_k) ? pf_ld_stream(&row[k]) : pf_mk<F>(0, 0);
     }
@@ -520,13 +533,17 @@
     } else {
       if (!PREFETCH && !SPEC && !LATE) fetch(R);
 #pragma unroll
-      for (int m = 0; m < 8; m++) L[tlj + m * NT] = nxt[m];
-      if (tlj == 0) L[M] = nxt[8];
+      for (int m = 0; m < 8; m++) {
+        if constexpr (ZC > 0) { if (pf_zreg(ZC, m)) continue; }
+        L[tlj + m * NT] = nxt[m];
+      }
+      if (tlj == 0) { L[M] = nxt[8]; if constexpr (ZC > 0) L[ZLO * NT] = pf_mk<F>(0, 0); }
     }
     line_sync();
     C v[8];
 #pragma unroll
     for (int m = 0; m < 8; m++) {
+      if constexpr (ZC > 0) { if (pf_zreg(ZC, m)) { v[m] = pf_zero<F>(); continue; } }
       const int e = tlj + m * NT;
       v[m] = pf_zfold<F>((PF_ZI_OWN && !PREFETCH && !DMA) ? nxt[m] : L[e], L[M - e], e, M, mul, kf, tw[e], m == 0 || PF_ZFOLD_K0_ALL(F));
     }
@@ -535,7 +552,7 @@
 #ifndef PF_ZI_HOIST_TW
 #define PF_ZI_HOIST_TW 0
 #endif
-    PfStages<F, M, +1, 2, 0, (NT <= 64)>::run(
+    PfStages<F, M, +1, 2, 0, (NT <= 64), false, ZMASK>::run(
         v, tlj, tw, [&](int pos, C val) { L[PLAN::pad(pos)] = val; }, [&](int pos) { return L[PLAN::pad(pos)]; }, PF_ZI_HOIST_TW ? tl : -1);
     line_sync();
     C *H = L;
@@ -546,7 +563,10 @@
       if (R + gridDim.x < nrows) fetch(R + gridDim.x);
       else {
 #pragma unroll
-        for (int m = 0; m < 9; m++) nxt[m] = pf_mk<F>(0, 0);
+        for (int m = 0; m < 9; m++) {
+          if constexpr (ZC > 0) { if (pf_zreg(ZC, m)) continue; }
+          nxt[m] = pf_mk<F>(0, 0);
+        }
       }
     }
     if (!SPEC) reduce_row(R, 2 * tidj, 2 * NTHR);
@@ -562,6 +582,9 @@
 template <typename F, int N, int MODE = 0>
 __global__ void __launch_bounds__(6 * (N / 16) + 64 * (N / 512)) __attribute__((amdgpu_waves_per_eu(N >= 2048 ? 8 : 6)))
 k_c2r_invariants_spec(const PfC2RParams p, long long nrows) { pf_c2r_invariants_body<F, N, MODE, true>(p, nrows); }
+template <typename F, int N, int ZC>
+__global__ void __launch_bounds__(6 * (N / 16) + 64 * (N / 512)) __attribute__((amdgpu_waves_per_eu(6)))
+k_c2r_invariants_spec_z(const PfC2RParams p, long long nrows) { pf_c2r_invariants_body<F, N, 0, true, ZC>(p, nrows); }
 
 #ifndef PF_ZI_PK2
 #define PF_ZI_PK2 1
@@ -820,6 +843,30 @@
 }
 
 
+#ifndef PF_BZ_ZPASS
+#define PF_BZ_ZPASS 1
+#endif
+#ifndef PF_BZ_STRIDED_ON
+#define PF_BZ_STRIDED_ON 1
+#endif
+int pf_band_zero_class(int kind, int field_bytes, int n, int band) {
+  if (field_bytes != 8 || band < 0 || band >= n / 2) return 0;
+  if (kind == PF_BZ_ZPASS_INV && !PF_BZ_ZPASS) return 0;
+  if (kind == PF_BZ_STRIDED && !PF_BZ_STRIDED_ON) return 0;
+  if (kind == PF_BZ_ZPASS_INV && (n == 1024 || n == 512)) {
+    const int nt = n / 16;
+    return band < 2 * nt ? 4 : band < 3 * nt ? 2 : 0;
+  }
+  if (kind == PF_BZ_STRIDED && n == 1024) {
+    const int nt = n / 8;
+    return band < nt ? 6 : band < 2 * nt ? 4 : 0;
+  }
+  return 0;
+}
+static std::atomic<long long> pf_bz_launches[2];
+long long pf_band_zero_launches(int kind) { return kind == PF_BZ_ZPASS_INV || kind == PF_BZ_STRIDED ? pf_bz_launches[kind].load() : 0; }
+constexpr int pf_dir_zero(int dir, int zc) { return dir * (16 + zc); }
+
 template <typename F, int N> struct PfTileCols {
 #ifndef PF_TILE_LDS_KB
 #define PF_TILE_LDS_KB 128
@@ -863,7 +910,14 @@
   auto lane_fits = [&](const PfAddr &a) {
     return (1 << a.el_shift) >= NT && a.els > 0 && ((unsigned long long)(NT - 1) * (unsigned long long)a.els + (unsigned long long)(NL * T)) * sizeof(pfc<S>) < (1ull << 32);
   };
-  if (lane_fits(p.ain) && lane_fits(p.aout)) return launch_strided_v<F, N, DIR, true>(p, st, ntiles, nwork);
+  const bool fa = lane_fits(p.ain) && lane_fits(p.aout);
+  if constexpr (sizeof(F) == 8 && NL == 1 && N == 1024 && (DIR == +1 || DIR == -1)) {
+    const int zc = p.band_zero ? pf_band_zero_class(PF_BZ_STRIDED, 8, N, p.band_e) : 0;
+    if (zc) pf_bz_launches[PF_BZ_STRIDED]++;
+    if (zc == 6) return fa ? launch_strided_v<F, N, pf_dir_zero(DIR, 6), true>(p, st, ntiles, nwork) : launch_strided_v<F, N, pf_dir_zero(DIR, 6), false>(p, st, ntiles, nwork);
+    if (zc == 4) return fa ? launch_strided_v<F, N, pf_dir_zero(DIR, 4), true>(p, st, ntiles, nwork) : launch_strided_v<F, N, pf_dir_zero(DIR, 4), false>(p, st, ntiles, nwork);
+  }
+  if (fa) return launch_strided_v<F, N, DIR, true>(p, st, ntiles, nwork);
   return launch_strided_v<F, N, DIR, false>(p, st, ntiles, nwork);
 }
 #ifndef PF_F32_PAIRS
@@ -933,8 +987,17 @@
     const long long npairs = (p.nlines + 1) / 2;
     if (g2 > npairs) g2 = npairs;
     hipLaunchKernelGGL((k_c2r_invariants_pk2<N, RW>), dim3((unsigned)g2), dim3(threads), shm2, st, p, p.nlines);
-  } else if constexpr (PfZiPlan<F, M>::spec(0)) hipLaunchKernelGGL((k_c2r_invariants_spec<F, N, 0>), dim3((unsigned)g), dim3(6 * NT + 64 * PfZiPlan<F, M>::reducer_waves), shm, st, p, p.nlines);
-  else hipLaunchKernelGGL((k_c2r_invariants<F, N, 0>), dim3((unsigned)g), dim3(6 * NT), shm, st, p, p.nlines);
+  } else if constexpr (PfZiPlan<F, M>::spec(0)) {
+    int zc = 0;
+    if constexpr (sizeof(F) == 8 && (N == 1024 || N == 512) && !PF_ZI_DMA && PF_ZI_OWN) zc = p.band_zero ? pf_band_zero_class(PF_BZ_ZPASS_INV, 8, N, p.band_k) : 0;
+    const dim3 blk(6 * NT + 64 * PfZiPlan<F, M>::reducer_waves);
+    if constexpr (sizeof(F) == 8 && (N == 1024 || N == 512) && !PF_ZI_DMA && PF_ZI_OWN) {
+      if (zc == 4) hipLaunchKernelGGL((k_c2r_invariants_spec_z<F, N, 4>), dim3((unsigned)g), blk, shm, st, p, p.nlines);
+      else if (zc == 2) hipLaunchKernelGGL((k_c2r_invariants_spec_z<F, N, 2>), dim3((unsigned)g), blk, shm, st, p, p.nlines);
+      if (zc) pf_bz_launches[PF_BZ_ZPASS_INV]++;
+    }
+    if (!zc) hipLaunchKernelGGL((k_c2r_invariants_spec<F, N, 0>), dim3((unsigned)g), blk, shm, st, p, p.nlines);
+  } else hipLaunchKernelGGL((k_c2r_invariants<F, N, 0>), dim3((unsigned)g), dim3(6 * NT), shm, st, p, p.nlines);
   return hipGetLastError() == hipSuccess ? 0 : 1;
 }
 
diff --git a/pinocchio_amd/csrc/pf_fft_stages.h b/pinocchio_amd/csrc/pf_fft_stages.h
--- a/pinocchio_amd/csrc/pf_fft_stages.h
+++ b/pinocchio_amd/csrc/pf_fft_stages.h
@@ -15,7 +15,7 @@
 __device__ __forceinline__ pf_f32x2 pf_lane_xor8(pf_f32x2 x) { pf_f32x2 r; r.x = pf_lane_xor8(x.x); r.y = pf_lane_xor8(x.y); return r; }
 template <typename F> __device__ __forceinline__ pfc<F> pf_lane_xor8(pfc<F> a) { return pf_mk<F>(pf_lane_xor8(a.x), pf_lane_xor8(a.y)); }
 
-template <typename F, int N, int DIR, int TWS, int S = 0, bool WAVE_LOCAL = false, bool P16 = false>
+template <typename F, int N, int DIR, int TWS, int S = 0, bool WAVE_LOCAL = false, bool P16 = false, int ZMASK = 0>
 struct PfStages {
   template <typename WR, typename RD>
   static __device__ __forceinline__ void exchange(pfc<F> (&v)[8], int tl, WR wr, RD rd) {
@@ -31,13 +31,16 @@
   static __device__ __forceinline__ void run(pfc<F> (&v)[8], int tl, const pfc<typename pf_lane<F>::type> *__restrict__ tw, WR wr, RD rd, int tl_tw = -1) {
     static_assert(!WAVE_LOCAL || N / 8 <= 64, "a wave-local transform has at most 64 threads");
     const int tt = tl_tw < 0 ? tl : tl_tw;
+    static_assert(ZMASK == 0 || pf_radix(N, 0, P16) >= 8, "a masked first stage is a radix-8 butterfly per thread");
     if constexpr (S == 0 && P16) {
-      pf_pair16_local<DIR>(v, tl);
+      if constexpr (ZMASK != 0) pf_pair16_local<DIR, ZMASK>(v, tl);
+      else pf_pair16_local<DIR>(v, tl);
       typedef typename pf_lane<F>::type SC;
       const F sgn = (F)((tl & 1) ? (SC)-1 : (SC)1);
 #pragma unroll
       for (int m = 0; m < 8; m++) v[m] = pf_pair16_combine1(v[m], pf_lane_xor8(v[m]), sgn);
-    } else if constexpr (S == 0) pf_stage<F, N, 0, DIR, TWS>(v, tt, tw);
+    } else if constexpr (S == 0 && ZMASK != 0) pf_bfly8_masked<DIR, ZMASK>(v);
+    else if constexpr (S == 0) pf_stage<F, N, 0, DIR, TWS>(v, tt, tw);
     if constexpr (S + 1 < pf_nstages(N, P16)) {
       pfc<F> w[8 / pf_radix(N, S + 1, P16)];
       pf_stage_twiddles<F, N, S + 1, DIR, TWS, 0, P16>(tt, tw, w);
diff --git a/pinocchio_amd/csrc/pf_internal.h b/pinocchio_amd/csrc/pf_internal.h
--- a/pinocchio_amd/csrc/pf_internal.h
+++ b/pinocchio_amd/csrc/pf_internal.h
@@ -24,6 +24,7 @@
   bool distribute_lds;
   bool gtab;
   bool lpt3b_start;
+  bool band_zero;
   bool lpt_xfuse;
 };
 
@@ -56,6 +57,7 @@
   int band_e, band_outer;
   int dev;
   int out_e0, out_ne;
+  int band_zero;
 };
 
 int pf_launch_strided(int field_bytes, int n, int dir, const PfStridedParams &p, hipStream_t st);
@@ -81,6 +83,7 @@
   const double *dc;
   const void *tw;
   int band_k;
+  int band_zero;
   void *acc;
   double *flag;
   int ncu, dev;
@@ -89,7 +92,11 @@
   double *inv_out[3];
   long long inv_pitch;
 };
+static_assert(sizeof(PfStridedParams) == 304 && sizeof(PfC2RParams) == 272, "kernel arguments: the layout every pass kernel was compiled against");
 int pf_launch_c2r(int field_bytes, int n, const PfC2RParams &p, hipStream_t st);
+enum { PF_BZ_ZPASS_INV = 0, PF_BZ_STRIDED = 1 };
+int pf_band_zero_class(int kind, int field_bytes, int n, int band);
+long long pf_band_zero_launches(int kind);
 int pf_launch_c2r_invariants(int field_bytes, int n, const PfC2RParams &p, hipStream_t st, int mode = 0);
 
 struct PfR2CParams {
```

After: 1.542 billion (median of 6 runs). About the same (+0.6%).
